# openjamoses/TOSEM-2021-Replication

Hardware: AMD Instinct MI355X
Metric: train_tokens_per_s (higher is better)
Workload: dtype bf16; 1 GPU; model=mltc-base, global_batch=128, seq_len=512, parallelism=dp1

## Files before the change

csrc/flash_attn.hip:

```cpp

#include "common.h"

typedef __attribute__((ext_vector_type(16))) float f32x16;
typedef __attribute__((ext_vector_type(2))) unsigned uint2_t;
typedef __attribute__((ext_vector_type(4))) unsigned uint4_t;

#define FA_DH 64
#define FA_KVB 32
#define FA_QB 32
#define FA_WAVES 4
#define FA_BLOCK (FA_WAVES * WAVE)
#define FA_QWG (FA_WAVES * FA_QB)
#define FA_Q2WG (2 * FA_QWG)

#define TILE_LDS_BYTES (FA_KVB * 128)
#define FWD_LDS_BYTES (2 * TILE_LDS_BYTES + FA_WAVES * 64 * sizeof(float))
#define BWD_LDS_BYTES (2 * TILE_LDS_BYTES + 64 * sizeof(float))
#define BWD_SEG_LDS_BYTES (BWD_LDS_BYTES + 32 * sizeof(int))
#define DQ_LDS_BYTES TILE_LDS_BYTES
#define DQR_LDS_BYTES (2 * TILE_LDS_BYTES + 16)

struct FaGeom {
  long qkv_bs, qkv_hs; int qkv_rs;
  long o_bs, o_hs; int o_rs;
  static FaGeom bhld(int H, int L) {
    return {(long)H * L * FA_DH, (long)L * FA_DH, FA_DH,
            (long)H * L * FA_DH, (long)L * FA_DH, FA_DH};
  }
  static FaGeom packed(int H, int L) {
    const int D = H * FA_DH;
    return {(long)L * 3 * D, 64L, 3 * D, (long)L * D, 64L, D};
  }
};


__device__ __forceinline__ int kswz(int row, int byte_off) {
  return byte_off ^ ((row & 7) << 4);
}

__device__ __forceinline__ int c_row(int r, int half) {
  return (r & 3) + 8 * (r >> 2) + 4 * half;
}

struct FaStager {
  int row, byte;
  __device__ __forceinline__ explicit FaStager(int tid)
      : row(tid >> 3), byte((tid & 7) * 16) {}
  __device__ __forceinline__ short8_t load(const short* base, int row0,
                                           int rs) const {
    return *(const short8_t*)(base + (long)(row0 + row) * rs + (byte >> 1));
  }
  __device__ __forceinline__ void store(short* lds, short8_t v) const {
    *(short8_t*)((char*)lds + row * 128 + kswz(row, byte)) = v;
  }
};

__device__ __forceinline__ short8_t tile_row_frag(const short* lds, int col,
                                                  int half, int c) {
  return *(const short8_t*)((const char*)lds + col * 128 +
                            kswz(col, (16 * c + 8 * half) * 2));
}

__device__ __forceinline__ void cvt_pk_swap(const float (&s)[16], int r0,
                                            int r1, uint4_t& u, int i) {
  unsigned lo, hi;
  asm("v_cvt_pk_bf16_f32 %0, %1, %2\n\ts_nop 1" : "=v"(lo)
      : "v"(s[r0]), "v"(s[r0 + 1]));
  asm("v_cvt_pk_bf16_f32 %0, %1, %2\n\ts_nop 1" : "=v"(hi)
      : "v"(s[r1]), "v"(s[r1 + 1]));
  auto sw = __builtin_amdgcn_permlane32_swap(lo, hi, false, false);
  u[i] = sw[0]; u[i + 2] = sw[1];
}

__device__ __forceinline__ void c_to_afrag2(const float (&sa)[16],
                                            short8_t (&fa)[2],
                                            const float (&sb)[16],
                                            short8_t (&fb)[2]) {
#pragma unroll
  for (int c = 0; c < 2; ++c) {
    uint4_t ua, ub;
#pragma unroll
    for (int i = 0; i < 2; ++i) {
      int r0 = c * 8 + 2 * i;
      int r1 = c * 8 + 4 + 2 * i;
      cvt_pk_swap(sa, r0, r1, ua, i);
      cvt_pk_swap(sb, r0, r1, ub, i);
    }
    fa[c] = __builtin_bit_cast(short8_t, ua);
    fb[c] = __builtin_bit_cast(short8_t, ub);
  }
}

struct FaTrFrags {
  uint2_t r[8];
  __device__ __forceinline__ short8_t frag(int c, int t) const {
    uint4_t w;
    w[0] = r[c * 4 + 0 * 2 + t][0];
    w[1] = r[c * 4 + 0 * 2 + t][1];
    w[2] = r[c * 4 + 1 * 2 + t][0];
    w[3] = r[c * 4 + 1 * 2 + t][1];
    return __builtin_bit_cast(short8_t, w);
  }
};

struct FaTrOffsets { unsigned a[8]; };

__device__ __forceinline__ FaTrOffsets tr_offsets(int lane, int half) {
  const int row_mate = (lane >> 2) & 3;
  const int d_lane = 16 * ((lane >> 4) & 1) + 4 * (lane & 3);
  FaTrOffsets o;
#pragma unroll
  for (int c = 0; c < 2; ++c)
#pragma unroll
    for (int rr = 0; rr < 2; ++rr)
#pragma unroll
      for (int t = 0; t < 2; ++t) {
        int row = 16 * c + 8 * half + 4 * rr + row_mate;
        int dcol = (32 * t + d_lane) * 2;
        o.a[c * 4 + rr * 2 + t] = row * 128 + kswz(row, dcol);
      }
  return o;
}

__device__ __forceinline__ void tr_issue(const short* lds,
                                         const FaTrOffsets& o, FaTrFrags& f) {
  const unsigned base = (unsigned)(unsigned long)(char*)lds;
  unsigned a[8];
#pragma unroll
  for (int i = 0; i < 8; ++i) a[i] = base + o.a[i];
  asm volatile(
      "ds_read_b64_tr_b16 %0, %8\n\t"
      "ds_read_b64_tr_b16 %1, %9\n\t"
      "ds_read_b64_tr_b16 %2, %10\n\t"
      "ds_read_b64_tr_b16 %3, %11\n\t"
      "ds_read_b64_tr_b16 %4, %12\n\t"
      "ds_read_b64_tr_b16 %5, %13\n\t"
      "ds_read_b64_tr_b16 %6, %14\n\t"
      "ds_read_b64_tr_b16 %7, %15\n\t"
      "s_waitcnt lgkmcnt(0)"
      : "=&v"(f.r[0]), "=&v"(f.r[1]), "=&v"(f.r[2]), "=&v"(f.r[3]),
        "=&v"(f.r[4]), "=&v"(f.r[5]), "=&v"(f.r[6]), "=&v"(f.r[7])
      : "v"(a[0]), "v"(a[1]), "v"(a[2]), "v"(a[3]), "v"(a[4]), "v"(a[5]),
        "v"(a[6]), "v"(a[7])
      : "memory");
}

__device__ __forceinline__ void tr_gather(const short* lds,
                                          const FaTrOffsets& o, FaTrFrags& f) {
  tr_issue(lds, o, f);
  __builtin_amdgcn_sched_barrier(0);
}

struct FaQBlocks { int bh, qA, qB; };

__device__ __forceinline__ FaQBlocks fa_qblocks(int L, int wid) {
  const int n_qblocks = (L + FA_Q2WG - 1) / FA_Q2WG;
  const int bid = xcd_group_remap(blockIdx.x, gridDim.x, n_qblocks);
  const int qA = (bid % n_qblocks) * FA_Q2WG + wid * FA_QB;
  return {bid / n_qblocks, qA, qA + FA_QWG};
}

__device__ __forceinline__ int fa_last_active_kv(const float* mrow, int L,
                                                 int tid, int* scratch) {
  if (tid == 0) *scratch = -1;
  __syncthreads();
  int loc = -1;
  for (int kv = tid; kv < L; kv += FA_BLOCK)
    if (mrow[kv] > -1.0e8f) loc = kv;
  if (loc >= 0) atomicMax(scratch, loc);
  __syncthreads();
  return *scratch;
}

#define FA_SEG_BIAS -1.0e9f

struct FaRange { int lo, hi; };

__device__ __forceinline__ FaRange fa_seg_range(const int* srow, int L,
                                                int r_lo, int r_hi, int tid,
                                                int* scratch) {
  const int s_first = srow[r_lo], s_last = srow[r_hi];
  if (tid == 0) { scratch[0] = r_lo; scratch[1] = r_hi; }
  __syncthreads();
  int lo = r_lo, hi = r_hi;
  for (int j = tid; j < L; j += FA_BLOCK) {
    const int s = srow[j];
    if (s == s_first) lo = min(lo, j);
    if (s == s_last) hi = max(hi, j);
  }
  atomicMin(&scratch[0], lo);
  atomicMax(&scratch[1], hi);
  __syncthreads();
  return {scratch[0], scratch[1]};
}

__device__ __forceinline__ bool fa_seg_tile_live(const int (&r)[16], int a,
                                                 int b) {
  bool hit = false;
#pragma unroll
  for (int i = 0; i < 16; ++i) hit |= (r[i] == a) | (r[i] == b);
  return __builtin_amdgcn_ballot_w64(hit) != 0;
}

template <bool SEG>
__global__ void __launch_bounds__(FA_BLOCK, 2)
flash_fwd_kernel(const short* __restrict__ q, const short* __restrict__ k,
                 const short* __restrict__ v, const float* __restrict__ mask,
                 const int* __restrict__ seg,
                 short* __restrict__ o, float* __restrict__ lse,
                 int B, int H, int L, float scale, FaGeom g) {
  extern __shared__ __attribute__((aligned(16))) char smem[];
  short* k_lds = (short*)smem;
  short* v_lds = (short*)(smem + TILE_LDS_BYTES);
  float* alpha_lds = (float*)(smem + 2 * TILE_LDS_BYTES);

  const int tid = threadIdx.x;
  const int lane = tid & (WAVE - 1);
  const int wid = tid / WAVE;
  const int col = lane & 31;
  const int half = lane >> 5;
  const FaTrOffsets tro = tr_offsets(lane, half);

  const FaQBlocks qb = fa_qblocks(L, wid);
  const int b = qb.bh / H;
  const int h = qb.bh % H;
  const long qkv_off = (long)b * g.qkv_bs + (long)h * g.qkv_hs;
  const long o_off = (long)b * g.o_bs + (long)h * g.o_hs;
  const int my_qA = qb.qA + col;
  const int my_qB = qb.qB + col;
  const bool validA = my_qA < L;
  const bool validB = my_qB < L;
  const float* mrow = (!SEG && mask) ? mask + (long)b * L : nullptr;
  const int* srow = SEG ? seg + (long)b * L : nullptr;
  int sqA = 0, sqB = 0;
  if constexpr (SEG) {
    sqA = srow[validA ? my_qA : L - 1];
    sqB = srow[validB ? my_qB : L - 1];
  }

  short8_t qfA[4], qfB[4];
  {
    const short* qrA = q + qkv_off + (long)(validA ? my_qA : L - 1) * g.qkv_rs;
    const short* qrB = q + qkv_off + (long)(validB ? my_qB : L - 1) * g.qkv_rs;
#pragma unroll
    for (int c = 0; c < 4; ++c) {
      qfA[c] = *(const short8_t*)(qrA + c * 16 + half * 8);
      qfB[c] = *(const short8_t*)(qrB + c * 16 + half * 8);
    }
  }

  f32x16 oA[2], oB[2];
#pragma unroll
  for (int t = 0; t < 2; ++t) { oA[t] = (f32x16)(0.f); oB[t] = (f32x16)(0.f); }
  float mA = -3.0e38f, lA = 0.f, mB = -3.0e38f, lB = 0.f;

  const int n_kv = L / FA_KVB;
  int kt_begin = 0;
  int n_kv_eff = n_kv;
  if (mrow) {
    int last = fa_last_active_kv(mrow, L, tid, (int*)alpha_lds);
    if (last >= 0) n_kv_eff = min(n_kv, last / FA_KVB + 1);
  }
  if constexpr (SEG) {
    const int q_lo = qb.qA - wid * FA_QB;
    const FaRange kr = fa_seg_range(srow, L, q_lo, min(q_lo + FA_Q2WG, L) - 1,
                                    tid, (int*)alpha_lds);
    kt_begin = kr.lo / FA_KVB;
    n_kv_eff = kr.hi / FA_KVB + 1;
  }
  const FaStager st(tid);
  short8_t kv8 = st.load(k + qkv_off, kt_begin * FA_KVB, g.qkv_rs);
  short8_t vv8 = st.load(v + qkv_off, kt_begin * FA_KVB, g.qkv_rs);
  for (int kt = kt_begin; kt < n_kv_eff; ++kt) {
    const int kv0 = kt * FA_KVB;
    __syncthreads();
    st.store(k_lds, kv8);
    st.store(v_lds, vv8);
    __syncthreads();
    if (kt + 1 < n_kv_eff) {
      kv8 = st.load(k + qkv_off, kv0 + FA_KVB, g.qkv_rs);
      vv8 = st.load(v + qkv_off, kv0 + FA_KVB, g.qkv_rs);
    }

    float mb_r[16];
    int sk_r[16];
#pragma unroll
    for (int r = 0; r < 16; ++r) {
      if constexpr (SEG) sk_r[r] = srow[kv0 + c_row(r, half)];
      else mb_r[r] = mrow ? mrow[kv0 + c_row(r, half)] : 0.f;
    }
    if constexpr (SEG) {
      if (!fa_seg_tile_live(sk_r, sqA, sqB)) continue;
    }

    f32x16 sA = (f32x16)(0.f), sB = (f32x16)(0.f);
    __builtin_amdgcn_s_setprio(1);
#pragma unroll
    for (int c = 0; c < 4; ++c) {
      short8_t kf = tile_row_frag(k_lds, col, half, c);
      sA = __builtin_amdgcn_mfma_f32_32x32x16_bf16(kf, qfA[c], sA, 0, 0, 0);
      sB = __builtin_amdgcn_mfma_f32_32x32x16_bf16(kf, qfB[c], sB, 0, 0, 0);
    }
    __builtin_amdgcn_s_setprio(0);

    float svA[16], svB[16];
    float tmaxA = -3.0e38f, tmaxB = -3.0e38f;
#pragma unroll
    for (int r = 0; r < 16; ++r) {
      float mbA, mbB;
      if constexpr (SEG) {
        mbA = sk_r[r] == sqA ? 0.f : FA_SEG_BIAS;
        mbB = sk_r[r] == sqB ? 0.f : FA_SEG_BIAS;
      } else {
        mbA = mbB = mb_r[r];
      }
      float xA = sA[r] * scale + mbA;
      float xB = sB[r] * scale + mbB;
      svA[r] = xA; svB[r] = xB;
      tmaxA = fmaxf(tmaxA, xA);
      tmaxB = fmaxf(tmaxB, xB);
    }
    tmaxA = fmaxf(tmaxA, __shfl_xor(tmaxA, 32, WAVE));
    tmaxB = fmaxf(tmaxB, __shfl_xor(tmaxB, 32, WAVE));
    float mnA = fmaxf(mA, tmaxA), mnB = fmaxf(mB, tmaxB);
    float aA = __expf(mA - mnA), aB = __expf(mB - mnB);
    float rsA = 0.f, rsB = 0.f;
#pragma unroll
    for (int r = 0; r < 16; ++r) {
      svA[r] = __expf(svA[r] - mnA);
      svB[r] = __expf(svB[r] - mnB);
      rsA += svA[r];
      rsB += svB[r];
    }
    rsA += __shfl_xor(rsA, 32, WAVE);
    rsB += __shfl_xor(rsB, 32, WAVE);
    lA = lA * aA + rsA; mA = mnA;
    lB = lB * aB + rsB; mB = mnB;

    if (__builtin_amdgcn_ballot_w64(aA != 1.f || aB != 1.f)) {
      alpha_lds[wid * 64 + col] = aA;
      alpha_lds[wid * 64 + 32 + col] = aB;
#pragma unroll
      for (int t = 0; t < 2; ++t) {
#pragma unroll
        for (int r = 0; r < 16; ++r) {
          int qrow = c_row(r, half);
          oA[t][r] *= alpha_lds[wid * 64 + qrow];
          oB[t][r] *= alpha_lds[wid * 64 + 32 + qrow];
        }
      }
    }

    short8_t pfA[2], pfB[2];
    c_to_afrag2(svA, pfA, svB, pfB);

    FaTrFrags vT;
    tr_gather(v_lds, tro, vT);
    __builtin_amdgcn_s_setprio(1);
#pragma unroll
    for (int t = 0; t < 2; ++t) {
#pragma unroll
      for (int c = 0; c < 2; ++c) {
        short8_t vf = vT.frag(c, t);
        oA[t] = __builtin_amdgcn_mfma_f32_32x32x16_bf16(pfA[c], vf, oA[t],
                                                        0, 0, 0);
        oB[t] = __builtin_amdgcn_mfma_f32_32x32x16_bf16(pfB[c], vf, oB[t],
                                                        0, 0, 0);
      }
    }
    __builtin_amdgcn_s_setprio(0);
  }

  if (lse != nullptr && half == 0) {
    if (validA) lse[(long)qb.bh * L + my_qA] = mA + __logf(lA);
    if (validB) lse[(long)qb.bh * L + my_qB] = mB + __logf(lB);
  }
  const float invA = 1.0f / lA, invB = 1.0f / lB;
#pragma unroll
  for (int r = 0; r < 16; ++r) {
    int rloc = c_row(r, half);
    float iA = __shfl(invA, rloc, WAVE);
    float iB = __shfl(invB, rloc, WAVE);
    int qA = qb.qA + rloc, qB = qb.qB + rloc;
#pragma unroll
    for (int t = 0; t < 2; ++t) {
      if (qA < L)
        o[o_off + (long)qA * g.o_rs + 32 * t + col] =
            f32_to_bf16(oA[t][r] * iA);
      if (qB < L)
        o[o_off + (long)qB * g.o_rs + 32 * t + col] =
            f32_to_bf16(oB[t][r] * iB);
    }
  }
}

static dim3 fa_grid(int B, int H, int L, int rows_per_wg) {
  return dim3(B * H * ((L + rows_per_wg - 1) / rows_per_wg));
}

static void fa_fwd_dispatch(const short* q, const short* k, const short* v,
                            const void* mask, const void* seg, void* o,
                            void* lse, int B, int H, int L, float scale,
                            FaGeom g, hipStream_t stream) {
  const dim3 grid = fa_grid(B, H, L, FA_Q2WG);
  if (seg)
    flash_fwd_kernel<true><<<grid, FA_BLOCK, FWD_LDS_BYTES, stream>>>(
        q, k, v, nullptr, (const int*)seg, (short*)o, (float*)lse, B, H, L,
        scale, g);
  else
    flash_fwd_kernel<false><<<grid, FA_BLOCK, FWD_LDS_BYTES, stream>>>(
        q, k, v, (const float*)mask, nullptr, (short*)o, (float*)lse, B, H, L,
        scale, g);
}

extern "C" hipError_t flash_fwd_launch(const void* q, const void* k,
                                       const void* v, const void* mask,
                                       const void* seg, void* o, void* lse,
                                       int B, int H, int L, float scale,
                                       hipStream_t stream) {
  fa_fwd_dispatch((const short*)q, (const short*)k, (const short*)v, mask,
                  seg, o, lse, B, H, L, scale, FaGeom::bhld(H, L), stream);
  return hipGetLastError();
}

extern "C" hipError_t flash_fwd_packed_launch(const void* qkv,
                                              const void* mask,
                                              const void* seg, void* o,
                                              void* lse, int B, int H, int L,
                                              float scale,
                                              hipStream_t stream) {
  const int D = H * FA_DH;
  fa_fwd_dispatch((const short*)qkv, (const short*)qkv + D,
                  (const short*)qkv + 2 * D, mask, seg, o, lse, B, H, L,
                  scale, FaGeom::packed(H, L), stream);
  return hipGetLastError();
}



template <bool SEG>
__global__ void __launch_bounds__(FA_BLOCK, 2)
flash_bwd_fused_kernel(const short* __restrict__ q, const short* __restrict__ k,
                       const short* __restrict__ v,
                       const short* __restrict__ dout,
                       const float* __restrict__ mask,
                       const int* __restrict__ seg,
                       const float* __restrict__ lse,
                       const float* __restrict__ ddot,
                       short* __restrict__ ds, short* __restrict__ dk,
                       short* __restrict__ dv,
                       int B, int H, int L, float scale, FaGeom g) {
  extern __shared__ __attribute__((aligned(16))) char smem[];
  short* q_lds = (short*)smem;
  short* do_lds = (short*)(smem + TILE_LDS_BYTES);
  float* lse_lds = (float*)(smem + 2 * TILE_LDS_BYTES);
  float* dd_lds = lse_lds + 32;
  int* seg_lds = (int*)(dd_lds + 32);

  const int tid = threadIdx.x;
  const int lane = tid & (WAVE - 1);
  const int wid = tid / WAVE;
  const int col = lane & 31;
  const int half = lane >> 5;
  const FaTrOffsets tro = tr_offsets(lane, half);

  const int n_kvblocks = (L + FA_QWG - 1) / FA_QWG;
  int bid = xcd_group_remap(blockIdx.x, gridDim.x, n_kvblocks);
  int bh = bid / n_kvblocks;
  int kb = bid % n_kvblocks;
  const int b = bh / H;
  const int h = bh % H;
  const long qkv_off = (long)b * g.qkv_bs + (long)h * g.qkv_hs;
  const long o_off = (long)b * g.o_bs + (long)h * g.o_hs;
  const long bh_sq = (long)bh * L * L;
  const int kv_base = kb * FA_QWG + wid * FA_KVB;
  const int my_kv = kv_base + col;
  const bool kv_valid = my_kv < L;
  const float* mrow = (!SEG && mask) ? mask + (long)b * L : nullptr;
  const float mb = mrow ? mrow[min(my_kv, L - 1)] : 0.f;
  const int* srow = SEG ? seg + (long)b * L : nullptr;
  int sk = 0;
  if constexpr (SEG) sk = srow[min(my_kv, L - 1)];

  bool skip_tile = false;
  bool wave_skip = false;
  if (mrow && ds == nullptr) {
    int* any_lds = (int*)lse_lds;
    if (tid == 0) *any_lds = 0;
    __syncthreads();
    if (kv_valid && mb > -1.0e8f) *any_lds = 1;
    __syncthreads();
    skip_tile = (*any_lds == 0) && (mrow[0] > -1.0e8f);
    __syncthreads();
    wave_skip = !skip_tile && (mrow[0] > -1.0e8f) &&
        __builtin_amdgcn_ballot_w64(kv_valid && mb > -1.0e8f) == 0;
  }

  short8_t kf[4], vf[4];
  if (!skip_tile) {
    const short* kr = k + qkv_off + (long)(kv_valid ? my_kv : L - 1) * g.qkv_rs;
    const short* vr = v + qkv_off + (long)(kv_valid ? my_kv : L - 1) * g.qkv_rs;
#pragma unroll
    for (int c = 0; c < 4; ++c) {
      kf[c] = *(const short8_t*)(kr + c * 16 + half * 8);
      vf[c] = *(const short8_t*)(vr + c * 16 + half * 8);
    }
  }
  f32x16 dv_acc[2], dk_acc[2];
#pragma unroll
  for (int t = 0; t < 2; ++t) {
    dv_acc[t] = (f32x16)(0.f);
    dk_acc[t] = (f32x16)(0.f);
  }
  if (!skip_tile) {
  int qt_begin = 0;
  int n_q = L / 32;
  if constexpr (SEG) {
    const int kv_lo = kb * FA_QWG;
    const FaRange qr = fa_seg_range(srow, L, kv_lo, min(kv_lo + FA_QWG, L) - 1,
                                    tid, (int*)lse_lds);
    qt_begin = qr.lo / 32;
    n_q = qr.hi / 32 + 1;
  }
  const FaStager st(tid);
  short8_t qv8 = st.load(q + qkv_off, qt_begin * 32, g.qkv_rs);
  short8_t dv8 = st.load(dout + o_off, qt_begin * 32, g.o_rs);
  for (int qt = qt_begin; qt < n_q; ++qt) {
    const int q0 = qt * 32;
    __syncthreads();
    st.store(q_lds, qv8);
    st.store(do_lds, dv8);
    if (tid < 32) {
      lse_lds[tid] = lse[(long)bh * L + q0 + tid];
      dd_lds[tid] = ddot[(long)bh * L + q0 + tid];
      if constexpr (SEG) seg_lds[tid] = srow[q0 + tid];
    }
    __syncthreads();
    if (qt + 1 < n_q) {
      qv8 = st.load(q + qkv_off, q0 + 32, g.qkv_rs);
      dv8 = st.load(dout + o_off, q0 + 32, g.o_rs);
    }

    if (wave_skip) continue;
    int sq_r[16];
    if constexpr (SEG) {
#pragma unroll
      for (int r = 0; r < 16; ++r) sq_r[r] = seg_lds[c_row(r, half)];
      if (!fa_seg_tile_live(sq_r, sk, sk)) continue;
    }
    f32x16 s_acc = (f32x16)(0.f);
    f32x16 dp_acc = (f32x16)(0.f);
    __builtin_amdgcn_s_setprio(1);
#pragma unroll
    for (int c = 0; c < 4; ++c) {
      short8_t qfrag = tile_row_frag(q_lds, col, half, c);
      short8_t dofrag = tile_row_frag(do_lds, col, half, c);
      s_acc = __builtin_amdgcn_mfma_f32_32x32x16_bf16(qfrag, kf[c], s_acc,
                                                      0, 0, 0);
      dp_acc = __builtin_amdgcn_mfma_f32_32x32x16_bf16(dofrag, vf[c], dp_acc,
                                                       0, 0, 0);
    }
    __builtin_amdgcn_s_setprio(0);

    float pv[16], gv[16];
#pragma unroll
    for (int r = 0; r < 16; ++r) {
      int ql = c_row(r, half);
      float bias = mb;
      if constexpr (SEG) bias = sq_r[r] == sk ? 0.f : FA_SEG_BIAS;
      pv[r] = __expf(s_acc[r] * scale + bias - lse_lds[ql]);
      gv[r] = scale * pv[r] * (dp_acc[r] - dd_lds[ql]);
    }
    if (!SEG && ds != nullptr && kv_valid) {
#pragma unroll
      for (int r = 0; r < 16; ++r)
        ds[bh_sq + (long)(q0 + c_row(r, half)) * L + my_kv] =
            f32_to_bf16(gv[r]);
    }

    short8_t pf[2], gf[2];
    c_to_afrag2(pv, pf, gv, gf);

    FaTrFrags doT, qT;
    tr_issue(do_lds, tro, doT);
    tr_gather(q_lds, tro, qT);
    __builtin_amdgcn_s_setprio(1);
#pragma unroll
    for (int t = 0; t < 2; ++t) {
#pragma unroll
      for (int c = 0; c < 2; ++c) {
        dv_acc[t] = __builtin_amdgcn_mfma_f32_32x32x16_bf16(
            pf[c], doT.frag(c, t), dv_acc[t], 0, 0, 0);
        dk_acc[t] = __builtin_amdgcn_mfma_f32_32x32x16_bf16(
            gf[c], qT.frag(c, t), dk_acc[t], 0, 0, 0);
      }
    }
    __builtin_amdgcn_s_setprio(0);
  }
  }

#pragma unroll
  for (int t = 0; t < 2; ++t) {
#pragma unroll
    for (int r = 0; r < 16; ++r) {
      int kvl = c_row(r, half);
      if (kv_base + kvl >= L) continue;
      long off = qkv_off + (long)(kv_base + kvl) * g.qkv_rs + 32 * t + col;
      dv[off] = f32_to_bf16(dv_acc[t][r]);
      dk[off] = f32_to_bf16(dk_acc[t][r]);
    }
  }
}

static void fa_bwd_fused_dispatch(const short* q, const short* k,
                                  const short* v, const void* dout,
                                  const void* mask, const void* seg,
                                  const void* lse, const void* ddot, void* ds,
                                  short* dk, short* dv, int B, int H, int L,
                                  float scale, FaGeom g, hipStream_t stream) {
  const dim3 grid = fa_grid(B, H, L, FA_QWG);
  if (seg)
    flash_bwd_fused_kernel<true><<<grid, FA_BLOCK, BWD_SEG_LDS_BYTES,
                                   stream>>>(
        q, k, v, (const short*)dout, nullptr, (const int*)seg,
        (const float*)lse, (const float*)ddot, nullptr, dk, dv, B, H, L,
        scale, g);
  else
    flash_bwd_fused_kernel<false><<<grid, FA_BLOCK, BWD_LDS_BYTES, stream>>>(
        q, k, v, (const short*)dout, (const float*)mask, nullptr,
        (const float*)lse, (const float*)ddot, (short*)ds, dk, dv, B, H, L,
        scale, g);
}

extern "C" hipError_t flash_bwd_fused_launch(
    const void* q, const void* k, const void* v, const void* dout,
    const void* mask, const void* seg, const void* lse, const void* ddot,
    void* ds, void* dk, void* dv, int B, int H, int L, float scale,
    hipStream_t stream) {
  if (seg && ds) return hipErrorInvalidValue;
  fa_bwd_fused_dispatch((const short*)q, (const short*)k, (const short*)v,
                        dout, mask, seg, lse, ddot, ds, (short*)dk,
                        (short*)dv, B, H, L, scale, FaGeom::bhld(H, L),
                        stream);
  return hipGetLastError();
}

extern "C" hipError_t flash_bwd_fused_packed_launch(
    const void* qkv, const void* dout, const void* mask, const void* seg,
    const void* lse, const void* ddot, void* dqkv, int B, int H, int L,
    float scale, hipStream_t stream) {
  const int D = H * FA_DH;
  fa_bwd_fused_dispatch((const short*)qkv, (const short*)qkv + D,
                        (const short*)qkv + 2 * D, dout, mask, seg, lse, ddot,
                        nullptr, (short*)dqkv + D, (short*)dqkv + 2 * D, B, H,
                        L, scale, FaGeom::packed(H, L), stream);
  return hipGetLastError();
}

extern "C" __global__ void __launch_bounds__(FA_BLOCK, 2)
flash_dq_kernel(const short* __restrict__ ds, const short* __restrict__ k,
                short* __restrict__ dq, int B, int H, int L) {
  extern __shared__ __attribute__((aligned(16))) char smem[];
  short* k_lds = (short*)smem;

  const int tid = threadIdx.x;
  const int lane = tid & (WAVE - 1);
  const int wid = tid / WAVE;
  const int col = lane & 31;
  const int half = lane >> 5;
  const FaTrOffsets tro = tr_offsets(lane, half);

  const FaQBlocks qb = fa_qblocks(L, wid);
  const long bh_off = (long)qb.bh * L * FA_DH;
  const long bh_sq = (long)qb.bh * L * L;
  const int my_qA = min(qb.qA + col, L - 1);
  const int my_qB = min(qb.qB + col, L - 1);
  const short* dsA_row = ds + bh_sq + (long)my_qA * L;
  const short* dsB_row = ds + bh_sq + (long)my_qB * L;

  f32x16 oA[2], oB[2];
#pragma unroll
  for (int t = 0; t < 2; ++t) { oA[t] = (f32x16)(0.f); oB[t] = (f32x16)(0.f); }

  const int n_kv = L / FA_KVB;
  const FaStager st(tid);
  short8_t kv8 = st.load(k + bh_off, 0, FA_DH);
  for (int kt = 0; kt < n_kv; ++kt) {
    const int kv0 = kt * FA_KVB;
    __syncthreads();
    st.store(k_lds, kv8);
    __syncthreads();
    if (kt + 1 < n_kv) kv8 = st.load(k + bh_off, kv0 + FA_KVB, FA_DH);
    short8_t aA[2], aB[2];
#pragma unroll
    for (int c = 0; c < 2; ++c) {
      aA[c] = *(const short8_t*)(dsA_row + kv0 + 16 * c + 8 * half);
      aB[c] = *(const short8_t*)(dsB_row + kv0 + 16 * c + 8 * half);
    }
    FaTrFrags kT;
    tr_gather(k_lds, tro, kT);
    __builtin_amdgcn_s_setprio(1);
#pragma unroll
    for (int t = 0; t < 2; ++t) {
#pragma unroll
      for (int c = 0; c < 2; ++c) {
        short8_t kf = kT.frag(c, t);
        oA[t] = __builtin_amdgcn_mfma_f32_32x32x16_bf16(aA[c], kf, oA[t],
                                                        0, 0, 0);
        oB[t] = __builtin_amdgcn_mfma_f32_32x32x16_bf16(aB[c], kf, oB[t],
                                                        0, 0, 0);
      }
    }
    __builtin_amdgcn_s_setprio(0);
  }

#pragma unroll
  for (int t = 0; t < 2; ++t) {
#pragma unroll
    for (int r = 0; r < 16; ++r) {
      int rloc = c_row(r, half);
      int qA = qb.qA + rloc, qB = qb.qB + rloc;
      if (qA < L)
        dq[bh_off + (long)qA * FA_DH + 32 * t + col] = f32_to_bf16(oA[t][r]);
      if (qB < L)
        dq[bh_off + (long)qB * FA_DH + 32 * t + col] = f32_to_bf16(oB[t][r]);
    }
  }
}

extern "C" hipError_t flash_dq_launch(const void* ds, const void* k, void* dq,
                                      int B, int H, int L,
                                      hipStream_t stream) {
  flash_dq_kernel<<<fa_grid(B, H, L, FA_Q2WG), FA_BLOCK, DQ_LDS_BYTES,
                    stream>>>(
      (const short*)ds, (const short*)k, (short*)dq, B, H, L);
  return hipGetLastError();
}

template <bool SEG>
__global__ void __launch_bounds__(FA_BLOCK, 2)
flash_dq_recompute_kernel(const short* __restrict__ q,
                          const short* __restrict__ k,
                          const short* __restrict__ v,
                          const short* __restrict__ dout,
                          const float* __restrict__ mask,
                          const int* __restrict__ seg,
                          const float* __restrict__ lse,
                          const float* __restrict__ ddot,
                          short* __restrict__ dq,
                          int B, int H, int L, float scale, FaGeom g) {
  extern __shared__ __attribute__((aligned(16))) char smem[];
  short* k_lds = (short*)smem;
  short* v_lds = (short*)(smem + TILE_LDS_BYTES);
  int* skip_scratch = (int*)(smem + 2 * TILE_LDS_BYTES);

  const int tid = threadIdx.x;
  const int lane = tid & (WAVE - 1);
  const int wid = tid / WAVE;
  const int col = lane & 31;
  const int half = lane >> 5;
  const FaTrOffsets tro = tr_offsets(lane, half);

  const FaQBlocks qb = fa_qblocks(L, wid);
  const int b = qb.bh / H;
  const int h = qb.bh % H;
  const long qkv_off = (long)b * g.qkv_bs + (long)h * g.qkv_hs;
  const long o_off = (long)b * g.o_bs + (long)h * g.o_hs;
  const int my_qA = qb.qA + col;
  const int my_qB = qb.qB + col;
  const bool validA = my_qA < L;
  const bool validB = my_qB < L;
  const float* mrow = (!SEG && mask) ? mask + (long)b * L : nullptr;
  const int* srow = SEG ? seg + (long)b * L : nullptr;
  int sqA = 0, sqB = 0;
  if constexpr (SEG) {
    sqA = srow[validA ? my_qA : L - 1];
    sqB = srow[validB ? my_qB : L - 1];
  }

  short8_t qfA[4], qfB[4], dofA[4], dofB[4];
  {
    const short* qrA = q + qkv_off + (long)(validA ? my_qA : L - 1) * g.qkv_rs;
    const short* qrB = q + qkv_off + (long)(validB ? my_qB : L - 1) * g.qkv_rs;
    const short* drA = dout + o_off + (long)(validA ? my_qA : L - 1) * g.o_rs;
    const short* drB = dout + o_off + (long)(validB ? my_qB : L - 1) * g.o_rs;
#pragma unroll
    for (int c = 0; c < 4; ++c) {
      qfA[c] = *(const short8_t*)(qrA + c * 16 + half * 8);
      qfB[c] = *(const short8_t*)(qrB + c * 16 + half * 8);
      dofA[c] = *(const short8_t*)(drA + c * 16 + half * 8);
      dofB[c] = *(const short8_t*)(drB + c * 16 + half * 8);
    }
  }
  const float lseA = lse[(long)qb.bh * L + (validA ? my_qA : L - 1)];
  const float lseB = lse[(long)qb.bh * L + (validB ? my_qB : L - 1)];
  const float ddA = ddot[(long)qb.bh * L + (validA ? my_qA : L - 1)];
  const float ddB = ddot[(long)qb.bh * L + (validB ? my_qB : L - 1)];

  f32x16 dqA[2], dqB[2];
#pragma unroll
  for (int t = 0; t < 2; ++t) { dqA[t] = (f32x16)(0.f); dqB[t] = (f32x16)(0.f); }

  const int n_kv = L / FA_KVB;
  int kt_begin = 0;
  int n_kv_eff = n_kv;
  if (mrow) {
    int last = fa_last_active_kv(mrow, L, tid, skip_scratch);
    if (last >= 0) n_kv_eff = min(n_kv, last / FA_KVB + 1);
  }
  if constexpr (SEG) {
    const int q_lo = qb.qA - wid * FA_QB;
    const FaRange kr = fa_seg_range(srow, L, q_lo, min(q_lo + FA_Q2WG, L) - 1,
                                    tid, skip_scratch);
    kt_begin = kr.lo / FA_KVB;
    n_kv_eff = kr.hi / FA_KVB + 1;
  }
  const FaStager st(tid);
  short8_t kv8 = st.load(k + qkv_off, kt_begin * FA_KVB, g.qkv_rs);
  short8_t vv8 = st.load(v + qkv_off, kt_begin * FA_KVB, g.qkv_rs);
  for (int kt = kt_begin; kt < n_kv_eff; ++kt) {
    const int kv0 = kt * FA_KVB;
    __syncthreads();
    st.store(k_lds, kv8);
    st.store(v_lds, vv8);
    __syncthreads();
    if (kt + 1 < n_kv_eff) {
      kv8 = st.load(k + qkv_off, kv0 + FA_KVB, g.qkv_rs);
      vv8 = st.load(v + qkv_off, kv0 + FA_KVB, g.qkv_rs);
    }

    float mb_r[16];
    int sk_r[16];
#pragma unroll
    for (int r = 0; r < 16; ++r) {
      if constexpr (SEG) sk_r[r] = srow[kv0 + c_row(r, half)];
      else mb_r[r] = mrow ? mrow[kv0 + c_row(r, half)] : 0.f;
    }
    if constexpr (SEG) {
      if (!fa_seg_tile_live(sk_r, sqA, sqB)) continue;
    }

    f32x16 sA = (f32x16)(0.f), sB = (f32x16)(0.f);
    f32x16 pA = (f32x16)(0.f), pB = (f32x16)(0.f);
    __builtin_amdgcn_s_setprio(1);
#pragma unroll
    for (int c = 0; c < 4; ++c) {
      short8_t kf = tile_row_frag(k_lds, col, half, c);
      short8_t vf = tile_row_frag(v_lds, col, half, c);
      sA = __builtin_amdgcn_mfma_f32_32x32x16_bf16(kf, qfA[c], sA, 0, 0, 0);
      sB = __builtin_amdgcn_mfma_f32_32x32x16_bf16(kf, qfB[c], sB, 0, 0, 0);
      pA = __builtin_amdgcn_mfma_f32_32x32x16_bf16(vf, dofA[c], pA, 0, 0, 0);
      pB = __builtin_amdgcn_mfma_f32_32x32x16_bf16(vf, dofB[c], pB, 0, 0, 0);
    }
    __builtin_amdgcn_s_setprio(0);

    float gA[16], gB[16];
#pragma unroll
    for (int r = 0; r < 16; ++r) {
      float mbA, mbB;
      if constexpr (SEG) {
        mbA = sk_r[r] == sqA ? 0.f : FA_SEG_BIAS;
        mbB = sk_r[r] == sqB ? 0.f : FA_SEG_BIAS;
      } else {
        mbA = mbB = mb_r[r];
      }
      float expA = __expf(sA[r] * scale + mbA - lseA);
      float expB = __expf(sB[r] * scale + mbB - lseB);
      gA[r] = scale * expA * (pA[r] - ddA);
      gB[r] = scale * expB * (pB[r] - ddB);
    }

    short8_t gfA[2], gfB[2];
    c_to_afrag2(gA, gfA, gB, gfB);

    FaTrFrags kT;
    tr_gather(k_lds, tro, kT);
    __builtin_amdgcn_s_setprio(1);
#pragma unroll
    for (int t = 0; t < 2; ++t) {
#pragma unroll
      for (int c = 0; c < 2; ++c) {
        short8_t kf = kT.frag(c, t);
        dqA[t] = __builtin_amdgcn_mfma_f32_32x32x16_bf16(gfA[c], kf, dqA[t],
                                                         0, 0, 0);
        dqB[t] = __builtin_amdgcn_mfma_f32_32x32x16_bf16(gfB[c], kf, dqB[t],
                                                         0, 0, 0);
      }
    }
    __builtin_amdgcn_s_setprio(0);
  }

#pragma unroll
  for (int t = 0; t < 2; ++t) {
#pragma unroll
    for (int r = 0; r < 16; ++r) {
      int rloc = c_row(r, half);
      int qA = qb.qA + rloc, qB = qb.qB + rloc;
      if (qA < L)
        dq[qkv_off + (long)qA * g.qkv_rs + 32 * t + col] =
            f32_to_bf16(dqA[t][r]);
      if (qB < L)
        dq[qkv_off + (long)qB * g.qkv_rs + 32 * t + col] =
            f32_to_bf16(dqB[t][r]);
    }
  }
}

static void fa_dq_recompute_dispatch(const short* q, const short* k,
                                     const short* v, const void* dout,
                                     const void* mask, const void* seg,
                                     const void* lse, const void* ddot,
                                     void* dq, int B, int H, int L,
                                     float scale, FaGeom g,
                                     hipStream_t stream) {
  const dim3 grid = fa_grid(B, H, L, FA_Q2WG);
  if (seg)
    flash_dq_recompute_kernel<true><<<grid, FA_BLOCK, DQR_LDS_BYTES,
                                      stream>>>(
        q, k, v, (const short*)dout, nullptr, (const int*)seg,
        (const float*)lse, (const float*)ddot, (short*)dq, B, H, L, scale, g);
  else
    flash_dq_recompute_kernel<false><<<grid, FA_BLOCK, DQR_LDS_BYTES,
                                       stream>>>(
        q, k, v, (const short*)dout, (const float*)mask, nullptr,
        (const float*)lse, (const float*)ddot, (short*)dq, B, H, L, scale, g);
}

extern "C" hipError_t flash_dq_recompute_launch(
    const void* q, const void* k, const void* v, const void* dout,
    const void* mask, const void* seg, const void* lse, const void* ddot,
    void* dq, int B, int H, int L, float scale, hipStream_t stream) {
  fa_dq_recompute_dispatch((const short*)q, (const short*)k, (const short*)v,
                           dout, mask, seg, lse, ddot, dq, B, H, L, scale,
                           FaGeom::bhld(H, L), stream);
  return hipGetLastError();
}

extern "C" hipError_t flash_dq_recompute_packed_launch(
    const void* qkv, const void* dout, const void* mask, const void* seg,
    const void* lse, const void* ddot, void* dqkv, int B, int H, int L,
    float scale, hipStream_t stream) {
  const int D = H * FA_DH;
  fa_dq_recompute_dispatch((const short*)qkv, (const short*)qkv + D,
                           (const short*)qkv + 2 * D, dout, mask, seg, lse,
                           ddot, dqkv, B, H, L, scale, FaGeom::packed(H, L),
                           stream);
  return hipGetLastError();
}

__device__ __forceinline__ float fa_row_dot(const short* dr, const short* orow,
                                            int sub) {
  short4_t a = *(const short4_t*)(dr + sub * 4);
  short4_t c = *(const short4_t*)(orow + sub * 4);
  float s = 0.f;
#pragma unroll
  for (int j = 0; j < 4; ++j) s += bf16_to_f32(a[j]) * bf16_to_f32(c[j]);
#pragma unroll
  for (int off = 8; off > 0; off >>= 1) s += __shfl_xor(s, off, 16);
  return s;
}

extern "C" __global__ void __launch_bounds__(256)
fa_dot_kernel(const short* __restrict__ dout, const short* __restrict__ o,
              float* __restrict__ ddot, long n_rows) {
  long row = ((long)blockIdx.x * 256 + threadIdx.x) >> 4;
  if (row >= n_rows) return;
  int sub = threadIdx.x & 15;
  float s = fa_row_dot(dout + row * FA_DH, o + row * FA_DH, sub);
  if (sub == 0) ddot[row] = s;
}

extern "C" __global__ void __launch_bounds__(256)
fa_dot_packed_kernel(const short* __restrict__ dout,
                     const short* __restrict__ o, float* __restrict__ ddot,
                     int B, int H, int L) {
  const int D = H * FA_DH;
  long n_rows = (long)B * L * H;
  long chunk = ((long)blockIdx.x * 256 + threadIdx.x) >> 4;
  if (chunk >= n_rows) return;
  int sub = threadIdx.x & 15;
  int h = (int)(chunk % H);
  long bl = chunk / H;
  int l = (int)(bl % L);
  int b = (int)(bl / L);
  float s = fa_row_dot(dout + bl * D + h * FA_DH, o + bl * D + h * FA_DH, sub);
  if (sub == 0) ddot[((long)b * H + h) * L + l] = s;
}

extern "C" hipError_t fa_dot_packed_launch(const void* dout, const void* o,
                                           void* ddot, int B, int H, int L,
                                           hipStream_t stream) {
  long total_threads = (long)B * H * L * 16;
  int grid = (int)((total_threads + 255) / 256);
  fa_dot_packed_kernel<<<grid, 256, 0, stream>>>(
      (const short*)dout, (const short*)o, (float*)ddot, B, H, L);
  return hipGetLastError();
}

extern "C" hipError_t fa_dot_launch(const void* dout, const void* o,
                                    void* ddot, long n_rows,
                                    hipStream_t stream) {
  long total_threads = n_rows * 16;
  int grid = (int)((total_threads + 255) / 256);
  fa_dot_kernel<<<grid, 256, 0, stream>>>((const short*)dout, (const short*)o,
                                          (float*)ddot, n_rows);
  return hipGetLastError();
}

extern "C" __global__ void __launch_bounds__(64)
tr_probe_kernel(const short* __restrict__ src, short* __restrict__ out,
                int scheme) {
  __shared__ __attribute__((aligned(16))) short lds[256];
  int lane = threadIdx.x;
  for (int i = lane; i < 256; i += 64) lds[i] = src[i];
  __syncthreads();
  int addr;
  switch (scheme) {
    case 0: addr = 0; break;
    case 1: addr = (lane & 15) * 2; break;
    case 2: addr = ((lane & 15) + (lane >> 4) * 64) * 2; break;
    case 3: addr = (lane >> 4) * 128; break;
    case 4: addr = (lane & 3) * 16; break;
    case 5: addr = ((lane & 3) * 32 + 4 * ((lane >> 2) & 7)) * 2; break;
    case 6: addr = ((lane & 3) * 8 + 4) * 2; break;
    case 7: addr = ((lane & 3) == 0) ? 16 : 0; break;
    case 8: addr = ((lane & 3) == 1) ? 16 : 0; break;
    case 9: addr = ((lane & 3) == 2) ? 16 : 0; break;
    case 10: addr = ((lane & 3) == 3) ? 16 : 0; break;
    case 11: addr = ((lane & 3) * 64 + 4 * ((lane >> 2) & 7)) * 2; break;
    default: addr = ((lane & 3) * 8 + ((lane >> 2) & 7) * 32) * 2; break;
  }
  typedef __attribute__((ext_vector_type(2))) unsigned uint2_t;
  uint2_t r;
  unsigned base = (unsigned)(unsigned long)((char*)lds + addr);
  asm volatile("ds_read_b64_tr_b16 %0, %1\n\ts_waitcnt lgkmcnt(0)"
               : "=v"(r) : "v"(base) : "memory");
  __builtin_amdgcn_sched_barrier(0);
  out[lane * 4 + 0] = (short)(r[0] & 0xffff);
  out[lane * 4 + 1] = (short)(r[0] >> 16);
  out[lane * 4 + 2] = (short)(r[1] & 0xffff);
  out[lane * 4 + 3] = (short)(r[1] >> 16);
}

extern "C" hipError_t tr_probe_launch(const void* src, void* out, int scheme,
                                      hipStream_t stream) {
  tr_probe_kernel<<<1, 64, 0, stream>>>((const short*)src, (short*)out,
                                        scheme);
  return hipGetLastError();
}
```

csrc/layernorm.hip:

```cpp

#include "common.h"
#include <cstdlib>
#include <cstring>

#define WAVES_PER_BLOCK 4
#define BLOCK (WAVES_PER_BLOCK * WAVE)
#define MAX_PKT 8

extern "C" {

__global__ void __launch_bounds__(BLOCK)
ln_fwd_kernel(const short* __restrict__ x, const short* __restrict__ res,
              const short* __restrict__ gamma,
              const short* __restrict__ beta, short* __restrict__ y,
              short* __restrict__ s_out,
              float* __restrict__ mean_out, float* __restrict__ rstd_out,
              int N, int D, float eps) {
  const int lane = threadIdx.x & (WAVE - 1);
  const int wid = threadIdx.x / WAVE;
  const int pkts = D / (WAVE * 8);
  for (int row = blockIdx.x * WAVES_PER_BLOCK + wid; row < N;
       row += gridDim.x * WAVES_PER_BLOCK) {
    const short* xr = x + (long)row * D;
    const short* rr = res ? res + (long)row * D : nullptr;
    short* yr = y + (long)row * D;
    short* sr = s_out ? s_out + (long)row * D : nullptr;
    float vals[MAX_PKT * 8];
    float s = 0.f;
    if (pkts <= MAX_PKT && D == pkts * WAVE * 8) {
#pragma unroll
      for (int p = 0; p < MAX_PKT; ++p) {
        if (p >= pkts) break;
        int base = (p * WAVE + lane) * 8;
        short8_t v = *(const short8_t*)(xr + base);
        short8_t so;
#pragma unroll
        for (int j = 0; j < 8; ++j) {
          float f = bf16_to_f32(v[j]);
          vals[p * 8 + j] = f;
        }
        if (rr) {
          short8_t rv = *(const short8_t*)(rr + base);
#pragma unroll
          for (int j = 0; j < 8; ++j) {
            short sum_b = f32_to_bf16(vals[p * 8 + j] + bf16_to_f32(rv[j]));
            vals[p * 8 + j] = bf16_to_f32(sum_b);
            so[j] = sum_b;
          }
          *(short8_t*)(sr + base) = so;
        }
#pragma unroll
        for (int j = 0; j < 8; ++j) s += vals[p * 8 + j];
      }
      float mean = wave_sum(s) / (float)D;
      float var = 0.f;
#pragma unroll
      for (int p = 0; p < MAX_PKT; ++p) {
        if (p >= pkts) break;
#pragma unroll
        for (int j = 0; j < 8; ++j) {
          float d = vals[p * 8 + j] - mean;
          var += d * d;
        }
      }
      var = wave_sum(var) / (float)D;
      float rstd = rsqrtf(var + eps);
      if (lane == 0) { mean_out[row] = mean; rstd_out[row] = rstd; }
#pragma unroll
      for (int p = 0; p < MAX_PKT; ++p) {
        if (p >= pkts) break;
        int base = (p * WAVE + lane) * 8;
        short8_t g8 = *(const short8_t*)(gamma + base);
        short8_t b8 = *(const short8_t*)(beta + base);
        short8_t o;
#pragma unroll
        for (int j = 0; j < 8; ++j) {
          float xhat = (vals[p * 8 + j] - mean) * rstd;
          o[j] = f32_to_bf16(xhat * bf16_to_f32(g8[j]) + bf16_to_f32(b8[j]));
        }
        *(short8_t*)(yr + base) = o;
      }
    } else {
      for (int i = lane * 8; i < D; i += WAVE * 8) {
        short8_t v = *(const short8_t*)(xr + i);
        if (rr) {
          short8_t rv = *(const short8_t*)(rr + i);
          short8_t so;
#pragma unroll
          for (int j = 0; j < 8; ++j) {
            so[j] = f32_to_bf16(bf16_to_f32(v[j]) + bf16_to_f32(rv[j]));
          }
          *(short8_t*)(sr + i) = so;
          v = so;
        }
#pragma unroll
        for (int j = 0; j < 8; ++j) s += bf16_to_f32(v[j]);
      }
      float mean = wave_sum(s) / (float)D;
      float var = 0.f;
      for (int i = lane * 8; i < D; i += WAVE * 8) {
        short8_t v = *(const short8_t*)((rr ? sr : xr) + i);
#pragma unroll
        for (int j = 0; j < 8; ++j) {
          float d = bf16_to_f32(v[j]) - mean;
          var += d * d;
        }
      }
      var = wave_sum(var) / (float)D;
      float rstd = rsqrtf(var + eps);
      if (lane == 0) { mean_out[row] = mean; rstd_out[row] = rstd; }
      for (int i = lane * 8; i < D; i += WAVE * 8) {
        short8_t v = *(const short8_t*)((rr ? sr : xr) + i);
        short8_t g8 = *(const short8_t*)(gamma + i);
        short8_t b8 = *(const short8_t*)(beta + i);
        short8_t o;
#pragma unroll
        for (int j = 0; j < 8; ++j) {
          float xhat = (bf16_to_f32(v[j]) - mean) * rstd;
          o[j] = f32_to_bf16(xhat * bf16_to_f32(g8[j]) + bf16_to_f32(b8[j]));
        }
        *(short8_t*)(yr + i) = o;
      }
    }
  }
}

}

template <int PKTS, bool HASRES>
__global__ void __launch_bounds__(BLOCK)
ln_fwd_t(const short* __restrict__ x, const short* __restrict__ res,
         const short* __restrict__ gamma, const short* __restrict__ beta,
         short* __restrict__ y, short* __restrict__ s_out,
         float* __restrict__ mean_out, float* __restrict__ rstd_out,
         int N, int D, float eps) {
  const int lane = threadIdx.x & (WAVE - 1);
  const int wid = threadIdx.x / WAVE;
  const int rstride = gridDim.x * WAVES_PER_BLOCK;
  int row = blockIdx.x * WAVES_PER_BLOCK + wid;
  if (row >= N) return;
  float gv[PKTS * 8], bv[PKTS * 8];
#pragma unroll
  for (int p = 0; p < PKTS; ++p) {
    int base = (p * WAVE + lane) * 8;
    short8_t g8 = *(const short8_t*)(gamma + base);
    short8_t b8 = *(const short8_t*)(beta + base);
#pragma unroll
    for (int j = 0; j < 8; ++j) {
      gv[p * 8 + j] = bf16_to_f32(g8[j]);
      bv[p * 8 + j] = bf16_to_f32(b8[j]);
    }
  }
  short8_t vx[PKTS], vr[PKTS];
#pragma unroll
  for (int p = 0; p < PKTS; ++p) {
    int base = (p * WAVE + lane) * 8;
    vx[p] = *(const short8_t*)(x + (long)row * D + base);
    if (HASRES) vr[p] = *(const short8_t*)(res + (long)row * D + base);
  }
  while (true) {
    const int next = row + rstride;
    float vals[PKTS * 8];
    float s = 0.f;
#pragma unroll
    for (int p = 0; p < PKTS; ++p) {
      short8_t so;
#pragma unroll
      for (int j = 0; j < 8; ++j) {
        float f = bf16_to_f32(vx[p][j]);
        if (HASRES) {
          short sum_b = f32_to_bf16(f + bf16_to_f32(vr[p][j]));
          f = bf16_to_f32(sum_b);
          so[j] = sum_b;
        }
        vals[p * 8 + j] = f;
        s += f;
      }
      if (HASRES)
        *(short8_t*)(s_out + (long)row * D + (p * WAVE + lane) * 8) = so;
    }
    if (next < N) {
#pragma unroll
      for (int p = 0; p < PKTS; ++p) {
        int base = (p * WAVE + lane) * 8;
        vx[p] = *(const short8_t*)(x + (long)next * D + base);
        if (HASRES) vr[p] = *(const short8_t*)(res + (long)next * D + base);
      }
    }
    float mean = wave_sum(s) / (float)D;
    float var = 0.f;
#pragma unroll
    for (int k = 0; k < PKTS * 8; ++k) {
      float d = vals[k] - mean;
      var += d * d;
    }
    var = wave_sum(var) / (float)D;
    float rstd = rsqrtf(var + eps);
    if (lane == 0) { mean_out[row] = mean; rstd_out[row] = rstd; }
#pragma unroll
    for (int p = 0; p < PKTS; ++p) {
      short8_t o;
#pragma unroll
      for (int j = 0; j < 8; ++j) {
        int k = p * 8 + j;
        o[j] = f32_to_bf16((vals[k] - mean) * rstd * gv[k] + bv[k]);
      }
      *(short8_t*)(y + (long)row * D + (p * WAVE + lane) * 8) = o;
    }
    if (next >= N) break;
    row = next;
  }
}

template <int PKTS, bool HASDE>
__global__ void __launch_bounds__(BLOCK)
ln_bwd_t(const short* __restrict__ dy, const short* __restrict__ x,
         const short* __restrict__ gamma, const float* __restrict__ mean_in,
         const float* __restrict__ rstd_in,
         const short* __restrict__ ds_extra, short* __restrict__ dx,
         float* __restrict__ ws_dgamma, float* __restrict__ ws_dbeta,
         int N, int D) {
  const int lane = threadIdx.x & (WAVE - 1);
  const int wid = threadIdx.x / WAVE;
  float gv[PKTS * 8];
#pragma unroll
  for (int p = 0; p < PKTS; ++p) {
    short8_t g8 = *(const short8_t*)(gamma + (p * WAVE + lane) * 8);
#pragma unroll
    for (int j = 0; j < 8; ++j) gv[p * 8 + j] = bf16_to_f32(g8[j]);
  }
  float dg_acc[PKTS * 8] = {0.f}, db_acc[PKTS * 8] = {0.f};
  const int rstride = gridDim.x * WAVES_PER_BLOCK;
  int row = blockIdx.x * WAVES_PER_BLOCK + wid;
  const bool active = row < N;
  short8_t vd[PKTS], vxp[PKTS], ve[PKTS];
  if (active) {
#pragma unroll
    for (int p = 0; p < PKTS; ++p) {
      int base = (p * WAVE + lane) * 8;
      vd[p] = *(const short8_t*)(dy + (long)row * D + base);
      vxp[p] = *(const short8_t*)(x + (long)row * D + base);
      if (HASDE) ve[p] = *(const short8_t*)(ds_extra + (long)row * D + base);
    }
  }
  while (active) {
    const int next = row + rstride;
    const float mean = mean_in[row], rstd = rstd_in[row];
    float xh[PKTS * 8], dyg[PKTS * 8], ev[PKTS * 8];
    float s1 = 0.f, s2 = 0.f;
#pragma unroll
    for (int p = 0; p < PKTS; ++p) {
#pragma unroll
      for (int j = 0; j < 8; ++j) {
        int k = p * 8 + j;
        float d = bf16_to_f32(vd[p][j]);
        float h = (bf16_to_f32(vxp[p][j]) - mean) * rstd;
        float g = d * gv[k];
        if (HASDE) ev[k] = bf16_to_f32(ve[p][j]);
        xh[k] = h; dyg[k] = g;
        dg_acc[k] += d * h;
        db_acc[k] += d;
        s1 += g; s2 += g * h;
      }
    }
    if (next < N) {
#pragma unroll
      for (int p = 0; p < PKTS; ++p) {
        int base = (p * WAVE + lane) * 8;
        vd[p] = *(const short8_t*)(dy + (long)next * D + base);
        vxp[p] = *(const short8_t*)(x + (long)next * D + base);
        if (HASDE) ve[p] = *(const short8_t*)(ds_extra + (long)next * D + base);
      }
    }
    s1 = wave_sum(s1) / (float)D;
    s2 = wave_sum(s2) / (float)D;
#pragma unroll
    for (int p = 0; p < PKTS; ++p) {
      short8_t o;
#pragma unroll
      for (int j = 0; j < 8; ++j) {
        int k = p * 8 + j;
        float d_ = rstd * (dyg[k] - s1 - xh[k] * s2);
        if (HASDE) d_ += ev[k];
        o[j] = f32_to_bf16(d_);
      }
      *(short8_t*)(dx + (long)row * D + (p * WAVE + lane) * 8) = o;
    }
    if (next >= N) break;
    row = next;
  }
  float* og = ws_dgamma +
              (long)(blockIdx.x * WAVES_PER_BLOCK + wid) * D;
  float* ob = ws_dbeta + (long)(blockIdx.x * WAVES_PER_BLOCK + wid) * D;
#pragma unroll
  for (int p = 0; p < PKTS; ++p) {
    int base = (p * WAVE + lane) * 8;
#pragma unroll
    for (int j = 0; j < 8; ++j) {
      og[base + j] = dg_acc[p * 8 + j];
      ob[base + j] = db_acc[p * 8 + j];
    }
  }
}

template <int PKTS, bool HASDE>
__global__ void __launch_bounds__(BLOCK)
ln_bwd_t2(const short* __restrict__ dy, const short* __restrict__ x,
          const short* __restrict__ gamma, const float* __restrict__ mean_in,
          const float* __restrict__ rstd_in,
          const short* __restrict__ ds_extra, short* __restrict__ dx,
          float* __restrict__ ws_dgamma, float* __restrict__ ws_dbeta,
          int N, int D) {
  const int lane = threadIdx.x & (WAVE - 1);
  const int wid = threadIdx.x / WAVE;
  float gv[PKTS * 8];
#pragma unroll
  for (int p = 0; p < PKTS; ++p) {
    short8_t g8 = *(const short8_t*)(gamma + (p * WAVE + lane) * 8);
#pragma unroll
    for (int j = 0; j < 8; ++j) gv[p * 8 + j] = bf16_to_f32(g8[j]);
  }
  float dg_acc[PKTS * 8] = {0.f}, db_acc[PKTS * 8] = {0.f};
  const int rstride = gridDim.x * WAVES_PER_BLOCK * 2;
  int rowA = (blockIdx.x * WAVES_PER_BLOCK + wid) * 2;
  short8_t vdA[PKTS], vxA[PKTS], veA[PKTS];
  short8_t vdB[PKTS], vxB[PKTS], veB[PKTS];
  bool actA = rowA < N, actB = rowA + 1 < N;
  if (actA) {
#pragma unroll
    for (int p = 0; p < PKTS; ++p) {
      int base = (p * WAVE + lane) * 8;
      vdA[p] = *(const short8_t*)(dy + (long)rowA * D + base);
      vxA[p] = *(const short8_t*)(x + (long)rowA * D + base);
      if (HASDE) veA[p] = *(const short8_t*)(ds_extra + (long)rowA * D + base);
      if (actB) {
        vdB[p] = *(const short8_t*)(dy + (long)(rowA + 1) * D + base);
        vxB[p] = *(const short8_t*)(x + (long)(rowA + 1) * D + base);
        if (HASDE)
          veB[p] = *(const short8_t*)(ds_extra + (long)(rowA + 1) * D + base);
      }
    }
  }
  while (actA) {
    const int next = rowA + rstride;
    const float meanA = mean_in[rowA], rstdA = rstd_in[rowA];
    const float meanB = actB ? mean_in[rowA + 1] : 0.f;
    const float rstdB = actB ? rstd_in[rowA + 1] : 0.f;
    float xhA[PKTS * 8], dygA[PKTS * 8];
    float xhB[PKTS * 8], dygB[PKTS * 8];
    float s1A = 0.f, s2A = 0.f, s1B = 0.f, s2B = 0.f;
#pragma unroll
    for (int p = 0; p < PKTS; ++p) {
#pragma unroll
      for (int j = 0; j < 8; ++j) {
        int k = p * 8 + j;
        float dA = bf16_to_f32(vdA[p][j]);
        float hA = (bf16_to_f32(vxA[p][j]) - meanA) * rstdA;
        float gA = dA * gv[k];
        xhA[k] = hA; dygA[k] = gA;
        dg_acc[k] += dA * hA;
        db_acc[k] += dA;
        s1A += gA; s2A += gA * hA;
        if (actB) {
          float dB = bf16_to_f32(vdB[p][j]);
          float hB = (bf16_to_f32(vxB[p][j]) - meanB) * rstdB;
          float gB = dB * gv[k];
          xhB[k] = hB; dygB[k] = gB;
          dg_acc[k] += dB * hB;
          db_acc[k] += dB;
          s1B += gB; s2B += gB * hB;
        }
      }
    }
    if (next < N) {
#pragma unroll
      for (int p = 0; p < PKTS; ++p) {
        int base = (p * WAVE + lane) * 8;
        vdA[p] = *(const short8_t*)(dy + (long)next * D + base);
        vxA[p] = *(const short8_t*)(x + (long)next * D + base);
        if (next + 1 < N) {
          vdB[p] = *(const short8_t*)(dy + (long)(next + 1) * D + base);
          vxB[p] = *(const short8_t*)(x + (long)(next + 1) * D + base);
        }
      }
    }
    s1A = wave_sum(s1A) / (float)D;
    s2A = wave_sum(s2A) / (float)D;
    if (actB) {
      s1B = wave_sum(s1B) / (float)D;
      s2B = wave_sum(s2B) / (float)D;
    }
#pragma unroll
    for (int p = 0; p < PKTS; ++p) {
      short8_t oA, oB;
#pragma unroll
      for (int j = 0; j < 8; ++j) {
        int k = p * 8 + j;
        float dA_ = rstdA * (dygA[k] - s1A - xhA[k] * s2A);
        if (HASDE) dA_ += bf16_to_f32(veA[p][j]);
        oA[j] = f32_to_bf16(dA_);
        if (actB) {
          float dB_ = rstdB * (dygB[k] - s1B - xhB[k] * s2B);
          if (HASDE) dB_ += bf16_to_f32(veB[p][j]);
          oB[j] = f32_to_bf16(dB_);
        }
      }
      int base = (p * WAVE + lane) * 8;
      *(short8_t*)(dx + (long)rowA * D + base) = oA;
      if (actB) *(short8_t*)(dx + (long)(rowA + 1) * D + base) = oB;
    }
    if (next >= N) break;
    rowA = next;
    actB = rowA + 1 < N;
    if (HASDE) {
#pragma unroll
      for (int p = 0; p < PKTS; ++p) {
        int base = (p * WAVE + lane) * 8;
        veA[p] = *(const short8_t*)(ds_extra + (long)rowA * D + base);
        if (actB)
          veB[p] = *(const short8_t*)(ds_extra + (long)(rowA + 1) * D + base);
      }
    }
  }
  float* og = ws_dgamma + (long)(blockIdx.x * WAVES_PER_BLOCK + wid) * D;
  float* ob = ws_dbeta + (long)(blockIdx.x * WAVES_PER_BLOCK + wid) * D;
#pragma unroll
  for (int p = 0; p < PKTS; ++p) {
    int base = (p * WAVE + lane) * 8;
#pragma unroll
    for (int j = 0; j < 8; ++j) {
      og[base + j] = dg_acc[p * 8 + j];
      ob[base + j] = db_acc[p * 8 + j];
    }
  }
}

template <int MAXP>
__global__ void __launch_bounds__(BLOCK)
ln_bwd_g(const short* __restrict__ dy, const short* __restrict__ x,
         const short* __restrict__ gamma, const float* __restrict__ mean_in,
         const float* __restrict__ rstd_in,
         const short* __restrict__ ds_extra,
         short* __restrict__ dx,
         float* __restrict__ ws_dgamma, float* __restrict__ ws_dbeta,
         int N, int D) {
  const int lane = threadIdx.x & (WAVE - 1);
  const int wid = threadIdx.x / WAVE;
  extern __shared__ __attribute__((aligned(16))) char smem[];
  float* sg = (float*)smem;
  float* sb = sg + D;
  float dg_acc[MAXP * 8] = {0.f}, db_acc[MAXP * 8] = {0.f};
  for (int row = blockIdx.x * WAVES_PER_BLOCK + wid; row < N;
       row += gridDim.x * WAVES_PER_BLOCK) {
    const short* dyr = dy + (long)row * D;
    const short* xr = x + (long)row * D;
    const short* der = ds_extra ? ds_extra + (long)row * D : nullptr;
    short* dxr = dx + (long)row * D;
    const float mean = mean_in[row], rstd = rstd_in[row];
    short8_t vd[MAXP], vx[MAXP], vg[MAXP];
    float s1 = 0.f, s2 = 0.f;
#pragma unroll
    for (int p = 0; p < MAXP; ++p) {
      int base = (p * WAVE + lane) * 8;
      if (base >= D) continue;
      vd[p] = *(const short8_t*)(dyr + base);
      vx[p] = *(const short8_t*)(xr + base);
      vg[p] = *(const short8_t*)(gamma + base);
#pragma unroll
      for (int j = 0; j < 8; ++j) {
        float d = bf16_to_f32(vd[p][j]);
        float h = (bf16_to_f32(vx[p][j]) - mean) * rstd;
        float g = d * bf16_to_f32(vg[p][j]);
        dg_acc[p * 8 + j] += d * h;
        db_acc[p * 8 + j] += d;
        s1 += g; s2 += g * h;
      }
    }
    s1 = wave_sum(s1) / (float)D;
    s2 = wave_sum(s2) / (float)D;
#pragma unroll
    for (int p = 0; p < MAXP; ++p) {
      int base = (p * WAVE + lane) * 8;
      if (base >= D) continue;
      short8_t ev;
      if (der) ev = *(const short8_t*)(der + base);
      short8_t o;
#pragma unroll
      for (int j = 0; j < 8; ++j) {
        float h = (bf16_to_f32(vx[p][j]) - mean) * rstd;
        float g = bf16_to_f32(vd[p][j]) * bf16_to_f32(vg[p][j]);
        float d_ = rstd * (g - s1 - h * s2);
        if (der) d_ += bf16_to_f32(ev[j]);
        o[j] = f32_to_bf16(d_);
      }
      *(short8_t*)(dxr + base) = o;
    }
  }
  for (int w = 0; w < WAVES_PER_BLOCK; ++w) {
    if (wid == w) {
#pragma unroll
      for (int p = 0; p < MAXP; ++p) {
        int base = (p * WAVE + lane) * 8;
        if (base >= D) continue;
#pragma unroll
        for (int j = 0; j < 8; ++j) {
          float pg = w ? sg[base + j] : 0.f, pb = w ? sb[base + j] : 0.f;
          sg[base + j] = pg + dg_acc[p * 8 + j];
          sb[base + j] = pb + db_acc[p * 8 + j];
        }
      }
    }
    __syncthreads();
  }
  float* og = ws_dgamma + (long)blockIdx.x * D;
  float* ob = ws_dbeta + (long)blockIdx.x * D;
  for (int i = threadIdx.x; i < D; i += BLOCK) { og[i] = sg[i]; ob[i] = sb[i]; }
}

#define LN_BWD_G_MAX_D 4096
__global__ void __launch_bounds__(BLOCK)
ln_bwd_wide_kernel(const short* __restrict__ dy, const short* __restrict__ x,
                   const short* __restrict__ gamma,
                   const float* __restrict__ mean_in,
                   const float* __restrict__ rstd_in,
                   const short* __restrict__ ds_extra,
                   short* __restrict__ dx, float* __restrict__ ws_dgamma,
                   float* __restrict__ ws_dbeta, int N, int D) {
  const int lane = threadIdx.x & (WAVE - 1);
  const int wid = threadIdx.x / WAVE;
  float* og = ws_dgamma + (long)(blockIdx.x * WAVES_PER_BLOCK + wid) * D;
  float* ob = ws_dbeta + (long)(blockIdx.x * WAVES_PER_BLOCK + wid) * D;
  for (int i = lane * 8; i < D; i += WAVE * 8) {
#pragma unroll
    for (int j = 0; j < 8; ++j) { og[i + j] = 0.f; ob[i + j] = 0.f; }
  }
  for (int row = blockIdx.x * WAVES_PER_BLOCK + wid; row < N;
       row += gridDim.x * WAVES_PER_BLOCK) {
    const short* dyr = dy + (long)row * D;
    const short* xr = x + (long)row * D;
    const short* der = ds_extra ? ds_extra + (long)row * D : nullptr;
    short* dxr = dx + (long)row * D;
    const float mean = mean_in[row], rstd = rstd_in[row];
    float s1 = 0.f, s2 = 0.f;
    for (int i = lane * 8; i < D; i += WAVE * 8) {
      short8_t vd = *(const short8_t*)(dyr + i);
      short8_t vx = *(const short8_t*)(xr + i);
      short8_t g8 = *(const short8_t*)(gamma + i);
#pragma unroll
      for (int j = 0; j < 8; ++j) {
        float g = bf16_to_f32(vd[j]) * bf16_to_f32(g8[j]);
        float h = (bf16_to_f32(vx[j]) - mean) * rstd;
        s1 += g; s2 += g * h;
      }
    }
    s1 = wave_sum(s1) / (float)D;
    s2 = wave_sum(s2) / (float)D;
    for (int i = lane * 8; i < D; i += WAVE * 8) {
      short8_t vd = *(const short8_t*)(dyr + i);
      short8_t vx = *(const short8_t*)(xr + i);
      short8_t g8 = *(const short8_t*)(gamma + i);
      short8_t ev;
      if (der) ev = *(const short8_t*)(der + i);
      short8_t o;
#pragma unroll
      for (int j = 0; j < 8; ++j) {
        float d = bf16_to_f32(vd[j]);
        float h = (bf16_to_f32(vx[j]) - mean) * rstd;
        float g = d * bf16_to_f32(g8[j]);
        float d_ = rstd * (g - s1 - h * s2);
        if (der) d_ += bf16_to_f32(ev[j]);
        o[j] = f32_to_bf16(d_);
        og[i + j] += d * h;
        ob[i + j] += d;
      }
      *(short8_t*)(dxr + i) = o;
    }
  }
}

extern "C" {

__global__ void __launch_bounds__(256)
colsum_stage_kernel(const float* __restrict__ ws, float* __restrict__ out,
                    int R, int D, int rows_per_split) {
  int col = (blockIdx.x * 256 + threadIdx.x) * 4;
  if (col >= D) return;
  int r0 = blockIdx.y * rows_per_split;
  int r1 = min(R, r0 + rows_per_split);
  float4_t s = {0.f, 0.f, 0.f, 0.f};
  for (int r = r0; r < r1; ++r) {
    float4_t v = *(const float4_t*)(ws + (long)r * D + col);
#pragma unroll
    for (int j = 0; j < 4; ++j) s[j] += v[j];
  }
  *(float4_t*)(out + (long)blockIdx.y * D + col) = s;
}

__global__ void __launch_bounds__(256)
colsum_bf16_stage1_kernel(const short* __restrict__ x,
                          float* __restrict__ scratch, long N, int D,
                          long rows_per_split) {
  int col = (blockIdx.x * 256 + threadIdx.x) * 8;
  if (col >= D) return;
  long r0 = (long)blockIdx.y * rows_per_split;
  long r1 = min(N, r0 + rows_per_split);
  float s[8] = {0.f};
  for (long r = r0; r < r1; ++r) {
    short8_t v = *(const short8_t*)(x + r * D + col);
#pragma unroll
    for (int j = 0; j < 8; ++j) s[j] += bf16_to_f32(v[j]);
  }
  float* out = scratch + (long)blockIdx.y * D + col;
#pragma unroll
  for (int j = 0; j < 8; ++j) out[j] = s[j];
}

__global__ void __launch_bounds__(256)
colsum_bf16_stage2_kernel(const float* __restrict__ scratch,
                          short* __restrict__ out, int splits, int D) {
  int col = blockIdx.x * 256 + threadIdx.x;
  if (col >= D) return;
  float s = 0.f;
  for (int r = 0; r < splits; ++r) s += scratch[(long)r * D + col];
  out[col] = f32_to_bf16(s);
}

hipError_t colsum_bf16_launch(const void* x, void* scratch, void* out,
                              long N, int D, hipStream_t stream) {
  int gx = (D / 8 + 255) / 256;
  int splits = 1024 / gx;
  if (splits > 1024) splits = 1024;
  if ((long)splits > N) splits = (int)N;
  long rows_per_split = (N + splits - 1) / splits;
  dim3 g1(gx, splits);
  colsum_bf16_stage1_kernel<<<g1, 256, 0, stream>>>(
      (const short*)x, (float*)scratch, N, D, rows_per_split);
  hipError_t e = hipGetLastError();
  if (e != hipSuccess) return e;
  if (splits > 16 && D % 4 == 0) {
    float* mid = (float*)scratch + (long)1024 * D;
    int rps2 = (splits + 15) / 16;
    colsum_stage_kernel<<<dim3((D / 4 + 255) / 256, 16), 256, 0, stream>>>(
        (const float*)scratch, mid, splits, D, rps2);
    e = hipGetLastError();
    if (e != hipSuccess) return e;
    colsum_bf16_stage2_kernel<<<dim3((D + 255) / 256), 256, 0, stream>>>(
        mid, (short*)out, 16, D);
    return hipGetLastError();
  }
  colsum_bf16_stage2_kernel<<<dim3((D + 255) / 256), 256, 0, stream>>>(
      (const float*)scratch, (short*)out, splits, D);
  return hipGetLastError();
}

hipError_t ln_fwd_launch(const void* x, const void* res, const void* gamma,
                         const void* beta, void* y, void* s_out, void* mean,
                         void* rstd, int N, int D, float eps, int grid,
                         hipStream_t stream) {
#define LNF_T(P)                                                              \
  do {                                                                        \
    if (res)                                                                  \
      ln_fwd_t<P, true><<<grid, BLOCK, 0, stream>>>(                          \
          (const short*)x, (const short*)res, (const short*)gamma,            \
          (const short*)beta, (short*)y, (short*)s_out, (float*)mean,         \
          (float*)rstd, N, D, eps);                                           \
    else                                                                      \
      ln_fwd_t<P, false><<<grid, BLOCK, 0, stream>>>(                         \
          (const short*)x, nullptr, (const short*)gamma, (const short*)beta,  \
          (short*)y, (short*)s_out, (float*)mean, (float*)rstd, N, D, eps);   \
  } while (0)
  if (D == 512) LNF_T(1);
  else if (D == 1024) LNF_T(2);
  else if (D == 2048) LNF_T(4);
  else
    ln_fwd_kernel<<<grid, BLOCK, 0, stream>>>(
        (const short*)x, (const short*)res, (const short*)gamma,
        (const short*)beta, (short*)y, (short*)s_out, (float*)mean,
        (float*)rstd, N, D, eps);
#undef LNF_T
  return hipGetLastError();
}

static int ln_bwd_use_1row() {
  static int v = -1;
  if (v < 0) {
    const char* e = getenv("TOSEM_LN_BWD");
    v = (e && strcmp(e, "1row") == 0) ? 1 : 0;
  }
  return v;
}

hipError_t ln_bwd_launch(const void* dy, const void* x, const void* gamma,
                         const void* mean, const void* rstd,
                         const void* ds_extra, void* dx,
                         void* ws_dgamma, void* ws_dbeta, int N, int D,
                         int grid, hipStream_t stream) {
  size_t shm = (size_t)D * 2 * sizeof(float);
#define LNB_T(P)                                                              \
  do {                                                                        \
    if (ln_bwd_use_1row()) {                                                  \
      if (ds_extra)                                                           \
        ln_bwd_t<P, true><<<grid, BLOCK, 0, stream>>>(                        \
            (const short*)dy, (const short*)x, (const short*)gamma,           \
            (const float*)mean, (const float*)rstd, (const short*)ds_extra,   \
            (short*)dx, (float*)ws_dgamma, (float*)ws_dbeta, N, D);           \
      else                                                                    \
        ln_bwd_t<P, false><<<grid, BLOCK, 0, stream>>>(                       \
            (const short*)dy, (const short*)x, (const short*)gamma,           \
            (const float*)mean, (const float*)rstd, nullptr, (short*)dx,      \
            (float*)ws_dgamma, (float*)ws_dbeta, N, D);                       \
      break;                                                                  \
    }                                                                         \
    if (ds_extra)                                                             \
      ln_bwd_t2<P, true><<<grid, BLOCK, 0, stream>>>(                         \
          (const short*)dy, (const short*)x, (const short*)gamma,             \
          (const float*)mean, (const float*)rstd, (const short*)ds_extra,     \
          (short*)dx, (float*)ws_dgamma, (float*)ws_dbeta, N, D);             \
    else                                                                      \
      ln_bwd_t2<P, false><<<grid, BLOCK, 0, stream>>>(                        \
          (const short*)dy, (const short*)x, (const short*)gamma,             \
          (const float*)mean, (const float*)rstd, nullptr, (short*)dx,        \
          (float*)ws_dgamma, (float*)ws_dbeta, N, D);                         \
  } while (0)
#define LNB_G(P)                                                              \
  ln_bwd_g<P><<<grid, BLOCK, shm, stream>>>(                                  \
      (const short*)dy, (const short*)x, (const short*)gamma,                 \
      (const float*)mean, (const float*)rstd, (const short*)ds_extra,         \
      (short*)dx, (float*)ws_dgamma, (float*)ws_dbeta, N, D)
  if (D == 512) LNB_T(1);
  else if (D == 1024) LNB_T(2);
  else if (D <= 512) LNB_G(1);
  else if (D <= 1024) LNB_G(2);
  else if (D <= 2048) LNB_G(4);
  else if (D <= LN_BWD_G_MAX_D) LNB_G(8);
  else
    ln_bwd_wide_kernel<<<grid, BLOCK, 0, stream>>>(
        (const short*)dy, (const short*)x, (const short*)gamma,
        (const float*)mean, (const float*)rstd, (const short*)ds_extra,
        (short*)dx, (float*)ws_dgamma, (float*)ws_dbeta, N, D);
#undef LNB_G
#undef LNB_T
  return hipGetLastError();
}

int ln_bwd_ws_rows(int D, int grid) {
  const bool per_wave = D == 512 || D == 1024 || D > LN_BWD_G_MAX_D;
  return per_wave ? grid * WAVES_PER_BLOCK : grid;
}

#define COLSUM_MAX_SPLITS 256
#define COLSUM_MID 16
hipError_t colsum_launch(const void* ws, void* scratch, void* out, int R,
                         int D, hipStream_t stream) {
  int gx = (D / 4 + 255) / 256;
  dim3 grid1(gx, 1);
  if (R <= COLSUM_MID) {
    colsum_stage_kernel<<<grid1, 256, 0, stream>>>(
        (const float*)ws, (float*)out, R, D, R);
    return hipGetLastError();
  }
  int splits = 1024 / gx;
  if (splits > COLSUM_MAX_SPLITS) splits = COLSUM_MAX_SPLITS;
  if (splits > R) splits = R;
  int rows_per_split = (R + splits - 1) / splits;
  colsum_stage_kernel<<<dim3(gx, splits), 256, 0, stream>>>(
      (const float*)ws, (float*)scratch, R, D, rows_per_split);
  hipError_t e = hipGetLastError();
  if (e != hipSuccess) return e;
  if (splits <= COLSUM_MID) {
    colsum_stage_kernel<<<grid1, 256, 0, stream>>>(
        (const float*)scratch, (float*)out, splits, D, splits);
    return hipGetLastError();
  }
  float* mid = (float*)scratch + (long)COLSUM_MAX_SPLITS * D;
  int rps2 = (splits + COLSUM_MID - 1) / COLSUM_MID;
  colsum_stage_kernel<<<dim3(gx, COLSUM_MID), 256, 0, stream>>>(
      (const float*)scratch, mid, splits, D, rps2);
  e = hipGetLastError();
  if (e != hipSuccess) return e;
  colsum_stage_kernel<<<grid1, 256, 0, stream>>>(
      mid, (float*)out, COLSUM_MID, D, COLSUM_MID);
  return hipGetLastError();
}

}
```

csrc/ops.cpp:

```cpp

#include <torch/extension.h>
#include <c10/hip/HIPStream.h>
#include <hip/hip_runtime.h>
#include <algorithm>
#include <numeric>

extern "C" {
hipError_t ln_fwd_launch(const void*, const void*, const void*, const void*,
                         void*, void*, void*, void*, int, int, float, int,
                         hipStream_t);
hipError_t ln_bwd_launch(const void*, const void*, const void*, const void*,
                         const void*, const void*, void*, void*, void*, int,
                         int, int, hipStream_t);
int ln_bwd_ws_rows(int, int);
hipError_t colsum_launch(const void*, void*, void*, int, int, hipStream_t);
hipError_t bias_gelu_fwd_launch(const void*, const void*, void*, long, int,
                                int, hipStream_t);
hipError_t bias_gelu_bwd_launch(const void*, const void*, const void*, void*,
                                void*, long, int, int, hipStream_t);
hipError_t softmax_fwd_launch(const void*, const void*, void*, long, int, int,
                              float, int, hipStream_t);
hipError_t softmax_bwd_launch(const void*, const void*, void*, long, int,
                              float, int, hipStream_t);
hipError_t adamw_launch(void*, const void*, int, void*, void*, void*, long,
                        float, float, float, float, float, int, float, int,
                        hipStream_t);
hipError_t adamw_clipped_launch(void*, const void*, int, void*, void*, void*,
                                long, float, float, float, float, float, int,
                                const void*, int, hipStream_t);
int grad_norm_grid(long);
hipError_t grad_clip_state_launch(const void*, int, long, float, float, void*,
                                  void*, hipStream_t);
hipError_t qkv_repack_launch(const void*, void*, int, int, int, int, int,
                             hipStream_t);
hipError_t out_repack_launch(const void*, void*, int, int, int, int, int,
                             hipStream_t);
hipError_t qkv_repack_bwd3_launch(const void*, const void*, const void*,
                                  void*, int, int, int, int, hipStream_t);
hipError_t flash_fwd_launch(const void*, const void*, const void*, const void*,
                            const void*, void*, void*, int, int, int, float,
                            hipStream_t);
hipError_t p_from_lse_launch(const void*, const void*, const void*, void*,
                             long, int, int, float, int, hipStream_t);
hipError_t flash_bwd_fused_launch(const void*, const void*, const void*,
                                  const void*, const void*, const void*,
                                  const void*, const void*, void*, void*,
                                  void*, int, int, int, float, hipStream_t);
hipError_t fa_dot_launch(const void*, const void*, void*, long, hipStream_t);
hipError_t fa_dot_packed_launch(const void*, const void*, void*, int, int,
                                int, hipStream_t);
hipError_t flash_fwd_packed_launch(const void*, const void*, const void*,
                                   void*, void*, int, int, int, float,
                                   hipStream_t);
hipError_t flash_bwd_fused_packed_launch(const void*, const void*,
                                         const void*, const void*,
                                         const void*, const void*, void*,
                                         int, int, int, float, hipStream_t);
hipError_t flash_dq_recompute_packed_launch(const void*, const void*,
                                            const void*, const void*,
                                            const void*, const void*, void*,
                                            int, int, int, float,
                                            hipStream_t);
hipError_t flash_dq_recompute_launch(const void*, const void*, const void*,
                                     const void*, const void*, const void*,
                                     const void*, const void*, void*, int,
                                     int, int, float, hipStream_t);
hipError_t flash_dq_launch(const void*, const void*, void*, int, int, int,
                           hipStream_t);
hipError_t masked_pool_fwd_launch(const void*, const void*, void*, void*,
                                  void*, int, int, int, hipStream_t);
hipError_t masked_pool_bwd_launch(const void*, const void*, const void*,
                                  void*, int, int, int, hipStream_t);
hipError_t segment_pool_fwd_launch(const void*, const void*, const void*,
                                   void*, int, long, int, hipStream_t);
hipError_t segment_pool_bwd_launch(const void*, const void*, const void*,
                                   void*, int, long, int, hipStream_t);
hipError_t tr_probe_launch(const void*, void*, int, hipStream_t);
hipError_t colsum_bf16_launch(const void*, void*, void*, long, int,
                              hipStream_t);
hipError_t wgrad_gemm_launch(const void*, const void*, void*, void*, int,
                             int, long, int, hipStream_t);
}

torch::Tensor lt_linear_gelu_bias(torch::Tensor, torch::Tensor,
                                  torch::Tensor);
bool lt_probe_epilogue(long, long, long, long);
std::vector<double> lt_bench_algos(long, long, long, bool, bool, long);

namespace {

#define CHECK_HIP(call)                                                   \
  do {                                                                    \
    hipError_t e_ = (call);                                               \
    TORCH_CHECK(e_ == hipSuccess, "HIP error: ", hipGetErrorString(e_));  \
  } while (0)

hipStream_t cur_stream() {
  return c10::hip::getCurrentHIPStream().stream();
}

void check_bf16(const torch::Tensor& t, const char* name) {
  TORCH_CHECK(t.is_contiguous(), name, " must be contiguous");
  TORCH_CHECK(t.scalar_type() == torch::kBFloat16, name, " must be bf16");
  TORCH_CHECK(t.device().is_cuda(), name, " must be on GPU");
}

void check_f32(const torch::Tensor& t, const char* name) {
  TORCH_CHECK(t.is_contiguous(), name, " must be contiguous");
  TORCH_CHECK(t.scalar_type() == torch::kFloat32, name, " must be f32");
  TORCH_CHECK(t.device().is_cuda(), name, " must be on GPU");
}


struct FlashDims { long B, H, L; };
using NamedTensor = std::pair<const char*, torch::Tensor>;

const void* flash_mask_ptr(const c10::optional<torch::Tensor>& mask,
                           const FlashDims& d) {
  if (!mask.has_value()) return nullptr;
  check_f32(*mask, "mask");
  TORCH_CHECK(mask->dim() == 2 && mask->size(0) == d.B &&
              mask->size(1) == d.L, "mask must be [B, L]");
  return mask->data_ptr();
}

const void* flash_seg_ptr(const c10::optional<torch::Tensor>& seg,
                          const c10::optional<torch::Tensor>& mask,
                          const torch::Tensor& x, const FlashDims& d) {
  if (!seg.has_value()) return nullptr;
  TORCH_CHECK(!mask.has_value(), "mask and seg are mutually exclusive");
  TORCH_CHECK(seg->scalar_type() == torch::kInt32, "seg must be int32");
  TORCH_CHECK(seg->device() == x.device(), "seg must be on the same device "
              "as the attention inputs");
  TORCH_CHECK(seg->is_contiguous(), "seg must be contiguous");
  TORCH_CHECK(seg->dim() == 2 && seg->size(0) == d.B && seg->size(1) == d.L,
              "seg must be [B, L]");
  return seg->data_ptr();
}

void check_i32(const torch::Tensor& t, const torch::Tensor& like,
               const char* name) {
  TORCH_CHECK(t.is_contiguous(), name, " must be contiguous");
  TORCH_CHECK(t.scalar_type() == torch::kInt32, name, " must be int32");
  TORCH_CHECK(t.device() == like.device(), name, " must be on the same "
              "device as the data");
}

void check_flash_rows(std::initializer_list<NamedTensor> rows,
                      const FlashDims& d) {
  for (const auto& [name, t] : rows) {
    check_f32(t, name);
    TORCH_CHECK(t.dim() == 3 && t.size(0) == d.B && t.size(1) == d.H &&
                t.size(2) == d.L, name, " must be [B, H, L]");
  }
}

FlashDims check_flash_bhld(const char* xname, const torch::Tensor& x,
                           std::initializer_list<NamedTensor> same,
                           std::initializer_list<NamedTensor> rows) {
  check_bf16(x, xname);
  TORCH_CHECK(x.dim() == 4, xname, " must be [B, H, L, 64]");
  const FlashDims d{x.size(0), x.size(1), x.size(2)};
  TORCH_CHECK(x.size(3) == 64, "flash kernels are specialized for head_dim 64");
  TORCH_CHECK(d.L % 32 == 0, "flash kernels need L % 32 == 0");
  for (const auto& [name, t] : same) {
    check_bf16(t, name);
    TORCH_CHECK(t.sizes() == x.sizes(), name, " must match ", xname,
                "'s shape");
  }
  check_flash_rows(rows, d);
  return d;
}

FlashDims check_flash_packed(const torch::Tensor& qkv, long H,
                             std::initializer_list<NamedTensor> outs,
                             std::initializer_list<NamedTensor> rows) {
  check_bf16(qkv, "qkv");
  TORCH_CHECK(qkv.dim() == 3, "qkv must be [B, L, 3D]");
  const FlashDims d{qkv.size(0), H, qkv.size(1)};
  TORCH_CHECK(qkv.size(2) == 3 * H * 64, "qkv last dim must be 3*H*64");
  TORCH_CHECK(d.L % 32 == 0, "flash kernels need L % 32 == 0");
  for (const auto& [name, t] : outs) {
    check_bf16(t, name);
    TORCH_CHECK(t.dim() == 3 && t.size(0) == d.B && t.size(1) == d.L &&
                t.size(2) == H * 64, name, " must be [B, L, H*64]");
  }
  check_flash_rows(rows, d);
  return d;
}

}

std::vector<torch::Tensor> layernorm_fwd(torch::Tensor x,
                                         c10::optional<torch::Tensor> residual,
                                         torch::Tensor gamma,
                                         torch::Tensor beta, double eps) {
  check_bf16(x, "x"); check_bf16(gamma, "gamma"); check_bf16(beta, "beta");
  const int D = (int)x.size(-1);
  const long N = x.numel() / D;
  TORCH_CHECK(D % 8 == 0, "D must be a multiple of 8, got ", D);
  auto y = torch::empty_like(x);
  auto opts = x.options().dtype(torch::kFloat32);
  auto mean = torch::empty({N}, opts);
  auto rstd = torch::empty({N}, opts);
  int grid = (int)std::min<long>((N + 3) / 4, 4096);
  const void* res_ptr = nullptr;
  torch::Tensor s_out;
  void* s_ptr = nullptr;
  if (residual.has_value()) {
    check_bf16(*residual, "residual");
    TORCH_CHECK(residual->sizes() == x.sizes(), "residual shape mismatch");
    res_ptr = residual->data_ptr();
    s_out = torch::empty_like(x);
    s_ptr = s_out.data_ptr();
  } else {
    s_out = x;
  }
  CHECK_HIP(ln_fwd_launch(x.data_ptr(), res_ptr, gamma.data_ptr(),
                          beta.data_ptr(), y.data_ptr(), s_ptr,
                          mean.data_ptr(), rstd.data_ptr(), (int)N, D,
                          (float)eps, grid, cur_stream()));
  return {y, s_out, mean, rstd};
}

std::vector<torch::Tensor> layernorm_bwd(torch::Tensor dy, torch::Tensor x,
                                         torch::Tensor gamma, torch::Tensor mean,
                                         torch::Tensor rstd,
                                         c10::optional<torch::Tensor> ds_extra) {
  check_bf16(dy, "dy"); check_bf16(x, "x"); check_bf16(gamma, "gamma");
  const int D = (int)x.size(-1);
  const long N = x.numel() / D;
  TORCH_CHECK(D % 8 == 0, "D must be a multiple of 8, got ", D);
  auto dx = torch::empty_like(x);
  int grid = (int)std::min<long>((N + 3) / 4, D > 4096 ? 256 : 1024);
  long ws_rows = ln_bwd_ws_rows(D, grid);
  auto opts = x.options().dtype(torch::kFloat32);
  auto ws_dg = torch::empty({ws_rows, D}, opts);
  auto ws_db = torch::empty({ws_rows, D}, opts);
  const void* de = nullptr;
  if (ds_extra.has_value()) {
    check_bf16(*ds_extra, "ds_extra");
    TORCH_CHECK(ds_extra->numel() == x.numel(), "ds_extra shape mismatch");
    de = ds_extra->data_ptr();
  }
  CHECK_HIP(ln_bwd_launch(dy.data_ptr(), x.data_ptr(), gamma.data_ptr(),
                          mean.data_ptr(), rstd.data_ptr(), de, dx.data_ptr(),
                          ws_dg.data_ptr(), ws_db.data_ptr(), (int)N, D, grid,
                          cur_stream()));
  auto dgamma = torch::empty({D}, opts);
  auto dbeta = torch::empty({D}, opts);
  auto scratch = torch::empty({256 + 16, D}, opts);
  CHECK_HIP(colsum_launch(ws_dg.data_ptr(), scratch.data_ptr(),
                          dgamma.data_ptr(), (int)ws_rows, D, cur_stream()));
  CHECK_HIP(colsum_launch(ws_db.data_ptr(), scratch.data_ptr(),
                          dbeta.data_ptr(), (int)ws_rows, D, cur_stream()));
  return {dx, dgamma, dbeta};
}

torch::Tensor bias_gelu_fwd(torch::Tensor x, torch::Tensor b) {
  check_bf16(x, "x"); check_bf16(b, "b");
  const int D = (int)x.size(-1);
  const long n = x.numel();
  TORCH_CHECK(D % 8 == 0, "D must be a multiple of 8");
  auto y = torch::empty_like(x);
  int grid = (int)std::min<long>((n / 32 + 255) / 256, 4096);
  long g0f = D / std::__gcd((long)D, 8192L);
  if (g0f <= 2048) grid = (int)((grid + g0f - 1) / g0f * g0f);
  CHECK_HIP(bias_gelu_fwd_launch(x.data_ptr(), b.data_ptr(), y.data_ptr(), n,
                                 D, grid, cur_stream()));
  return y;
}

std::vector<torch::Tensor> bias_gelu_bwd(torch::Tensor dy, torch::Tensor x,
                                         torch::Tensor b) {
  check_bf16(dy, "dy"); check_bf16(x, "x"); check_bf16(b, "b");
  const int D = (int)x.size(-1);
  const long n = x.numel();
  TORCH_CHECK(D % 8 == 0, "D must be a multiple of 8");
  auto dx = torch::empty_like(x);
  int grid = (int)std::min<long>((n / 32 + 255) / 256, 1024);
  long g = std::__gcd((long)D, 8192L);
  long g0 = D / g;
  if (g0 <= 2048) grid = (int)((grid + g0 - 1) / g0 * g0);
  auto ws = torch::empty({grid, D}, x.options().dtype(torch::kFloat32));
  CHECK_HIP(bias_gelu_bwd_launch(dy.data_ptr(), x.data_ptr(), b.data_ptr(),
                                 dx.data_ptr(), ws.data_ptr(), n, D, grid,
                                 cur_stream()));
  auto dbias = torch::empty({D}, x.options().dtype(torch::kFloat32));
  auto scratch = torch::empty({256 + 16, D},
                             x.options().dtype(torch::kFloat32));
  CHECK_HIP(colsum_launch(ws.data_ptr(), scratch.data_ptr(), dbias.data_ptr(),
                          grid, D, cur_stream()));
  return {dx, dbias};
}

torch::Tensor softmax_fwd(torch::Tensor scores, c10::optional<torch::Tensor> mask,
                          double scale) {
  check_bf16(scores, "scores");
  const int Lk = (int)scores.size(-1);
  const long n_rows = scores.numel() / Lk;
  TORCH_CHECK(Lk % 8 == 0, "Lk must be a multiple of 8");
  int H_Lq = 1;
  const void* mptr = nullptr;
  if (mask.has_value()) {
    check_f32(*mask, "mask");
    TORCH_CHECK(scores.dim() == 4, "masked softmax expects [B,H,Lq,Lk]");
    TORCH_CHECK(mask->size(0) == scores.size(0) && mask->size(-1) == Lk,
                "mask must be [B,Lk]");
    H_Lq = (int)(scores.size(1) * scores.size(2));
    mptr = mask->data_ptr();
  }
  auto p = torch::empty_like(scores);
  int grid = (int)std::min<long>((n_rows + 3) / 4, 2048);
  CHECK_HIP(softmax_fwd_launch(scores.data_ptr(), mptr, p.data_ptr(), n_rows,
                               Lk, H_Lq, (float)scale, grid, cur_stream()));
  return p;
}

torch::Tensor softmax_bwd(torch::Tensor dp, torch::Tensor p, double scale) {
  check_bf16(dp, "dp"); check_bf16(p, "p");
  const int Lk = (int)p.size(-1);
  const long n_rows = p.numel() / Lk;
  auto ds = torch::empty_like(p);
  int grid = (int)std::min<long>((n_rows + 3) / 4, 2048);
  CHECK_HIP(softmax_bwd_launch(dp.data_ptr(), p.data_ptr(), ds.data_ptr(),
                               n_rows, Lk, (float)scale, grid, cur_stream()));
  return ds;
}

void adamw_step(torch::Tensor p, torch::Tensor grad, torch::Tensor m,
                torch::Tensor v, torch::Tensor master, double lr, double beta1,
                double beta2, double eps, double wd, long step,
                double grad_scale) {
  check_bf16(p, "p"); check_f32(m, "m"); check_f32(v, "v");
  check_f32(master, "master");
  TORCH_CHECK(grad.is_contiguous() && grad.device().is_cuda(), "bad grad");
  int gf32 = grad.scalar_type() == torch::kFloat32;
  TORCH_CHECK(gf32 || grad.scalar_type() == torch::kBFloat16,
              "grad must be f32 or bf16");
  const long n = p.numel();
  TORCH_CHECK(n % 4 == 0, "flat parameter buffer must be padded to 4 elems");
  TORCH_CHECK(grad.numel() == n && m.numel() == n && v.numel() == n &&
              master.numel() == n, "size mismatch");
  int grid = (int)std::min<long>((n / 4 + 255) / 256, 2048);
  CHECK_HIP(adamw_launch(p.data_ptr(), grad.data_ptr(), gf32, m.data_ptr(),
                         v.data_ptr(), master.data_ptr(), n, (float)lr,
                         (float)beta1, (float)beta2, (float)eps, (float)wd,
                         (int)step, (float)grad_scale, grid, cur_stream()));
}

int check_flat_grad(const torch::Tensor& grad) {
  TORCH_CHECK(grad.is_contiguous() && grad.device().is_cuda(), "bad grad");
  int gf32 = grad.scalar_type() == torch::kFloat32;
  TORCH_CHECK(gf32 || grad.scalar_type() == torch::kBFloat16,
              "grad must be f32 or bf16");
  TORCH_CHECK(grad.numel() > 0 && grad.numel() % 8 == 0,
              "flat gradient buffer must be padded to 8 elems");
  TORCH_CHECK(reinterpret_cast<uintptr_t>(grad.data_ptr()) % 16 == 0,
              "flat gradient buffer must be 16-byte aligned");
  return gf32;
}

torch::Tensor grad_clip_state(torch::Tensor grad, double grad_scale,
                              double max_norm) {
  int gf32 = check_flat_grad(grad);
  TORCH_CHECK(max_norm > 0, "max_norm must be greater than 0");
  const long n = grad.numel();
  auto opts = torch::TensorOptions().dtype(torch::kFloat32)
                  .device(grad.device());
  auto partials = torch::empty({grad_norm_grid(n)}, opts);
  auto state = torch::empty({4}, opts);
  CHECK_HIP(grad_clip_state_launch(grad.data_ptr(), gf32, n,
                                   (float)grad_scale, (float)max_norm,
                                   partials.data_ptr(), state.data_ptr(),
                                   cur_stream()));
  return state;
}

void adamw_step_clipped(torch::Tensor p, torch::Tensor grad, torch::Tensor m,
                        torch::Tensor v, torch::Tensor master, double lr,
                        double beta1, double beta2, double eps, double wd,
                        long step, torch::Tensor clip_state) {
  check_bf16(p, "p"); check_f32(m, "m"); check_f32(v, "v");
  check_f32(master, "master"); check_f32(clip_state, "clip_state");
  int gf32 = check_flat_grad(grad);
  TORCH_CHECK(clip_state.numel() == 4, "clip_state must hold 4 floats");
  const long n = p.numel();
  TORCH_CHECK(grad.numel() == n && m.numel() == n && v.numel() == n &&
              master.numel() == n, "size mismatch");
  int grid = (int)std::min<long>((n / 4 + 255) / 256, 2048);
  CHECK_HIP(adamw_clipped_launch(p.data_ptr(), grad.data_ptr(), gf32,
                                 m.data_ptr(), v.data_ptr(),
                                 master.data_ptr(), n, (float)lr,
                                 (float)beta1, (float)beta2, (float)eps,
                                 (float)wd, (int)step, clip_state.data_ptr(),
                                 grid, cur_stream()));
}

torch::Tensor qkv_repack(torch::Tensor qkv, long H, bool backward) {
  check_bf16(qkv, "qkv");
  long B, L, dh;
  torch::Tensor out;
  if (!backward) {
    B = qkv.size(0); L = qkv.size(1);
    dh = qkv.numel() / (B * L * 3 * H);
    out = torch::empty({3, B, H, L, dh}, qkv.options());
  } else {
    B = qkv.size(1); L = qkv.size(3);
    dh = qkv.size(4);
    out = torch::empty({B, L, 3 * H * dh}, qkv.options());
  }
  TORCH_CHECK(dh % 8 == 0, "head_dim must be a multiple of 8");
  CHECK_HIP(qkv_repack_launch(qkv.data_ptr(), out.data_ptr(), (int)B, (int)L,
                              (int)H, (int)dh, backward ? 1 : 0,
                              cur_stream()));
  return out;
}

torch::Tensor qkv_repack_bwd3(torch::Tensor dq, torch::Tensor dk,
                              torch::Tensor dv) {
  check_bf16(dq, "dq"); check_bf16(dk, "dk"); check_bf16(dv, "dv");
  long B = dq.size(0), H = dq.size(1), L = dq.size(2), dh = dq.size(3);
  auto out = torch::empty({B, L, 3 * H * dh}, dq.options());
  CHECK_HIP(qkv_repack_bwd3_launch(dq.data_ptr(), dk.data_ptr(), dv.data_ptr(),
                                   out.data_ptr(), (int)B, (int)L, (int)H,
                                   (int)dh, cur_stream()));
  return out;
}

torch::Tensor out_repack(torch::Tensor x, bool backward) {
  check_bf16(x, "x");
  long B, L, H, dh;
  torch::Tensor out;
  if (!backward) {
    B = x.size(0); H = x.size(1); L = x.size(2); dh = x.size(3);
    out = torch::empty({B, L, H * dh}, x.options());
  } else {
    TORCH_CHECK(false, "pass the 4-D grad with explicit dims via out_repack_bwd");
  }
  TORCH_CHECK(dh % 8 == 0, "head_dim must be a multiple of 8");
  CHECK_HIP(out_repack_launch(x.data_ptr(), out.data_ptr(), (int)B, (int)L,
                              (int)H, (int)dh, 0, cur_stream()));
  return out;
}

torch::Tensor out_repack_bwd(torch::Tensor dgrad, long H) {
  check_bf16(dgrad, "dgrad");
  long B = dgrad.size(0), L = dgrad.size(1);
  long dh = dgrad.numel() / (B * L * H);
  auto out = torch::empty({B, H, L, dh}, dgrad.options());
  CHECK_HIP(out_repack_launch(dgrad.data_ptr(), out.data_ptr(), (int)B,
                              (int)L, (int)H, (int)dh, 1, cur_stream()));
  return out;
}

std::vector<torch::Tensor> flash_fwd(torch::Tensor q, torch::Tensor k,
                                     torch::Tensor v,
                                     c10::optional<torch::Tensor> mask,
                                     double scale,
                                     c10::optional<torch::Tensor> seg) {
  const auto [B, H, L] = check_flash_bhld("q", q, {{"k", k}, {"v", v}}, {});
  const void* mptr = flash_mask_ptr(mask, {B, H, L});
  const void* sptr = flash_seg_ptr(seg, mask, q, {B, H, L});
  auto o = torch::empty_like(q);
  auto lse = torch::empty({B, H, L}, q.options().dtype(torch::kFloat32));
  CHECK_HIP(flash_fwd_launch(q.data_ptr(), k.data_ptr(), v.data_ptr(), mptr,
                             sptr, o.data_ptr(), lse.data_ptr(), (int)B,
                             (int)H, (int)L, (float)scale, cur_stream()));
  return {o, lse};
}

torch::Tensor p_from_lse(torch::Tensor scores, c10::optional<torch::Tensor> mask,
                         torch::Tensor lse, double scale) {
  check_bf16(scores, "scores"); check_f32(lse, "lse");
  const int Lk = (int)scores.size(-1);
  const long n_rows = scores.numel() / Lk;
  TORCH_CHECK(lse.numel() == n_rows, "lse size mismatch");
  int H_Lq = 1;
  const void* mptr = nullptr;
  if (mask.has_value()) {
    check_f32(*mask, "mask");
    H_Lq = (int)(scores.size(1) * scores.size(2));
    mptr = mask->data_ptr();
  }
  auto p = torch::empty_like(scores);
  int grid = (int)std::min<long>((n_rows + 3) / 4, 2048);
  CHECK_HIP(p_from_lse_launch(scores.data_ptr(), mptr, lse.data_ptr(),
                              p.data_ptr(), n_rows, Lk, H_Lq, (float)scale,
                              grid, cur_stream()));
  return p;
}

torch::Tensor fa_dot(torch::Tensor dout, torch::Tensor o) {
  check_bf16(dout, "dout"); check_bf16(o, "o");
  TORCH_CHECK(dout.dim() == 4 && o.sizes() == dout.sizes(),
              "dout and o must both be [B, H, L, 64]");
  const long n_rows = dout.numel() / dout.size(-1);
  TORCH_CHECK(dout.size(-1) == 64, "fa_dot expects head_dim 64");
  auto d = torch::empty({n_rows}, dout.options().dtype(torch::kFloat32));
  CHECK_HIP(fa_dot_launch(dout.data_ptr(), o.data_ptr(), d.data_ptr(), n_rows,
                          cur_stream()));
  return d.view({dout.size(0), dout.size(1), dout.size(2)});
}

std::vector<torch::Tensor> flash_bwd_fused(torch::Tensor q, torch::Tensor k,
                                           torch::Tensor v, torch::Tensor dout,
                                           c10::optional<torch::Tensor> mask,
                                           torch::Tensor lse,
                                           torch::Tensor ddot, double scale,
                                           bool emit_ds,
                                           c10::optional<torch::Tensor> seg) {
  const auto [B, H, L] = check_flash_bhld(
      "q", q, {{"k", k}, {"v", v}, {"dout", dout}},
      {{"lse", lse}, {"ddot", ddot}});
  const void* mptr = flash_mask_ptr(mask, {B, H, L});
  const void* sptr = flash_seg_ptr(seg, mask, q, {B, H, L});
  TORCH_CHECK(!(sptr && emit_ds), "seg with emit_ds=True is not supported: "
              "the flash_dq A/B path is unsegmented");
  auto dk = torch::empty_like(k);
  auto dv = torch::empty_like(v);
  torch::Tensor ds;
  void* ds_ptr = nullptr;
  if (emit_ds) {
    ds = torch::empty({B, H, L, L}, q.options());
    ds_ptr = ds.data_ptr();
  }
  CHECK_HIP(flash_bwd_fused_launch(q.data_ptr(), k.data_ptr(), v.data_ptr(),
                                   dout.data_ptr(), mptr, sptr,
                                   lse.data_ptr(), ddot.data_ptr(), ds_ptr,
                                   dk.data_ptr(), dv.data_ptr(), (int)B,
                                   (int)H, (int)L, (float)scale,
                                   cur_stream()));
  if (emit_ds) return {ds, dk, dv};
  return {dk, dv};
}

torch::Tensor wgrad_gemm(torch::Tensor dy, torch::Tensor x,
                         long splits) {
  check_bf16(dy, "dy"); check_bf16(x, "x");
  TORCH_CHECK(dy.dim() == 2 && x.dim() == 2, "2-D operands required");
  const long K = dy.size(0), M = dy.size(1), N = x.size(1);
  TORCH_CHECK(x.size(0) == K, "K mismatch");
  TORCH_CHECK(M % 256 == 0 && N % 256 == 0, "M, N must be 256-multiples");
  TORCH_CHECK(K % 32 == 0, "K must be a 32-multiple");
  int S = (int)splits;
  if (S <= 0) {
    long tiles = (M / 256) * (N / 256);
    S = 1;
    while (S < 32 && tiles * S < 512 && (K / (2L * S)) % 32 == 0) S *= 2;
  }
  TORCH_CHECK((K / S) % 32 == 0, "K/S must be a 32-multiple");
  auto ws = torch::empty({S, M, N}, dy.options().dtype(torch::kFloat32));
  auto out = torch::empty({M, N}, dy.options());
  CHECK_HIP(wgrad_gemm_launch(dy.data_ptr(), x.data_ptr(), ws.data_ptr(),
                              out.data_ptr(), (int)M, (int)N, K, S,
                              cur_stream()));
  return out;
}

torch::Tensor bias_grad(torch::Tensor dy) {
  check_bf16(dy, "dy");
  const int D = (int)dy.size(-1);
  const long N = dy.numel() / D;
  TORCH_CHECK(D % 8 == 0, "D % 8 == 0 required");
  auto scratch = torch::empty({1024 + 16, D},
                              dy.options().dtype(torch::kFloat32));
  auto out = torch::empty({D}, dy.options());
  CHECK_HIP(colsum_bf16_launch(dy.data_ptr(), scratch.data_ptr(),
                               out.data_ptr(), N, D, cur_stream()));
  return out;
}

std::vector<torch::Tensor> flash_fwd_packed(torch::Tensor qkv, long H,
                                            c10::optional<torch::Tensor> mask,
                                            double scale,
                                            c10::optional<torch::Tensor> seg) {
  const auto dims = check_flash_packed(qkv, H, {}, {});
  const long B = dims.B, L = dims.L;
  const void* mptr = flash_mask_ptr(mask, dims);
  const void* sptr = flash_seg_ptr(seg, mask, qkv, dims);
  auto o = torch::empty({B, L, H * 64}, qkv.options());
  auto lse = torch::empty({B, H, L}, qkv.options().dtype(torch::kFloat32));
  CHECK_HIP(flash_fwd_packed_launch(qkv.data_ptr(), mptr, sptr, o.data_ptr(),
                                    lse.data_ptr(), (int)B, (int)H, (int)L,
                                    (float)scale, cur_stream()));
  return {o, lse};
}

torch::Tensor flash_bwd_packed(torch::Tensor qkv, torch::Tensor o,
                               torch::Tensor dout,
                               c10::optional<torch::Tensor> mask,
                               torch::Tensor lse, long H, double scale,
                               c10::optional<torch::Tensor> seg) {
  const auto dims = check_flash_packed(qkv, H, {{"o", o}, {"dout", dout}},
                                       {{"lse", lse}});
  const long B = dims.B, L = dims.L;
  const void* mptr = flash_mask_ptr(mask, dims);
  const void* sptr = flash_seg_ptr(seg, mask, qkv, dims);
  auto ddot = torch::empty({B, H, L}, qkv.options().dtype(torch::kFloat32));
  CHECK_HIP(fa_dot_packed_launch(dout.data_ptr(), o.data_ptr(),
                                 ddot.data_ptr(), (int)B, (int)H, (int)L,
                                 cur_stream()));
  auto dqkv = torch::empty_like(qkv);
  CHECK_HIP(flash_bwd_fused_packed_launch(
      qkv.data_ptr(), dout.data_ptr(), mptr, sptr, lse.data_ptr(),
      ddot.data_ptr(), dqkv.data_ptr(), (int)B, (int)H, (int)L, (float)scale,
      cur_stream()));
  CHECK_HIP(flash_dq_recompute_packed_launch(
      qkv.data_ptr(), dout.data_ptr(), mptr, sptr, lse.data_ptr(),
      ddot.data_ptr(), dqkv.data_ptr(), (int)B, (int)H, (int)L, (float)scale,
      cur_stream()));
  return dqkv;
}

torch::Tensor flash_dq_recompute(torch::Tensor q, torch::Tensor k,
                                 torch::Tensor v, torch::Tensor dout,
                                 c10::optional<torch::Tensor> mask,
                                 torch::Tensor lse, torch::Tensor ddot,
                                 double scale,
                                 c10::optional<torch::Tensor> seg) {
  const auto [B, H, L] = check_flash_bhld(
      "q", q, {{"k", k}, {"v", v}, {"dout", dout}},
      {{"lse", lse}, {"ddot", ddot}});
  const void* mptr = flash_mask_ptr(mask, {B, H, L});
  const void* sptr = flash_seg_ptr(seg, mask, q, {B, H, L});
  auto dq = torch::empty_like(q);
  CHECK_HIP(flash_dq_recompute_launch(q.data_ptr(), k.data_ptr(),
                                      v.data_ptr(), dout.data_ptr(), mptr,
                                      sptr, lse.data_ptr(), ddot.data_ptr(),
                                      dq.data_ptr(), (int)B, (int)H, (int)L,
                                      (float)scale, cur_stream()));
  return dq;
}

torch::Tensor flash_dq(torch::Tensor ds, torch::Tensor k) {
  const auto [B, H, L] = check_flash_bhld("k", k, {}, {});
  check_bf16(ds, "ds");
  TORCH_CHECK(ds.dim() == 4 && ds.size(0) == B && ds.size(1) == H &&
              ds.size(2) == L && ds.size(3) == L, "ds must be [B, H, L, L]");
  auto dq = torch::empty_like(k);
  CHECK_HIP(flash_dq_launch(ds.data_ptr(), k.data_ptr(), dq.data_ptr(),
                            (int)B, (int)H, (int)L, cur_stream()));
  return dq;
}

std::vector<torch::Tensor> masked_pool_fwd(torch::Tensor x,
                                           c10::optional<torch::Tensor> mask) {
  check_bf16(x, "x");
  TORCH_CHECK(x.dim() == 3, "x must be [B, L, D]");
  long B = x.size(0), L = x.size(1), D = x.size(2);
  TORCH_CHECK(D % 8 == 0, "D must be a multiple of 8");
  const void* mptr = nullptr;
  if (mask.has_value()) {
    TORCH_CHECK(mask->scalar_type() == torch::kBool && mask->is_contiguous(),
                "mask must be contiguous bool");
    mptr = mask->data_ptr();
  }
  auto pooled = torch::empty({B, D}, x.options());
  auto counts = torch::empty({B}, x.options().dtype(torch::kFloat32));
  auto ws = torch::empty({B, 16, D}, x.options().dtype(torch::kFloat32));
  CHECK_HIP(masked_pool_fwd_launch(x.data_ptr(), mptr, pooled.data_ptr(),
                                   counts.data_ptr(), ws.data_ptr(), (int)B,
                                   (int)L, (int)D, cur_stream()));
  return {pooled, counts};
}

torch::Tensor masked_pool_bwd(torch::Tensor dpooled,
                              c10::optional<torch::Tensor> mask,
                              torch::Tensor counts, long L) {
  check_bf16(dpooled, "dpooled");
  long B = dpooled.size(0), D = dpooled.size(1);
  const void* mptr = nullptr;
  if (mask.has_value()) mptr = mask->data_ptr();
  auto dx = torch::empty({B, L, D}, dpooled.options());
  CHECK_HIP(masked_pool_bwd_launch(dpooled.data_ptr(), mptr,
                                   counts.data_ptr(), dx.data_ptr(), (int)B,
                                   (int)L, (int)D, cur_stream()));
  return dx;
}

torch::Tensor segment_pool_fwd(torch::Tensor x, torch::Tensor seg_start,
                               torch::Tensor seg_len) {
  check_bf16(x, "x");
  TORCH_CHECK(x.dim() == 2, "x must be [T, D]");
  const long T = x.size(0), D = x.size(1);
  TORCH_CHECK(D % 8 == 0, "D must be a multiple of 8");
  check_i32(seg_start, x, "seg_start");
  check_i32(seg_len, x, "seg_len");
  TORCH_CHECK(seg_start.dim() == 1 && seg_len.dim() == 1 &&
              seg_start.size(0) == seg_len.size(0),
              "seg_start and seg_len must both be [N]");
  const long N = seg_start.size(0);
  auto pooled = torch::empty({N, D}, x.options());
  CHECK_HIP(segment_pool_fwd_launch(x.data_ptr(), seg_start.data_ptr(),
                                    seg_len.data_ptr(), pooled.data_ptr(),
                                    (int)N, T, (int)D, cur_stream()));
  return pooled;
}

torch::Tensor segment_pool_bwd(torch::Tensor dpooled, torch::Tensor pos2seg,
                               torch::Tensor seg_len, long T) {
  check_bf16(dpooled, "dpooled");
  TORCH_CHECK(dpooled.dim() == 2, "dpooled must be [N, D]");
  const long N = dpooled.size(0), D = dpooled.size(1);
  TORCH_CHECK(D % 8 == 0, "D must be a multiple of 8");
  check_i32(pos2seg, dpooled, "pos2seg");
  check_i32(seg_len, dpooled, "seg_len");
  TORCH_CHECK(pos2seg.dim() == 1 && pos2seg.size(0) == T,
              "pos2seg must be [T]");
  TORCH_CHECK(seg_len.dim() == 1 && seg_len.size(0) == N,
              "seg_len must be [N]");
  auto dx = torch::empty({T, D}, dpooled.options());
  CHECK_HIP(segment_pool_bwd_launch(dpooled.data_ptr(), pos2seg.data_ptr(),
                                    seg_len.data_ptr(), dx.data_ptr(), (int)N,
                                    T, (int)D, cur_stream()));
  return dx;
}

torch::Tensor tr_probe(torch::Tensor src, long scheme) {
  check_bf16(src, "src");
  TORCH_CHECK(src.numel() == 256);
  auto out = torch::zeros({64, 4}, src.options());
  CHECK_HIP(tr_probe_launch(src.data_ptr(), out.data_ptr(), (int)scheme,
                            cur_stream()));
  return out;
}

PYBIND11_MODULE(TORCH_EXTENSION_NAME, m) {
  m.def("tr_probe", &tr_probe, "ds_read_b64_tr_b16 semantics probe");
  m.def("masked_pool_fwd", &masked_pool_fwd, "masked mean-pool fwd");
  m.def("masked_pool_bwd", &masked_pool_bwd, "masked mean-pool bwd");
  m.def("segment_pool_fwd", &segment_pool_fwd,
        "per-segment mean-pool fwd (sequence packing)");
  m.def("segment_pool_bwd", &segment_pool_bwd,
        "per-segment mean-pool bwd (sequence packing)");
  m.def("flash_fwd", &flash_fwd,
        "flash attention fwd (gfx950 MFMA, dh=64); seg: optional int32 "
        "[B, L] non-decreasing segment ids, exclusive with mask",
        py::arg("q"), py::arg("k"), py::arg("v"), py::arg("mask"),
        py::arg("scale"), py::arg("seg") = py::none());
  m.def("flash_bwd_fused", &flash_bwd_fused,
        "fused flash bwd: register-accumulated dK/dV (+ optional dS)",
        py::arg("q"), py::arg("k"), py::arg("v"), py::arg("dout"),
        py::arg("mask"), py::arg("lse"), py::arg("ddot"), py::arg("scale"),
        py::arg("emit_ds") = false, py::arg("seg") = py::none());
  m.def("flash_dq_recompute", &flash_dq_recompute,
        "dQ by recompute: S/dP/dS in-register, no dS materialization",
        py::arg("q"), py::arg("k"), py::arg("v"), py::arg("dout"),
        py::arg("mask"), py::arg("lse"), py::arg("ddot"), py::arg("scale"),
        py::arg("seg") = py::none());
  m.def("wgrad_gemm", &wgrad_gemm,
        "split-K wgrad GEMM: dW = dy^T @ x (custom MFMA)",
        py::arg("dy"), py::arg("x"), py::arg("splits") = 0);
  m.def("flash_fwd_packed", &flash_fwd_packed,
        "flash fwd on the packed [B,L,3D] QKV projection output",
        py::arg("qkv"), py::arg("H"), py::arg("mask"), py::arg("scale"),
        py::arg("seg") = py::none());
  m.def("flash_bwd_packed", &flash_bwd_packed,
        "full packed flash bwd: ddot + dK/dV + dQ into one [B,L,3D] grad",
        py::arg("qkv"), py::arg("o"), py::arg("dout"), py::arg("mask"),
        py::arg("lse"), py::arg("H"), py::arg("scale"),
        py::arg("seg") = py::none());
  m.def("fa_dot", &fa_dot, "rowsum(dO*O) per attention row");
  m.def("flash_dq", &flash_dq, "dQ = dS @ K (MFMA, tr_b16 K^T fragments)");
  m.def("bias_grad", &bias_grad, "bf16 column-sum for linear bias grads");
  m.def("p_from_lse", &p_from_lse, "probabilities from saved logsumexp");
  m.def("qkv_repack", &qkv_repack, "qkv layout repack (fwd/bwd)");
  m.def("qkv_repack_bwd3", &qkv_repack_bwd3, "qkv repack bwd from dq,dk,dv");
  m.def("out_repack", &out_repack, "attention output merge");
  m.def("out_repack_bwd", &out_repack_bwd, "attention output merge bwd");
  m.def("layernorm_fwd", &layernorm_fwd, "fused LayerNorm fwd (bf16, gfx950)");
  m.def("layernorm_bwd", &layernorm_bwd, "fused LayerNorm bwd");
  m.def("bias_gelu_fwd", &bias_gelu_fwd, "fused bias+GeLU fwd");
  m.def("lt_linear_gelu_bias", &lt_linear_gelu_bias,
        "hipBLASLt GEMM with fused GELU_BIAS epilogue (inference)");
  m.def("lt_bench_algos", &lt_bench_algos,
        "time the heuristic's top algos for a bf16 GEMM config");
  m.def("lt_probe_epilogue", &lt_probe_epilogue,
        "does this hipBLASLt have kernels for (m, n, k, epilogue)?");
  m.def("bias_gelu_bwd", &bias_gelu_bwd, "fused bias+GeLU bwd");
  m.def("softmax_fwd", &softmax_fwd, "fused scaled masked softmax fwd");
  m.def("softmax_bwd", &softmax_bwd, "fused softmax bwd");
  m.def("adamw_step", &adamw_step, "fused AdamW over flat params");
  m.def("grad_clip_state", &grad_clip_state,
        "deterministic global grad norm -> device {norm, scale, finite, "
        "sumsq}");
  m.def("adamw_step_clipped", &adamw_step_clipped,
        "fused AdamW reading its grad scale / skip flag from clip_state");
}
```

tosem2021_amd/models/classifier.py:

```python
from __future__ import annotations

import math
import os
from dataclasses import dataclass, field
from typing import Dict, Optional

import torch
import torch.nn as nn
import torch.nn.functional as F

from tosem2021_amd import ops

N_STRATEGIES = 19
N_PROPERTIES = 21
N_STAGES = 9
N_METHODS = 4

HEAD_SIZES = {
    "strategy": N_STRATEGIES,
    "property": N_PROPERTIES,
    "stage": N_STAGES,
    "method": N_METHODS,
}
MULTILABEL_HEADS = ("strategy", "property")


@dataclass
class MLTCConfig:
    vocab_size: int = 32768
    d_model: int = 1024
    n_heads: int = 16
    n_layers: int = 12
    d_ff: int = 4096
    max_seq: int = 512
    dropout: float = 0.0
    layer_norm_eps: float = 1e-5
    heads: Dict[str, int] = field(default_factory=lambda: dict(HEAD_SIZES))

    @property
    def head_dim(self) -> int:
        assert self.d_model % self.n_heads == 0
        return self.d_model // self.n_heads


CONFIGS: Dict[str, MLTCConfig] = {
    "mltc-base": MLTCConfig(),
    "mltc-tiny": MLTCConfig(vocab_size=512, d_model=128, n_heads=4, n_layers=2,
                            d_ff=256, max_seq=64),
    "mltc-large": MLTCConfig(d_model=2048, n_heads=32, n_layers=24,
                             d_ff=8192),
}


class FusedLayerNorm(nn.Module):
    def __init__(self, d: int, eps: float):
        super().__init__()
        self.weight = nn.Parameter(torch.ones(d))
        self.bias = nn.Parameter(torch.zeros(d))
        self.eps = eps

    def forward(self, x):
        return ops.fused_layernorm(x, self.weight, self.bias, self.eps)


_USE_FUSED_LINEAR = os.environ.get("TOSEM_FUSED_LINEAR", "0") == "1"
_USE_WGRAD = os.environ.get("TOSEM_WGRAD", "0") == "1"


def _linear(mod: nn.Linear, x: torch.Tensor) -> torch.Tensor:
    if x.is_cuda and torch.is_grad_enabled():
        if _USE_WGRAD and ops.wgrad_linear_supported(
                mod.out_features, mod.in_features,
                x.numel() // x.shape[-1]):
            return ops.wgrad_linear(x, mod.weight, mod.bias)
        if _USE_FUSED_LINEAR and mod.bias is not None:
            return ops.fused_linear(x, mod.weight, mod.bias)
    return mod(x)


class Attention(nn.Module):

    def __init__(self, cfg: MLTCConfig):
        super().__init__()
        self.n_heads = cfg.n_heads
        self.head_dim = cfg.head_dim
        self.scale = 1.0 / math.sqrt(cfg.head_dim)
        self.qkv = nn.Linear(cfg.d_model, 3 * cfg.d_model, bias=True)
        self.proj = nn.Linear(cfg.d_model, cfg.d_model, bias=True)

    def forward(self, x, mask_bias: Optional[torch.Tensor],
                seg: Optional[torch.Tensor] = None):
        B, L, D = x.shape
        if ops.flash_supported(self.head_dim, L):
            out = ops.flash_attention_packed(_linear(self.qkv, x), self.n_heads,
                                             mask_bias, self.scale, seg)
            return _linear(self.proj, out)
        if seg is not None:
            if x.is_cuda:
                raise RuntimeError(
                    "sequence packing on the GPU needs the segment-aware "
                    f"flash kernels: head_dim 64 and L % 32 == 0, got "
                    f"head_dim {self.head_dim}, L {L}")
            q, k, v = ops.qkv_repack(self.qkv(x), self.n_heads)
            s = torch.matmul(q, k.transpose(-1, -2)).float() * self.scale
            p = torch.softmax(s + ops.reference.segment_bias(seg), dim=-1)
            out = torch.matmul(p.to(v.dtype), v)
            return self.proj(ops.out_repack(out))
        q, k, v = ops.qkv_repack(self.qkv(x), self.n_heads)
        scores = torch.matmul(q, k.transpose(-1, -2))
        p = ops.fused_softmax(scores, mask_bias, self.scale)
        out = torch.matmul(p, v)
        return self.proj(ops.out_repack(out))


class FFN(nn.Module):

    def __init__(self, cfg: MLTCConfig):
        super().__init__()
        self.up = nn.Linear(cfg.d_model, cfg.d_ff, bias=False)
        self.up_bias = nn.Parameter(torch.zeros(cfg.d_ff))
        self.down = nn.Linear(cfg.d_ff, cfg.d_model, bias=True)

    def forward(self, x):
        if x.is_cuda and not torch.is_grad_enabled():
            B, L, D = x.shape
            a = ops.lt_linear_gelu_bias(x.reshape(-1, D).contiguous(),
                                        self.up.weight, self.up_bias)
            return self.down(a.view(B, L, -1))
        h = _linear(self.up, x)
        h = ops.fused_bias_gelu(h, self.up_bias)
        return _linear(self.down, h)


class EncoderBlock(nn.Module):

    def __init__(self, cfg: MLTCConfig):
        super().__init__()
        self.ln1 = FusedLayerNorm(cfg.d_model, cfg.layer_norm_eps)
        self.attn = Attention(cfg)
        self.ln2 = FusedLayerNorm(cfg.d_model, cfg.layer_norm_eps)
        self.ffn = FFN(cfg)
        self.dropout = cfg.dropout

    def _drop(self, h):
        return F.dropout(h, self.dropout, self.training) if self.dropout else h

    def forward(self, x, delta, mask_bias, seg=None):
        if delta is None:
            y1 = ops.fused_layernorm(x, self.ln1.weight, self.ln1.bias,
                                     self.ln1.eps)
            s1 = x
        else:
            y1, s1 = ops.fused_add_layernorm(x, delta, self.ln1.weight,
                                             self.ln1.bias, self.ln1.eps)
        h = self._drop(self.attn(y1, mask_bias, seg))
        y2, s2 = ops.fused_add_layernorm(s1, h, self.ln2.weight,
                                         self.ln2.bias, self.ln2.eps)
        h2 = self._drop(self.ffn(y2))
        return s2, h2


class MLTC(nn.Module):
    def __init__(self, cfg: MLTCConfig):
        super().__init__()
        self.cfg = cfg
        self.tok_emb = nn.Embedding(cfg.vocab_size, cfg.d_model)
        self.pos_emb = nn.Embedding(cfg.max_seq, cfg.d_model)
        self.blocks = nn.ModuleList(EncoderBlock(cfg) for _ in range(cfg.n_layers))
        self.ln_f = FusedLayerNorm(cfg.d_model, cfg.layer_norm_eps)
        self.heads = nn.ModuleDict(
            {name: nn.Linear(cfg.d_model, n) for name, n in cfg.heads.items()}
        )
        self.apply(self._init)

    @staticmethod
    def _init(m):
        if isinstance(m, (nn.Linear, nn.Embedding)):
            nn.init.normal_(m.weight, std=0.02)
            if isinstance(m, nn.Linear) and m.bias is not None:
                nn.init.zeros_(m.bias)

    def forward(self, tokens: Optional[torch.Tensor],
                attn_mask: Optional[torch.Tensor] = None,
                packing=None) -> Dict[str, torch.Tensor]:
        if packing is not None:
            return self._forward_packed(tokens, attn_mask, packing)
        B, L = tokens.shape
        pos = torch.arange(L, device=tokens.device)
        x = self.tok_emb(tokens) + self.pos_emb(pos)[None, :, :]
        mask_bias = None
        if attn_mask is not None:
            mask_bias = torch.where(
                attn_mask, 0.0, -1e9
            ).to(torch.float32).contiguous()
        delta = None
        for blk in self.blocks:
            x, delta = blk(x, delta, mask_bias)
        if delta is None:
            x = self.ln_f(x)
        else:
            x, _ = ops.fused_add_layernorm(x, delta, self.ln_f.weight,
                                           self.ln_f.bias, self.ln_f.eps)
        pooled = ops.masked_mean_pool(x, attn_mask)
        return {name: head(pooled) for name, head in self.heads.items()}

    def _forward_packed(self, tokens, attn_mask, packing):
        if attn_mask is not None:
            raise ValueError("attn_mask and packing are mutually exclusive: "
                             "a packed batch carries its own padding segment")
        if tokens is None:
            tokens = packing.tokens
        R, L = tokens.shape
        x = self.tok_emb(tokens) + self.pos_emb(packing.pos)
        delta = None
        for blk in self.blocks:
            x, delta = blk(x, delta, None, packing.seg)
        if delta is None:
            x = self.ln_f(x)
        else:
            x, _ = ops.fused_add_layernorm(x, delta, self.ln_f.weight,
                                           self.ln_f.bias, self.ln_f.eps)
        pooled = ops.segment_mean_pool(x.reshape(R * L, -1), packing.seg_start,
                                       packing.seg_len, packing.pos2seg)
        return {name: head(pooled) for name, head in self.heads.items()}

    def set_pos_weights(self, weights: Dict[str, torch.Tensor]) -> None:
        for name, w in weights.items():
            self.register_buffer(f"_pw_{name}", w.float(), persistent=False)

    def set_loss_options(self, focal_gamma: Dict[str, float] = None,
                         label_smoothing: float = 0.0) -> None:
        self._focal_gamma = dict(focal_gamma or {})
        self._label_smoothing = float(label_smoothing)

    def loss(self, logits: Dict[str, torch.Tensor],
             labels: Dict[str, torch.Tensor]) -> torch.Tensor:
        total = None
        gammas = getattr(self, "_focal_gamma", {})
        smooth = getattr(self, "_label_smoothing", 0.0)
        for name, lg in logits.items():
            if name not in labels:
                continue
            lg = lg.float()
            if name in MULTILABEL_HEADS:
                pw = getattr(self, f"_pw_{name}", None)
                y = labels[name].float()
                if smooth > 0:
                    y = y * (1.0 - smooth) + 0.5 * smooth
                gamma = gammas.get(name, 0.0)
                if gamma > 0:
                    bce = F.binary_cross_entropy_with_logits(
                        lg, y, pos_weight=pw, reduction="none")
                    p = torch.sigmoid(lg)
                    p_t = p * y + (1 - p) * (1 - y)
                    li = ((1 - p_t).clamp(min=1e-4) ** gamma * bce).mean()
                else:
                    li = F.binary_cross_entropy_with_logits(
                        lg, y, pos_weight=pw)
            else:
                li = F.cross_entropy(lg, labels[name],
                                     label_smoothing=smooth)
            total = li if total is None else total + li
        assert total is not None, "no labels matched any head"
        return total


def build_model(name_or_cfg, dtype=torch.bfloat16) -> MLTC:
    cfg = CONFIGS[name_or_cfg] if isinstance(name_or_cfg, str) else name_or_cfg
    model = MLTC(cfg)
    return model.to(dtype)
```

tosem2021_amd/ops/__init__.py:

```python
from __future__ import annotations

from typing import Optional

import torch

from . import reference

_EXT = None
_EXT_ERR: Optional[str] = None


def hip_ops():
    global _EXT, _EXT_ERR
    if _EXT is None:
        try:
            from tosem2021_amd import _hip_ops

            _EXT = _hip_ops
        except ImportError as e:
            _EXT_ERR = str(e)
            raise RuntimeError(
                "tosem2021_amd._hip_ops is not built. On a GPU box this is a "
                "hard error (no eager fallback). Build it in-tree with: "
                "PYTORCH_ROCM_ARCH=gfx950 python setup.py build_ext --inplace "
                f"(import error: {e})"
            ) from e
    return _EXT


def hip_available() -> bool:
    try:
        hip_ops()
        return True
    except RuntimeError:
        return False


class _LayerNormFn(torch.autograd.Function):
    @staticmethod
    def forward(ctx, x, gamma, beta, eps):
        if x.is_cuda:
            y, _, mean, rstd = hip_ops().layernorm_fwd(x, None, gamma, beta, eps)
        else:
            y, mean, rstd = reference.layernorm_fwd(x, gamma, beta, eps)
        ctx.save_for_backward(x, gamma, mean, rstd)
        return y

    @staticmethod
    def backward(ctx, dy):
        x, gamma, mean, rstd = ctx.saved_tensors
        dy = dy.contiguous()
        if x.is_cuda:
            dx, dgamma, dbeta = hip_ops().layernorm_bwd(dy, x, gamma, mean,
                                                        rstd, None)
        else:
            dx, dgamma, dbeta = reference.layernorm_bwd(dy, x, gamma, mean, rstd)
        return dx, dgamma.to(gamma.dtype), dbeta.to(gamma.dtype), None


def fused_layernorm(x, gamma, beta, eps: float = 1e-5):
    return _LayerNormFn.apply(x.contiguous(), gamma, beta, eps)


class _AddLayerNormFn(torch.autograd.Function):

    @staticmethod
    def forward(ctx, x, residual, gamma, beta, eps):
        if x.is_cuda:
            y, s, mean, rstd = hip_ops().layernorm_fwd(x, residual, gamma,
                                                       beta, eps)
        else:
            y, s, mean, rstd = reference.add_layernorm_fwd(x, residual, gamma,
                                                           beta, eps)
        ctx.save_for_backward(s, gamma, mean, rstd)
        return y, s

    @staticmethod
    def backward(ctx, dy, ds):
        s, gamma, mean, rstd = ctx.saved_tensors
        dy = dy.contiguous()
        if s.is_cuda:
            de = ds.contiguous() if ds is not None else None
            dx, dgamma, dbeta = hip_ops().layernorm_bwd(dy, s, gamma, mean,
                                                        rstd, de)
        else:
            dx, dgamma, dbeta = reference.layernorm_bwd(dy, s, gamma, mean, rstd)
            if ds is not None:
                dx = dx + ds
        return dx, dx, dgamma.to(gamma.dtype), dbeta.to(gamma.dtype), None


def fused_add_layernorm(x, residual, gamma, beta, eps: float = 1e-5):
    return _AddLayerNormFn.apply(x.contiguous(), residual.contiguous(),
                                 gamma, beta, eps)


class _BiasGeluFn(torch.autograd.Function):
    @staticmethod
    def forward(ctx, x, b):
        ctx.save_for_backward(x, b)
        if x.is_cuda:
            return hip_ops().bias_gelu_fwd(x, b)
        return reference.bias_gelu_fwd(x, b)

    @staticmethod
    def backward(ctx, dy):
        x, b = ctx.saved_tensors
        dy = dy.contiguous()
        if x.is_cuda:
            dx, dbias = hip_ops().bias_gelu_bwd(dy, x, b)
        else:
            dx, dbias = reference.bias_gelu_bwd(dy, x, b)
        return dx, dbias.to(b.dtype)


def fused_bias_gelu(x, b):
    return _BiasGeluFn.apply(x.contiguous(), b)


class _SoftmaxFn(torch.autograd.Function):
    @staticmethod
    def forward(ctx, scores, mask, scale):
        if scores.is_cuda:
            p = hip_ops().softmax_fwd(scores, mask, scale)
        else:
            p = reference.softmax_fwd(scores, mask, scale)
        ctx.save_for_backward(p)
        ctx.scale = scale
        return p

    @staticmethod
    def backward(ctx, dp):
        (p,) = ctx.saved_tensors
        dp = dp.contiguous()
        if p.is_cuda:
            ds = hip_ops().softmax_bwd(dp, p, ctx.scale)
        else:
            ds = reference.softmax_bwd(dp, p, ctx.scale)
        return ds, None, None


def fused_softmax(scores, mask=None, scale: float = 1.0):
    return _SoftmaxFn.apply(scores.contiguous(), mask, scale)


class _QkvRepackFn(torch.autograd.Function):

    @staticmethod
    def forward(ctx, qkv, n_heads):
        ctx.n_heads = n_heads
        if qkv.is_cuda:
            stacked = hip_ops().qkv_repack(qkv, n_heads, False)
        else:
            B, L, _ = qkv.shape
            dh = qkv.shape[-1] // (3 * n_heads)
            stacked = (qkv.view(B, L, 3, n_heads, dh).permute(2, 0, 3, 1, 4)
                       .contiguous())
        q, k, v = stacked.unbind(0)
        return q, k, v

    @staticmethod
    def backward(ctx, dq, dk, dv):
        dq = dq.contiguous(); dk = dk.contiguous(); dv = dv.contiguous()
        if dq.is_cuda:
            return hip_ops().qkv_repack_bwd3(dq, dk, dv), None
        B, H, L, dh = dq.shape
        g = torch.stack([dq, dk, dv], dim=0)
        return g.permute(1, 3, 0, 2, 4).reshape(B, L, 3 * H * dh), None


def qkv_repack(qkv, n_heads: int):
    return _QkvRepackFn.apply(qkv.contiguous(), n_heads)


class _OutRepackFn(torch.autograd.Function):

    @staticmethod
    def forward(ctx, x):
        ctx.n_heads = x.shape[1]
        if x.is_cuda:
            return hip_ops().out_repack(x, False)
        B, H, L, dh = x.shape
        return x.permute(0, 2, 1, 3).reshape(B, L, H * dh)

    @staticmethod
    def backward(ctx, g):
        g = g.contiguous()
        if g.is_cuda:
            return hip_ops().out_repack_bwd(g, ctx.n_heads)
        B, L, D = g.shape
        H = ctx.n_heads
        return g.view(B, L, H, D // H).permute(0, 2, 1, 3).contiguous()


def out_repack(x):
    return _OutRepackFn.apply(x.contiguous())


class _LinearFn(torch.autograd.Function):

    @staticmethod
    def forward(ctx, x, w, b):
        ctx.save_for_backward(x, w)
        return torch.addmm(b, x, w.t())

    @staticmethod
    def backward(ctx, dy):
        x, w = ctx.saved_tensors
        dy = dy.contiguous()
        dx = torch.matmul(dy, w)
        dw = torch.matmul(dy.transpose(0, 1), x)
        db = hip_ops().bias_grad(dy) if dy.is_cuda else dy.sum(0)
        return dx, dw, db


def fused_linear(x, w, b):
    lead = x.shape[:-1]
    y = _LinearFn.apply(x.reshape(-1, x.shape[-1]).contiguous(), w, b)
    return y.view(*lead, -1)


class _LinearWgradFn(torch.autograd.Function):

    @staticmethod
    def forward(ctx, x, w, b):
        ctx.save_for_backward(x, w)
        ctx.has_bias = b is not None
        if b is None:
            return torch.matmul(x, w.t())
        return torch.addmm(b, x, w.t())

    @staticmethod
    def backward(ctx, dy):
        x, w = ctx.saved_tensors
        dy = dy.contiguous()
        dx = torch.matmul(dy, w)
        dw = hip_ops().wgrad_gemm(dy, x, 0)
        db = hip_ops().bias_grad(dy) if ctx.has_bias else None
        return dx, dw, db


def wgrad_linear_supported(out_features: int, in_features: int,
                           tokens: int) -> bool:
    return out_features % 256 == 0 and in_features % 256 == 0 and \
        tokens % 32 == 0


def wgrad_linear(x, w, b=None):
    lead = x.shape[:-1]
    y = _LinearWgradFn.apply(x.reshape(-1, x.shape[-1]).contiguous(), w, b)
    return y.view(*lead, -1)


def lt_linear_gelu_bias(x, w1, b1):
    return hip_ops().lt_linear_gelu_bias(x, w1, b1)


class _FlashAttentionFn(torch.autograd.Function):

    @staticmethod
    def forward(ctx, q, k, v, mask, scale, seg=None):
        if q.is_cuda:
            o, lse = hip_ops().flash_fwd(q, k, v, mask, scale, seg)
        else:
            bias = reference.segment_bias(seg) if seg is not None else None
            o, lse = reference.flash_attention_fwd(q, k, v, mask, scale, bias)
        ctx.save_for_backward(q, k, v, o, lse)
        ctx.mask = mask
        ctx.seg = seg
        ctx.scale = scale
        return o

    @staticmethod
    def backward(ctx, do):
        q, k, v, o, lse = ctx.saved_tensors
        mask, seg, scale = ctx.mask, ctx.seg, ctx.scale
        do = do.contiguous()
        if q.is_cuda:
            ddot = hip_ops().fa_dot(do, o)
            dk, dv = hip_ops().flash_bwd_fused(q, k, v, do, mask, lse,
                                               ddot, scale, False, seg)
            dq = hip_ops().flash_dq_recompute(q, k, v, do, mask, lse,
                                              ddot, scale, seg)
            return dq, dk, dv, None, None, None
        bias = reference.segment_bias(seg) if seg is not None else None
        s = torch.matmul(q, k.transpose(-1, -2))
        p = reference.p_from_lse(s, mask, lse, scale, bias)
        dp = torch.matmul(do, v.transpose(-1, -2))
        dsc = reference.softmax_bwd(dp, p, scale)
        dq = torch.matmul(dsc, k)
        dk = torch.matmul(dsc.transpose(-1, -2), q)
        dv = torch.matmul(p.transpose(-1, -2), do)
        return dq, dk, dv, None, None, None


def _check_mask_seg(mask, seg):
    if mask is not None and seg is not None:
        raise ValueError("mask and seg are mutually exclusive: a packed "
                         "batch marks its padding as a trailing segment")


def check_segments(seg: torch.Tensor) -> None:
    if seg.dim() != 2 or seg.dtype not in (torch.int32, torch.int64):
        raise ValueError("seg must be an integer [B, L] tensor")
    if seg.shape[1] > 1:
        bad = (seg[:, 1:] < seg[:, :-1]).any(dim=1)
        if bool(bad.any()):
            rows = torch.nonzero(bad).flatten().tolist()
            raise ValueError(f"seg rows {rows} are not non-decreasing")


def flash_attention(q, k, v, mask=None, scale: float = 1.0, seg=None):
    _check_mask_seg(mask, seg)
    return _FlashAttentionFn.apply(q.contiguous(), k.contiguous(),
                                   v.contiguous(), mask, scale, seg)


class _FlashAttentionPackedFn(torch.autograd.Function):

    @staticmethod
    def forward(ctx, qkv, n_heads, mask, scale, seg=None):
        if qkv.is_cuda:
            o, lse = hip_ops().flash_fwd_packed(qkv, n_heads, mask, scale,
                                                seg)
        else:
            B, L, D3 = qkv.shape
            d = D3 // 3
            q, k, v = (t.view(B, L, n_heads, 64).transpose(1, 2).contiguous()
                       for t in qkv.split(d, dim=-1))
            bias = reference.segment_bias(seg) if seg is not None else None
            o4, lse = reference.flash_attention_fwd(q, k, v, mask, scale,
                                                    bias)
            o = o4.transpose(1, 2).reshape(B, L, d)
        ctx.save_for_backward(qkv, o, lse)
        ctx.n_heads = n_heads
        ctx.mask = mask
        ctx.seg = seg
        ctx.scale = scale
        return o

    @staticmethod
    def backward(ctx, do):
        qkv, o, lse = ctx.saved_tensors
        n_heads, mask, scale = ctx.n_heads, ctx.mask, ctx.scale
        seg = ctx.seg
        do = do.contiguous()
        if qkv.is_cuda:
            dqkv = hip_ops().flash_bwd_packed(qkv, o, do, mask, lse,
                                              n_heads, scale, seg)
            return dqkv, None, None, None, None
        bias = reference.segment_bias(seg) if seg is not None else None
        B, L, D3 = qkv.shape
        d = D3 // 3
        q, k, v = (t.view(B, L, n_heads, 64).transpose(1, 2).contiguous()
                   for t in qkv.split(d, dim=-1))
        do4 = do.view(B, L, n_heads, 64).transpose(1, 2).contiguous()
        s = torch.matmul(q, k.transpose(-1, -2))
        p = reference.p_from_lse(s, mask, lse, scale, bias)
        dp = torch.matmul(do4, v.transpose(-1, -2))
        dsc = reference.softmax_bwd(dp, p, scale)
        dq = torch.matmul(dsc, k)
        dk = torch.matmul(dsc.transpose(-1, -2), q)
        dv = torch.matmul(p.transpose(-1, -2), do4)
        dqkv = torch.cat(
            [t.transpose(1, 2).reshape(B, L, d) for t in (dq, dk, dv)],
            dim=-1)
        return dqkv, None, None, None, None


def flash_attention_packed(qkv, n_heads: int, mask=None, scale: float = 1.0,
                           seg=None):
    _check_mask_seg(mask, seg)
    return _FlashAttentionPackedFn.apply(qkv.contiguous(), n_heads, mask,
                                         scale, seg)


def flash_supported(head_dim: int, L: int) -> bool:
    return head_dim == 64 and L % 32 == 0


class _MaskedPoolFn(torch.autograd.Function):
    @staticmethod
    def forward(ctx, x, mask):
        if x.is_cuda:
            pooled, counts = hip_ops().masked_pool_fwd(x, mask)
        else:
            if mask is not None:
                w = mask.to(x.dtype).unsqueeze(-1)
                counts = mask.sum(-1).clamp(min=1).float()
                pooled = ((x.float() * w.float()).sum(1) /
                          counts.unsqueeze(-1)).to(x.dtype)
            else:
                counts = torch.full((x.shape[0],), x.shape[1],
                                    dtype=torch.float32)
                pooled = x.float().mean(1).to(x.dtype)
        ctx.save_for_backward(counts)
        ctx.mask = mask
        ctx.L = x.shape[1]
        return pooled

    @staticmethod
    def backward(ctx, dpooled):
        (counts,) = ctx.saved_tensors
        mask = ctx.mask
        dpooled = dpooled.contiguous()
        if dpooled.is_cuda:
            dx = hip_ops().masked_pool_bwd(dpooled, mask, counts, ctx.L)
        else:
            g = (dpooled.float() / counts.unsqueeze(-1)).unsqueeze(1)
            dx = g.expand(-1, ctx.L, -1)
            if mask is not None:
                dx = dx * mask.unsqueeze(-1).float()
            dx = dx.to(dpooled.dtype)
        return dx, None


def masked_mean_pool(x, mask=None):
    return _MaskedPoolFn.apply(x.contiguous(),
                               mask.contiguous() if mask is not None else None)


class _SegmentPoolFn(torch.autograd.Function):
    @staticmethod
    def forward(ctx, x, seg_start, seg_len, pos2seg):
        if x.is_cuda:
            pooled = hip_ops().segment_pool_fwd(x, seg_start, seg_len)
        else:
            pooled = reference.segment_pool_fwd(x, seg_start, seg_len,
                                                pos2seg)
        ctx.save_for_backward(seg_len, pos2seg)
        return pooled

    @staticmethod
    def backward(ctx, dpooled):
        seg_len, pos2seg = ctx.saved_tensors
        dpooled = dpooled.contiguous()
        if dpooled.is_cuda:
            dx = hip_ops().segment_pool_bwd(dpooled, pos2seg, seg_len,
                                            pos2seg.shape[0])
        else:
            dx = reference.segment_pool_bwd(dpooled, seg_len, pos2seg)
        return dx, None, None, None


def segment_mean_pool(x, seg_start, seg_len, pos2seg):
    return _SegmentPoolFn.apply(x.contiguous(), seg_start, seg_len, pos2seg)


def adamw_step(p, grad, m, v, master, *, lr, beta1=0.9, beta2=0.999, eps=1e-8,
               wd=0.01, step, grad_scale=1.0):
    if p.is_cuda:
        hip_ops().adamw_step(p, grad, m, v, master, lr, beta1, beta2, eps, wd,
                             step, grad_scale)
    else:
        reference.adamw_step(p, grad, m, v, master, lr, beta1, beta2, eps, wd,
                             step, grad_scale)


def grad_clip_state(grad, *, grad_scale=1.0, max_norm):
    if not max_norm > 0:
        raise ValueError(f"max_norm must be greater than 0, got {max_norm}")
    if grad.is_cuda:
        return hip_ops().grad_clip_state(grad, grad_scale, max_norm)
    return reference.grad_clip_state(grad, grad_scale, max_norm)


def adamw_step_clipped(p, grad, m, v, master, *, lr, beta1=0.9, beta2=0.999,
                       eps=1e-8, wd=0.01, step, clip_state):
    if p.is_cuda:
        hip_ops().adamw_step_clipped(p, grad, m, v, master, lr, beta1, beta2,
                                     eps, wd, step, clip_state)
    else:
        reference.adamw_step_clipped(p, grad, m, v, master, lr, beta1, beta2,
                                     eps, wd, step, clip_state)
```

tosem2021_amd/ops/reference.py:

```python
from __future__ import annotations

import math
from typing import Optional, Tuple

import torch


def layernorm_fwd(
    x: torch.Tensor, gamma: torch.Tensor, beta: torch.Tensor, eps: float
) -> Tuple[torch.Tensor, torch.Tensor, torch.Tensor]:
    xf = x.float()
    mean = xf.mean(dim=-1)
    var = xf.var(dim=-1, unbiased=False)
    rstd = torch.rsqrt(var + eps)
    xhat = (xf - mean.unsqueeze(-1)) * rstd.unsqueeze(-1)
    y = xhat * gamma.float() + beta.float()
    return y.to(x.dtype), mean.reshape(-1), rstd.reshape(-1)


def add_layernorm_fwd(x, residual, gamma, beta, eps):
    s = (x.float() + residual.float()).to(x.dtype)
    y, mean, rstd = layernorm_fwd(s, gamma, beta, eps)
    return y, s, mean, rstd


def layernorm_bwd(
    dy: torch.Tensor,
    x: torch.Tensor,
    gamma: torch.Tensor,
    mean: torch.Tensor,
    rstd: torch.Tensor,
) -> Tuple[torch.Tensor, torch.Tensor, torch.Tensor]:
    D = x.shape[-1]
    xf = x.float().reshape(-1, D)
    dyf = dy.float().reshape(-1, D)
    mean = mean.reshape(-1, 1)
    rstd = rstd.reshape(-1, 1)
    xhat = (xf - mean) * rstd
    dyg = dyf * gamma.float()
    c1 = dyg.mean(dim=-1, keepdim=True)
    c2 = (dyg * xhat).mean(dim=-1, keepdim=True)
    dx = rstd * (dyg - c1 - xhat * c2)
    dgamma = (dyf * xhat).sum(dim=0)
    dbeta = dyf.sum(dim=0)
    return dx.reshape(x.shape).to(x.dtype), dgamma, dbeta


def bias_gelu_fwd(x: torch.Tensor, b: torch.Tensor) -> torch.Tensor:
    pre = x.float() + b.float()
    return torch.nn.functional.gelu(pre, approximate="tanh").to(x.dtype)


def bias_gelu_bwd(
    dy: torch.Tensor, x: torch.Tensor, b: torch.Tensor
) -> Tuple[torch.Tensor, torch.Tensor]:
    pre = (x.float() + b.float()).requires_grad_(True)
    with torch.enable_grad():
        y = torch.nn.functional.gelu(pre, approximate="tanh")
    (dpre,) = torch.autograd.grad(y, pre, dy.float())
    dbias = dpre.reshape(-1, x.shape[-1]).sum(dim=0)
    return dpre.to(x.dtype), dbias


def softmax_fwd(
    scores: torch.Tensor, mask: Optional[torch.Tensor], scale: float
) -> torch.Tensor:
    s = scores.float() * scale
    if mask is not None:
        s = s + mask.float().view(mask.shape[0], 1, 1, mask.shape[-1])
    return torch.softmax(s, dim=-1).to(scores.dtype)


def softmax_bwd(dp: torch.Tensor, p: torch.Tensor, scale: float) -> torch.Tensor:
    dpf = dp.float()
    pf = p.float()
    dot = (dpf * pf).sum(dim=-1, keepdim=True)
    return (scale * pf * (dpf - dot)).to(p.dtype)


def segment_bias(seg: torch.Tensor) -> torch.Tensor:
    same = seg.unsqueeze(-1) == seg.unsqueeze(-2)
    zero = torch.zeros((), dtype=torch.float32, device=seg.device)
    return torch.where(same, zero, zero - 1e9).unsqueeze(1)


def flash_attention_fwd(q, k, v, mask, scale, bias=None):
    s = torch.matmul(q.float(), k.float().transpose(-1, -2)) * scale
    if mask is not None:
        s = s + mask.float().view(mask.shape[0], 1, 1, -1)
    if bias is not None:
        s = s + bias
    lse = torch.logsumexp(s, dim=-1)
    p = torch.softmax(s, dim=-1)
    o = torch.matmul(p, v.float())
    return o.to(q.dtype), lse


def p_from_lse(scores, mask, lse, scale, bias=None):
    s = scores.float() * scale
    if mask is not None:
        s = s + mask.float().view(mask.shape[0], 1, 1, -1)
    if bias is not None:
        s = s + bias
    return torch.exp(s - lse.unsqueeze(-1)).to(scores.dtype)


def segment_pool_fwd(x, seg_start, seg_len, pos2seg):
    n = seg_len.shape[0]
    valid = pos2seg >= 0
    acc = torch.zeros(n, x.shape[-1], dtype=torch.float32, device=x.device)
    acc.index_add_(0, pos2seg[valid].long(), x[valid].float())
    return (acc / seg_len.clamp(min=1).float().unsqueeze(-1)).to(x.dtype)


def segment_pool_bwd(dpooled, seg_len, pos2seg):
    valid = pos2seg >= 0
    idx = pos2seg.clamp(min=0).long()
    g = dpooled.float() / seg_len.clamp(min=1).float().unsqueeze(-1)
    dx = g[idx] * valid.unsqueeze(-1).float()
    return dx.to(dpooled.dtype)


def adamw_step(
    p: torch.Tensor,
    grad: torch.Tensor,
    m: torch.Tensor,
    v: torch.Tensor,
    master: torch.Tensor,
    lr: float,
    beta1: float,
    beta2: float,
    eps: float,
    wd: float,
    step: int,
    grad_scale: float = 1.0,
) -> None:
    g = grad.float() * grad_scale
    m.mul_(beta1).add_(g, alpha=1 - beta1)
    v.mul_(beta2).addcmul_(g, g, value=1 - beta2)
    bc1 = 1.0 / (1.0 - beta1**step)
    bc2 = 1.0 / (1.0 - beta2**step)
    mhat = m * bc1
    vhat = v * bc2
    master.add_(-(lr * (mhat / (vhat.sqrt() + eps) + wd * master)))
    p.copy_(master.to(p.dtype))


def grad_clip_state(grad: torch.Tensor, grad_scale: float,
                    max_norm: float) -> torch.Tensor:
    f32 = torch.float32
    sumsq64 = grad.detach().double().pow(2).sum().cpu()
    sumsq = sumsq64.to(f32)
    gs = torch.tensor(grad_scale, dtype=f32)
    norm = (gs.double() * sumsq64.sqrt()).to(f32)
    ratio = torch.tensor(max_norm, dtype=f32) / (norm + 1e-6)
    one = torch.ones((), dtype=f32)
    coef = torch.where(ratio < 1, ratio, one)
    finite = torch.isfinite(sumsq).to(f32)
    return torch.stack([norm, gs * coef, finite, sumsq]).to(grad.device)


def adamw_step_clipped(p, grad, m, v, master, lr, beta1, beta2, eps, wd,
                       step, clip_state) -> None:
    if float(clip_state[2]) == 0.0:
        return
    adamw_step(p, grad, m, v, master, lr, beta1, beta2, eps, wd, step,
               grad_scale=float(clip_state[1]))
```

Measured before the change: 795,800 tokens/s.

## Fold bias-gradient column sums into attention and layernorm backward kernels

Adds optional epilogues to the fused flash-attention backward kernels (dK/dV and dQ recompute) and the layernorm backward kernels. They accumulate per-column sums of the bf16 gradients they already write and store per-block partials to a workspace, so the QKV bias and down-projection bias gradients come out without separate reduction passes over the activations. Layernorm backward also merges per-wave dgamma/dbeta partials in shared memory before writing, which shrinks the workspace. The model gains a fold mode that routes these biases through the fused ops. The cost is extra shared-memory syncs, more template variants and an extra workspace reduction.

```diff
diff --git a/csrc/flash_attn.hip b/csrc/flash_attn.hip
--- a/csrc/flash_attn.hip
+++ b/csrc/flash_attn.hip
@@ -160,6 +160,24 @@
   return {bid / n_qblocks, qA, qA + FA_QWG};
 }
 
+__device__ __forceinline__ float fa_half_merge(float s) {
+  return s + __shfl_xor(s, 32, WAVE);
+}
+
+__device__ __forceinline__ void fa_colsum_merge_store(const float* cs, int tid,
+                                                      float* dst0,
+                                                      float* dst1) {
+  if (tid < 2 * FA_DH) {
+    const int slot = tid / FA_DH, c = tid % FA_DH;
+    const float* p = cs + slot * FA_WAVES * FA_DH + c;
+    float s = p[0];
+#pragma unroll
+    for (int w = 1; w < FA_WAVES; ++w) s += p[w * FA_DH];
+    float* dst = slot ? dst1 : dst0;
+    if (dst) dst[c] = s;
+  }
+}
+
 __device__ __forceinline__ int fa_last_active_kv(const float* mrow, int L,
                                                  int tid, int* scratch) {
   if (tid == 0) *scratch = -1;
@@ -438,7 +456,7 @@
 
 
 
-template <bool SEG>
+template <bool SEG, bool BIAS>
 __global__ void __launch_bounds__(FA_BLOCK, 2)
 flash_bwd_fused_kernel(const short* __restrict__ q, const short* __restrict__ k,
                        const short* __restrict__ v,
@@ -449,7 +467,8 @@
                        const float* __restrict__ ddot,
                        short* __restrict__ ds, short* __restrict__ dk,
                        short* __restrict__ dv,
-                       int B, int H, int L, float scale, FaGeom g) {
+                       int B, int H, int L, float scale, FaGeom g,
+                       float* __restrict__ bias_ws, int bias_ld) {
   extern __shared__ __attribute__((aligned(16))) char smem[];
   short* q_lds = (short*)smem;
   short* do_lds = (short*)(smem + TILE_LDS_BYTES);
@@ -599,6 +618,7 @@
   }
   }
 
+  float csk[2] = {0.f, 0.f}, csv[2] = {0.f, 0.f};
 #pragma unroll
   for (int t = 0; t < 2; ++t) {
 #pragma unroll
@@ -606,9 +626,32 @@
       int kvl = c_row(r, half);
       if (kv_base + kvl >= L) continue;
       long off = qkv_off + (long)(kv_base + kvl) * g.qkv_rs + 32 * t + col;
-      dv[off] = f32_to_bf16(dv_acc[t][r]);
-      dk[off] = f32_to_bf16(dk_acc[t][r]);
-    }
+      const short vb = f32_to_bf16(dv_acc[t][r]);
+      const short kb16 = f32_to_bf16(dk_acc[t][r]);
+      dv[off] = vb;
+      dk[off] = kb16;
+      if constexpr (BIAS) {
+        csv[t] += bf16_to_f32(vb);
+        csk[t] += bf16_to_f32(kb16);
+      }
+    }
+  }
+  if constexpr (BIAS) {
+    float* cs = (float*)smem;
+    __syncthreads();
+#pragma unroll
+    for (int t = 0; t < 2; ++t) {
+      float sk_ = fa_half_merge(csk[t]);
+      float sv_ = fa_half_merge(csv[t]);
+      if (half == 0) {
+        cs[(0 * FA_WAVES + wid) * FA_DH + 32 * t + col] = sk_;
+        cs[(1 * FA_WAVES + wid) * FA_DH + 32 * t + col] = sv_;
+      }
+    }
+    __syncthreads();
+    const int third = bias_ld / 3;
+    float* row = bias_ws + ((long)b * n_kvblocks + kb) * bias_ld + h * FA_DH;
+    fa_colsum_merge_store(cs, tid, row + third, row + 2 * third);
   }
 }
 
@@ -617,19 +660,32 @@
                                   const void* mask, const void* seg,
                                   const void* lse, const void* ddot, void* ds,
                                   short* dk, short* dv, int B, int H, int L,
-                                  float scale, FaGeom g, hipStream_t stream) {
+                                  float scale, FaGeom g, float* bias_ws,
+                                  hipStream_t stream) {
   const dim3 grid = fa_grid(B, H, L, FA_QWG);
-  if (seg)
-    flash_bwd_fused_kernel<true><<<grid, FA_BLOCK, BWD_SEG_LDS_BYTES,
-                                   stream>>>(
-        q, k, v, (const short*)dout, nullptr, (const int*)seg,
-        (const float*)lse, (const float*)ddot, nullptr, dk, dv, B, H, L,
-        scale, g);
-  else
-    flash_bwd_fused_kernel<false><<<grid, FA_BLOCK, BWD_LDS_BYTES, stream>>>(
-        q, k, v, (const short*)dout, (const float*)mask, nullptr,
-        (const float*)lse, (const float*)ddot, (short*)ds, dk, dv, B, H, L,
-        scale, g);
+  const int bias_ld = 3 * H * FA_DH;
+#define FA_BWD_SEG_ARGS                                                       \
+  q, k, v, (const short*)dout, nullptr, (const int*)seg, (const float*)lse,   \
+      (const float*)ddot, nullptr, dk, dv, B, H, L, scale, g, bias_ws, bias_ld
+#define FA_BWD_ARGS                                                           \
+  q, k, v, (const short*)dout, (const float*)mask, nullptr,                   \
+      (const float*)lse, (const float*)ddot, (short*)ds, dk, dv, B, H, L,     \
+      scale, g, bias_ws, bias_ld
+  if (seg && bias_ws) {
+    flash_bwd_fused_kernel<true, true><<<grid, FA_BLOCK, BWD_SEG_LDS_BYTES,
+                                         stream>>>(FA_BWD_SEG_ARGS);
+  } else if (seg) {
+    flash_bwd_fused_kernel<true, false><<<grid, FA_BLOCK, BWD_SEG_LDS_BYTES,
+                                          stream>>>(FA_BWD_SEG_ARGS);
+  } else if (bias_ws) {
+    flash_bwd_fused_kernel<false, true><<<grid, FA_BLOCK, BWD_LDS_BYTES,
+                                          stream>>>(FA_BWD_ARGS);
+  } else {
+    flash_bwd_fused_kernel<false, false><<<grid, FA_BLOCK, BWD_LDS_BYTES,
+                                           stream>>>(FA_BWD_ARGS);
+  }
+#undef FA_BWD_ARGS
+#undef FA_BWD_SEG_ARGS
 }
 
 extern "C" hipError_t flash_bwd_fused_launch(
@@ -641,19 +697,20 @@
   fa_bwd_fused_dispatch((const short*)q, (const short*)k, (const short*)v,
                         dout, mask, seg, lse, ddot, ds, (short*)dk,
                         (short*)dv, B, H, L, scale, FaGeom::bhld(H, L),
-                        stream);
+                        nullptr, stream);
   return hipGetLastError();
 }
 
 extern "C" hipError_t flash_bwd_fused_packed_launch(
     const void* qkv, const void* dout, const void* mask, const void* seg,
-    const void* lse, const void* ddot, void* dqkv, int B, int H, int L,
-    float scale, hipStream_t stream) {
+    const void* lse, const void* ddot, void* dqkv, void* bias_ws, int B,
+    int H, int L, float scale, hipStream_t stream) {
   const int D = H * FA_DH;
   fa_bwd_fused_dispatch((const short*)qkv, (const short*)qkv + D,
                         (const short*)qkv + 2 * D, dout, mask, seg, lse, ddot,
                         nullptr, (short*)dqkv + D, (short*)dqkv + 2 * D, B, H,
-                        L, scale, FaGeom::packed(H, L), stream);
+                        L, scale, FaGeom::packed(H, L), (float*)bias_ws,
+                        stream);
   return hipGetLastError();
 }
 
@@ -737,7 +794,7 @@
   return hipGetLastError();
 }
 
-template <bool SEG>
+template <bool SEG, bool BIAS>
 __global__ void __launch_bounds__(FA_BLOCK, 2)
 flash_dq_recompute_kernel(const short* __restrict__ q,
                           const short* __restrict__ k,
@@ -748,7 +805,8 @@
                           const float* __restrict__ lse,
                           const float* __restrict__ ddot,
                           short* __restrict__ dq,
-                          int B, int H, int L, float scale, FaGeom g) {
+                          int B, int H, int L, float scale, FaGeom g,
+                          float* __restrict__ bias_ws, int bias_ld) {
   extern __shared__ __attribute__((aligned(16))) char smem[];
   short* k_lds = (short*)smem;
   short* v_lds = (short*)(smem + TILE_LDS_BYTES);
@@ -890,19 +948,43 @@
     __builtin_amdgcn_s_setprio(0);
   }
 
+  float csA[2] = {0.f, 0.f}, csB[2] = {0.f, 0.f};
 #pragma unroll
   for (int t = 0; t < 2; ++t) {
 #pragma unroll
     for (int r = 0; r < 16; ++r) {
       int rloc = c_row(r, half);
       int qA = qb.qA + rloc, qB = qb.qB + rloc;
-      if (qA < L)
-        dq[qkv_off + (long)qA * g.qkv_rs + 32 * t + col] =
-            f32_to_bf16(dqA[t][r]);
-      if (qB < L)
-        dq[qkv_off + (long)qB * g.qkv_rs + 32 * t + col] =
-            f32_to_bf16(dqB[t][r]);
-    }
+      if (qA < L) {
+        const short a16 = f32_to_bf16(dqA[t][r]);
+        dq[qkv_off + (long)qA * g.qkv_rs + 32 * t + col] = a16;
+        if constexpr (BIAS) csA[t] += bf16_to_f32(a16);
+      }
+      if (qB < L) {
+        const short b16 = f32_to_bf16(dqB[t][r]);
+        dq[qkv_off + (long)qB * g.qkv_rs + 32 * t + col] = b16;
+        if constexpr (BIAS) csB[t] += bf16_to_f32(b16);
+      }
+    }
+  }
+  if constexpr (BIAS) {
+    float* cs = (float*)smem;
+    __syncthreads();
+#pragma unroll
+    for (int t = 0; t < 2; ++t) {
+      float sA_ = fa_half_merge(csA[t]);
+      float sB_ = fa_half_merge(csB[t]);
+      if (half == 0) {
+        cs[(0 * FA_WAVES + wid) * FA_DH + 32 * t + col] = sA_;
+        cs[(1 * FA_WAVES + wid) * FA_DH + 32 * t + col] = sB_;
+      }
+    }
+    __syncthreads();
+    const int n128 = (L + FA_QWG - 1) / FA_QWG;
+    const int blkA = (qb.qA - wid * FA_QB) / FA_QWG;
+    float* row = bias_ws + ((long)b * n128 + blkA) * bias_ld + h * FA_DH;
+    fa_colsum_merge_store(cs, tid, row,
+                          blkA + 1 < n128 ? row + bias_ld : nullptr);
   }
 }
 
@@ -911,19 +993,32 @@
                                      const void* mask, const void* seg,
                                      const void* lse, const void* ddot,
                                      void* dq, int B, int H, int L,
-                                     float scale, FaGeom g,
+                                     float scale, FaGeom g, float* bias_ws,
                                      hipStream_t stream) {
   const dim3 grid = fa_grid(B, H, L, FA_Q2WG);
-  if (seg)
-    flash_dq_recompute_kernel<true><<<grid, FA_BLOCK, DQR_LDS_BYTES,
-                                      stream>>>(
-        q, k, v, (const short*)dout, nullptr, (const int*)seg,
-        (const float*)lse, (const float*)ddot, (short*)dq, B, H, L, scale, g);
-  else
-    flash_dq_recompute_kernel<false><<<grid, FA_BLOCK, DQR_LDS_BYTES,
-                                       stream>>>(
-        q, k, v, (const short*)dout, (const float*)mask, nullptr,
-        (const float*)lse, (const float*)ddot, (short*)dq, B, H, L, scale, g);
+  const int bias_ld = 3 * H * FA_DH;
+#define FA_DQR_SEG_ARGS                                                       \
+  q, k, v, (const short*)dout, nullptr, (const int*)seg, (const float*)lse,   \
+      (const float*)ddot, (short*)dq, B, H, L, scale, g, bias_ws, bias_ld
+#define FA_DQR_ARGS                                                           \
+  q, k, v, (const short*)dout, (const float*)mask, nullptr,                   \
+      (const float*)lse, (const float*)ddot, (short*)dq, B, H, L, scale, g,   \
+      bias_ws, bias_ld
+  if (seg && bias_ws) {
+    flash_dq_recompute_kernel<true, true><<<grid, FA_BLOCK, DQR_LDS_BYTES,
+                                            stream>>>(FA_DQR_SEG_ARGS);
+  } else if (seg) {
+    flash_dq_recompute_kernel<true, false><<<grid, FA_BLOCK, DQR_LDS_BYTES,
+                                             stream>>>(FA_DQR_SEG_ARGS);
+  } else if (bias_ws) {
+    flash_dq_recompute_kernel<false, true><<<grid, FA_BLOCK, DQR_LDS_BYTES,
+                                             stream>>>(FA_DQR_ARGS);
+  } else {
+    flash_dq_recompute_kernel<false, false><<<grid, FA_BLOCK, DQR_LDS_BYTES,
+                                              stream>>>(FA_DQR_ARGS);
+  }
+#undef FA_DQR_ARGS
+#undef FA_DQR_SEG_ARGS
 }
 
 extern "C" hipError_t flash_dq_recompute_launch(
@@ -932,19 +1027,19 @@
     void* dq, int B, int H, int L, float scale, hipStream_t stream) {
   fa_dq_recompute_dispatch((const short*)q, (const short*)k, (const short*)v,
                            dout, mask, seg, lse, ddot, dq, B, H, L, scale,
-                           FaGeom::bhld(H, L), stream);
+                           FaGeom::bhld(H, L), nullptr, stream);
   return hipGetLastError();
 }
 
 extern "C" hipError_t flash_dq_recompute_packed_launch(
     const void* qkv, const void* dout, const void* mask, const void* seg,
-    const void* lse, const void* ddot, void* dqkv, int B, int H, int L,
-    float scale, hipStream_t stream) {
+    const void* lse, const void* ddot, void* dqkv, void* bias_ws, int B,
+    int H, int L, float scale, hipStream_t stream) {
   const int D = H * FA_DH;
   fa_dq_recompute_dispatch((const short*)qkv, (const short*)qkv + D,
                            (const short*)qkv + 2 * D, dout, mask, seg, lse,
                            ddot, dqkv, B, H, L, scale, FaGeom::packed(H, L),
-                           stream);
+                           (float*)bias_ws, stream);
   return hipGetLastError();
 }
 
diff --git a/csrc/layernorm.hip b/csrc/layernorm.hip
--- a/csrc/layernorm.hip
+++ b/csrc/layernorm.hip
@@ -212,14 +212,45 @@
   }
 }
 
-template <int PKTS, bool HASDE>
+template <int PKTS, int NOUT>
+__device__ __forceinline__ void ln_bwd_merge_store(
+    const float (&acc)[NOUT][PKTS * 8], float* __restrict__ sm,
+    float* __restrict__ ws, int lane, int wid) {
+  constexpr int DT = PKTS * WAVE * 8;
+  for (int w = 0; w < WAVES_PER_BLOCK; ++w) {
+    if (wid == w) {
+#pragma unroll
+      for (int o = 0; o < NOUT; ++o) {
+#pragma unroll
+        for (int p = 0; p < PKTS; ++p) {
+          float4_t* s4 = (float4_t*)(sm + o * DT + (p * WAVE + lane) * 8);
+          float4_t a = {0.f, 0.f, 0.f, 0.f}, b = {0.f, 0.f, 0.f, 0.f};
+          if (w) { a = s4[0]; b = s4[1]; }
+#pragma unroll
+          for (int j = 0; j < 4; ++j) {
+            a[j] += acc[o][p * 8 + j];
+            b[j] += acc[o][p * 8 + 4 + j];
+          }
+          s4[0] = a; s4[1] = b;
+        }
+      }
+    }
+    __syncthreads();
+  }
+  float* orow = ws + (long)blockIdx.x * (NOUT * DT);
+  for (int i = threadIdx.x * 4; i < NOUT * DT; i += BLOCK * 4)
+    *(float4_t*)(orow + i) = *(const float4_t*)(sm + i);
+}
+
+template <int PKTS, bool HASDE, bool DRES>
 __global__ void __launch_bounds__(BLOCK)
 ln_bwd_t(const short* __restrict__ dy, const short* __restrict__ x,
          const short* __restrict__ gamma, const float* __restrict__ mean_in,
          const float* __restrict__ rstd_in,
          const short* __restrict__ ds_extra, short* __restrict__ dx,
-         float* __restrict__ ws_dgamma, float* __restrict__ ws_dbeta,
-         int N, int D) {
+         float* __restrict__ ws, int N, int D) {
+  constexpr int NOUT = DRES ? 3 : 2;
+  __shared__ __attribute__((aligned(16))) float sm[NOUT * PKTS * WAVE * 8];
   const int lane = threadIdx.x & (WAVE - 1);
   const int wid = threadIdx.x / WAVE;
   float gv[PKTS * 8];
@@ -229,7 +260,7 @@
 #pragma unroll
     for (int j = 0; j < 8; ++j) gv[p * 8 + j] = bf16_to_f32(g8[j]);
   }
-  float dg_acc[PKTS * 8] = {0.f}, db_acc[PKTS * 8] = {0.f};
+  float acc[NOUT][PKTS * 8] = {{0.f}};
   const int rstride = gridDim.x * WAVES_PER_BLOCK;
   int row = blockIdx.x * WAVES_PER_BLOCK + wid;
   const bool active = row < N;
@@ -258,8 +289,8 @@
         float g = d * gv[k];
         if (HASDE) ev[k] = bf16_to_f32(ve[p][j]);
         xh[k] = h; dyg[k] = g;
-        dg_acc[k] += d * h;
-        db_acc[k] += d;
+        acc[0][k] += d * h;
+        acc[1][k] += d;
         s1 += g; s2 += g * h;
       }
     }
@@ -283,34 +314,25 @@
         float d_ = rstd * (dyg[k] - s1 - xh[k] * s2);
         if (HASDE) d_ += ev[k];
         o[j] = f32_to_bf16(d_);
+        if (DRES) acc[NOUT - 1][k] += bf16_to_f32(o[j]);
       }
       *(short8_t*)(dx + (long)row * D + (p * WAVE + lane) * 8) = o;
     }
     if (next >= N) break;
     row = next;
   }
-  float* og = ws_dgamma +
-              (long)(blockIdx.x * WAVES_PER_BLOCK + wid) * D;
-  float* ob = ws_dbeta + (long)(blockIdx.x * WAVES_PER_BLOCK + wid) * D;
-#pragma unroll
-  for (int p = 0; p < PKTS; ++p) {
-    int base = (p * WAVE + lane) * 8;
-#pragma unroll
-    for (int j = 0; j < 8; ++j) {
-      og[base + j] = dg_acc[p * 8 + j];
-      ob[base + j] = db_acc[p * 8 + j];
-    }
-  }
-}
-
-template <int PKTS, bool HASDE>
+  ln_bwd_merge_store<PKTS, NOUT>(acc, sm, ws, lane, wid);
+}
+
+template <int PKTS, bool HASDE, bool DRES>
 __global__ void __launch_bounds__(BLOCK)
 ln_bwd_t2(const short* __restrict__ dy, const short* __restrict__ x,
           const short* __restrict__ gamma, const float* __restrict__ mean_in,
           const float* __restrict__ rstd_in,
           const short* __restrict__ ds_extra, short* __restrict__ dx,
-          float* __restrict__ ws_dgamma, float* __restrict__ ws_dbeta,
-          int N, int D) {
+          float* __restrict__ ws, int N, int D) {
+  constexpr int NOUT = DRES ? 3 : 2;
+  __shared__ __attribute__((aligned(16))) float sm[NOUT * PKTS * WAVE * 8];
   const int lane = threadIdx.x & (WAVE - 1);
   const int wid = threadIdx.x / WAVE;
   float gv[PKTS * 8];
@@ -320,7 +342,7 @@
 #pragma unroll
     for (int j = 0; j < 8; ++j) gv[p * 8 + j] = bf16_to_f32(g8[j]);
   }
-  float dg_acc[PKTS * 8] = {0.f}, db_acc[PKTS * 8] = {0.f};
+  float acc[NOUT][PKTS * 8] = {{0.f}};
   const int rstride = gridDim.x * WAVES_PER_BLOCK * 2;
   int rowA = (blockIdx.x * WAVES_PER_BLOCK + wid) * 2;
   short8_t vdA[PKTS], vxA[PKTS], veA[PKTS];
@@ -358,16 +380,16 @@
         float hA = (bf16_to_f32(vxA[p][j]) - meanA) * rstdA;
         float gA = dA * gv[k];
         xhA[k] = hA; dygA[k] = gA;
-        dg_acc[k] += dA * hA;
-        db_acc[k] += dA;
+        acc[0][k] += dA * hA;
+        acc[1][k] += dA;
         s1A += gA; s2A += gA * hA;
         if (actB) {
           float dB = bf16_to_f32(vdB[p][j]);
           float hB = (bf16_to_f32(vxB[p][j]) - meanB) * rstdB;
           float gB = dB * gv[k];
           xhB[k] = hB; dygB[k] = gB;
-          dg_acc[k] += dB * hB;
-          db_acc[k] += dB;
+          acc[0][k] += dB * hB;
+          acc[1][k] += dB;
           s1B += gB; s2B += gB * hB;
         }
       }
@@ -399,10 +421,12 @@
         float dA_ = rstdA * (dygA[k] - s1A - xhA[k] * s2A);
         if (HASDE) dA_ += bf16_to_f32(veA[p][j]);
         oA[j] = f32_to_bf16(dA_);
+        if (DRES) acc[NOUT - 1][k] += bf16_to_f32(oA[j]);
         if (actB) {
           float dB_ = rstdB * (dygB[k] - s1B - xhB[k] * s2B);
           if (HASDE) dB_ += bf16_to_f32(veB[p][j]);
           oB[j] = f32_to_bf16(dB_);
+          if (DRES) acc[NOUT - 1][k] += bf16_to_f32(oB[j]);
         }
       }
       int base = (p * WAVE + lane) * 8;
@@ -422,34 +446,22 @@
       }
     }
   }
-  float* og = ws_dgamma + (long)(blockIdx.x * WAVES_PER_BLOCK + wid) * D;
-  float* ob = ws_dbeta + (long)(blockIdx.x * WAVES_PER_BLOCK + wid) * D;
-#pragma unroll
-  for (int p = 0; p < PKTS; ++p) {
-    int base = (p * WAVE + lane) * 8;
-#pragma unroll
-    for (int j = 0; j < 8; ++j) {
-      og[base + j] = dg_acc[p * 8 + j];
-      ob[base + j] = db_acc[p * 8 + j];
-    }
-  }
-}
-
-template <int MAXP>
+  ln_bwd_merge_store<PKTS, NOUT>(acc, sm, ws, lane, wid);
+}
+
+template <int MAXP, bool DRES>
 __global__ void __launch_bounds__(BLOCK)
 ln_bwd_g(const short* __restrict__ dy, const short* __restrict__ x,
          const short* __restrict__ gamma, const float* __restrict__ mean_in,
          const float* __restrict__ rstd_in,
          const short* __restrict__ ds_extra,
-         short* __restrict__ dx,
-         float* __restrict__ ws_dgamma, float* __restrict__ ws_dbeta,
-         int N, int D) {
+         short* __restrict__ dx, float* __restrict__ ws, int N, int D) {
+  constexpr int NOUT = DRES ? 3 : 2;
   const int lane = threadIdx.x & (WAVE - 1);
   const int wid = threadIdx.x / WAVE;
   extern __shared__ __attribute__((aligned(16))) char smem[];
-  float* sg = (float*)smem;
-  float* sb = sg + D;
-  float dg_acc[MAXP * 8] = {0.f}, db_acc[MAXP * 8] = {0.f};
+  float* sm = (float*)smem;
+  float acc[NOUT][MAXP * 8] = {{0.f}};
   for (int row = blockIdx.x * WAVES_PER_BLOCK + wid; row < N;
        row += gridDim.x * WAVES_PER_BLOCK) {
     const short* dyr = dy + (long)row * D;
@@ -471,8 +483,8 @@
         float d = bf16_to_f32(vd[p][j]);
         float h = (bf16_to_f32(vx[p][j]) - mean) * rstd;
         float g = d * bf16_to_f32(vg[p][j]);
-        dg_acc[p * 8 + j] += d * h;
-        db_acc[p * 8 + j] += d;
+        acc[0][p * 8 + j] += d * h;
+        acc[1][p * 8 + j] += d;
         s1 += g; s2 += g * h;
       }
     }
@@ -492,6 +504,7 @@
         float d_ = rstd * (g - s1 - h * s2);
         if (der) d_ += bf16_to_f32(ev[j]);
         o[j] = f32_to_bf16(d_);
+        if (DRES) acc[NOUT - 1][p * 8 + j] += bf16_to_f32(o[j]);
       }
       *(short8_t*)(dxr + base) = o;
     }
@@ -499,40 +512,48 @@
   for (int w = 0; w < WAVES_PER_BLOCK; ++w) {
     if (wid == w) {
 #pragma unroll
-      for (int p = 0; p < MAXP; ++p) {
-        int base = (p * WAVE + lane) * 8;
-        if (base >= D) continue;
-#pragma unroll
-        for (int j = 0; j < 8; ++j) {
-          float pg = w ? sg[base + j] : 0.f, pb = w ? sb[base + j] : 0.f;
-          sg[base + j] = pg + dg_acc[p * 8 + j];
-          sb[base + j] = pb + db_acc[p * 8 + j];
+      for (int o = 0; o < NOUT; ++o) {
+#pragma unroll
+        for (int p = 0; p < MAXP; ++p) {
+          int base = (p * WAVE + lane) * 8;
+          if (base >= D) continue;
+          float* so = sm + o * D;
+#pragma unroll
+          for (int j = 0; j < 8; ++j) {
+            float prev = w ? so[base + j] : 0.f;
+            so[base + j] = prev + acc[o][p * 8 + j];
+          }
         }
       }
     }
     __syncthreads();
   }
-  float* og = ws_dgamma + (long)blockIdx.x * D;
-  float* ob = ws_dbeta + (long)blockIdx.x * D;
-  for (int i = threadIdx.x; i < D; i += BLOCK) { og[i] = sg[i]; ob[i] = sb[i]; }
+  float* orow = ws + (long)blockIdx.x * (NOUT * D);
+  for (int i = threadIdx.x; i < NOUT * D; i += BLOCK) orow[i] = sm[i];
 }
 
 #define LN_BWD_G_MAX_D 4096
+template <bool DRES>
 __global__ void __launch_bounds__(BLOCK)
 ln_bwd_wide_kernel(const short* __restrict__ dy, const short* __restrict__ x,
                    const short* __restrict__ gamma,
                    const float* __restrict__ mean_in,
                    const float* __restrict__ rstd_in,
                    const short* __restrict__ ds_extra,
-                   short* __restrict__ dx, float* __restrict__ ws_dgamma,
-                   float* __restrict__ ws_dbeta, int N, int D) {
+                   short* __restrict__ dx, float* __restrict__ ws, int N,
+                   int D) {
+  constexpr int NOUT = DRES ? 3 : 2;
   const int lane = threadIdx.x & (WAVE - 1);
   const int wid = threadIdx.x / WAVE;
-  float* og = ws_dgamma + (long)(blockIdx.x * WAVES_PER_BLOCK + wid) * D;
-  float* ob = ws_dbeta + (long)(blockIdx.x * WAVES_PER_BLOCK + wid) * D;
+  float* og = ws + (long)(blockIdx.x * WAVES_PER_BLOCK + wid) * (NOUT * D);
+  float* ob = og + D;
+  float* od = og + (NOUT - 1) * D;
   for (int i = lane * 8; i < D; i += WAVE * 8) {
 #pragma unroll
-    for (int j = 0; j < 8; ++j) { og[i + j] = 0.f; ob[i + j] = 0.f; }
+    for (int j = 0; j < 8; ++j) {
+      og[i + j] = 0.f; ob[i + j] = 0.f;
+      if (DRES) od[i + j] = 0.f;
+    }
   }
   for (int row = blockIdx.x * WAVES_PER_BLOCK + wid; row < N;
        row += gridDim.x * WAVES_PER_BLOCK) {
@@ -572,6 +593,7 @@
         o[j] = f32_to_bf16(d_);
         og[i + j] += d * h;
         ob[i + j] += d;
+        if (DRES) od[i + j] += bf16_to_f32(o[j]);
       }
       *(short8_t*)(dxr + i) = o;
     }
@@ -594,6 +616,23 @@
     for (int j = 0; j < 4; ++j) s[j] += v[j];
   }
   *(float4_t*)(out + (long)blockIdx.y * D + col) = s;
+}
+
+__global__ void __launch_bounds__(256)
+colsum_stage_bf16_kernel(const float* __restrict__ ws, short* __restrict__ out,
+                         int R, int D) {
+  int col = (blockIdx.x * 256 + threadIdx.x) * 4;
+  if (col >= D) return;
+  float4_t s = {0.f, 0.f, 0.f, 0.f};
+  for (int r = 0; r < R; ++r) {
+    float4_t v = *(const float4_t*)(ws + (long)r * D + col);
+#pragma unroll
+    for (int j = 0; j < 4; ++j) s[j] += v[j];
+  }
+  short4_t o;
+#pragma unroll
+  for (int j = 0; j < 4; ++j) o[j] = f32_to_bf16(s[j]);
+  *(short4_t*)(out + col) = o;
 }
 
 __global__ void __launch_bounds__(256)
@@ -692,74 +731,84 @@
 
 hipError_t ln_bwd_launch(const void* dy, const void* x, const void* gamma,
                          const void* mean, const void* rstd,
-                         const void* ds_extra, void* dx,
-                         void* ws_dgamma, void* ws_dbeta, int N, int D,
-                         int grid, hipStream_t stream) {
-  size_t shm = (size_t)D * 2 * sizeof(float);
+                         const void* ds_extra, void* dx, void* ws, int n_out,
+                         int N, int D, int grid, hipStream_t stream) {
+  if (n_out != 2 && n_out != 3) return hipErrorInvalidValue;
+  const bool dres = n_out == 3;
+  size_t shm = (size_t)D * n_out * sizeof(float);
+#define LNB_ARGS                                                              \
+  (const short*)dy, (const short*)x, (const short*)gamma, (const float*)mean, \
+      (const float*)rstd, (const short*)ds_extra, (short*)dx, (float*)ws, N, D
+#define LNB_K(K, P)                                                           \
+  do {                                                                        \
+    if (ds_extra && dres) {                                                   \
+      K<P, true, true><<<grid, BLOCK, 0, stream>>>(LNB_ARGS);                 \
+    } else if (ds_extra) {                                                    \
+      K<P, true, false><<<grid, BLOCK, 0, stream>>>(LNB_ARGS);                \
+    } else if (dres) {                                                        \
+      K<P, false, true><<<grid, BLOCK, 0, stream>>>(LNB_ARGS);                \
+    } else {                                                                  \
+      K<P, false, false><<<grid, BLOCK, 0, stream>>>(LNB_ARGS);               \
+    }                                                                         \
+  } while (0)
 #define LNB_T(P)                                                              \
   do {                                                                        \
     if (ln_bwd_use_1row()) {                                                  \
-      if (ds_extra)                                                           \
-        ln_bwd_t<P, true><<<grid, BLOCK, 0, stream>>>(                        \
-            (const short*)dy, (const short*)x, (const short*)gamma,           \
-            (const float*)mean, (const float*)rstd, (const short*)ds_extra,   \
-            (short*)dx, (float*)ws_dgamma, (float*)ws_dbeta, N, D);           \
-      else                                                                    \
-        ln_bwd_t<P, false><<<grid, BLOCK, 0, stream>>>(                       \
-            (const short*)dy, (const short*)x, (const short*)gamma,           \
-            (const float*)mean, (const float*)rstd, nullptr, (short*)dx,      \
-            (float*)ws_dgamma, (float*)ws_dbeta, N, D);                       \
-      break;                                                                  \
+      LNB_K(ln_bwd_t, P);                                                     \
+    } else {                                                                  \
+      LNB_K(ln_bwd_t2, P);                                                    \
     }                                                                         \
-    if (ds_extra)                                                             \
-      ln_bwd_t2<P, true><<<grid, BLOCK, 0, stream>>>(                         \
-          (const short*)dy, (const short*)x, (const short*)gamma,             \
-          (const float*)mean, (const float*)rstd, (const short*)ds_extra,     \
-          (short*)dx, (float*)ws_dgamma, (float*)ws_dbeta, N, D);             \
-    else                                                                      \
-      ln_bwd_t2<P, false><<<grid, BLOCK, 0, stream>>>(                        \
-          (const short*)dy, (const short*)x, (const short*)gamma,             \
-          (const float*)mean, (const float*)rstd, nullptr, (short*)dx,        \
-          (float*)ws_dgamma, (float*)ws_dbeta, N, D);                         \
   } while (0)
 #define LNB_G(P)                                                              \
-  ln_bwd_g<P><<<grid, BLOCK, shm, stream>>>(                                  \
-      (const short*)dy, (const short*)x, (const short*)gamma,                 \
-      (const float*)mean, (const float*)rstd, (const short*)ds_extra,         \
-      (short*)dx, (float*)ws_dgamma, (float*)ws_dbeta, N, D)
+  do {                                                                        \
+    if (dres) {                                                               \
+      ln_bwd_g<P, true><<<grid, BLOCK, shm, stream>>>(LNB_ARGS);              \
+    } else {                                                                  \
+      ln_bwd_g<P, false><<<grid, BLOCK, shm, stream>>>(LNB_ARGS);             \
+    }                                                                         \
+  } while (0)
   if (D == 512) LNB_T(1);
   else if (D == 1024) LNB_T(2);
   else if (D <= 512) LNB_G(1);
   else if (D <= 1024) LNB_G(2);
   else if (D <= 2048) LNB_G(4);
   else if (D <= LN_BWD_G_MAX_D) LNB_G(8);
-  else
-    ln_bwd_wide_kernel<<<grid, BLOCK, 0, stream>>>(
-        (const short*)dy, (const short*)x, (const short*)gamma,
-        (const float*)mean, (const float*)rstd, (const short*)ds_extra,
-        (short*)dx, (float*)ws_dgamma, (float*)ws_dbeta, N, D);
+  else if (dres) {
+    ln_bwd_wide_kernel<true><<<grid, BLOCK, 0, stream>>>(LNB_ARGS);
+  } else {
+    ln_bwd_wide_kernel<false><<<grid, BLOCK, 0, stream>>>(LNB_ARGS);
+  }
 #undef LNB_G
 #undef LNB_T
+#undef LNB_K
+#undef LNB_ARGS
   return hipGetLastError();
 }
 
 int ln_bwd_ws_rows(int D, int grid) {
-  const bool per_wave = D == 512 || D == 1024 || D > LN_BWD_G_MAX_D;
-  return per_wave ? grid * WAVES_PER_BLOCK : grid;
+  return D > LN_BWD_G_MAX_D ? grid * WAVES_PER_BLOCK : grid;
 }
 
 #define COLSUM_MAX_SPLITS 256
 #define COLSUM_MID 16
+static hipError_t colsum_final(const float* in, void* out, int R, int D,
+                               int out_bf16, hipStream_t stream) {
+  dim3 grid1((D / 4 + 255) / 256, 1);
+  if (out_bf16) {
+    colsum_stage_bf16_kernel<<<grid1, 256, 0, stream>>>(in, (short*)out, R, D);
+  } else {
+    colsum_stage_kernel<<<grid1, 256, 0, stream>>>(in, (float*)out, R, D, R);
+  }
+  return hipGetLastError();
+}
+
 hipError_t colsum_launch(const void* ws, void* scratch, void* out, int R,
-                         int D, hipStream_t stream) {
+                         int D, int split_w, int out_bf16,
+                         hipStream_t stream) {
   int gx = (D / 4 + 255) / 256;
-  dim3 grid1(gx, 1);
-  if (R <= COLSUM_MID) {
-    colsum_stage_kernel<<<grid1, 256, 0, stream>>>(
-        (const float*)ws, (float*)out, R, D, R);
-    return hipGetLastError();
-  }
-  int splits = 1024 / gx;
+  if (R <= COLSUM_MID)
+    return colsum_final((const float*)ws, out, R, D, out_bf16, stream);
+  int splits = 1024 / ((split_w / 4 + 255) / 256);
   if (splits > COLSUM_MAX_SPLITS) splits = COLSUM_MAX_SPLITS;
   if (splits > R) splits = R;
   int rows_per_split = (R + splits - 1) / splits;
@@ -767,20 +816,16 @@
       (const float*)ws, (float*)scratch, R, D, rows_per_split);
   hipError_t e = hipGetLastError();
   if (e != hipSuccess) return e;
-  if (splits <= COLSUM_MID) {
-    colsum_stage_kernel<<<grid1, 256, 0, stream>>>(
-        (const float*)scratch, (float*)out, splits, D, splits);
-    return hipGetLastError();
-  }
+  if (splits <= COLSUM_MID)
+    return colsum_final((const float*)scratch, out, splits, D, out_bf16,
+                        stream);
   float* mid = (float*)scratch + (long)COLSUM_MAX_SPLITS * D;
   int rps2 = (splits + COLSUM_MID - 1) / COLSUM_MID;
   colsum_stage_kernel<<<dim3(gx, COLSUM_MID), 256, 0, stream>>>(
       (const float*)scratch, mid, splits, D, rps2);
   e = hipGetLastError();
   if (e != hipSuccess) return e;
-  colsum_stage_kernel<<<grid1, 256, 0, stream>>>(
-      mid, (float*)out, COLSUM_MID, D, COLSUM_MID);
-  return hipGetLastError();
-}
-
-}
+  return colsum_final(mid, out, COLSUM_MID, D, out_bf16, stream);
+}
+
+}
diff --git a/csrc/ops.cpp b/csrc/ops.cpp
--- a/csrc/ops.cpp
+++ b/csrc/ops.cpp
@@ -10,10 +10,11 @@
                          void*, void*, void*, void*, int, int, float, int,
                          hipStream_t);
 hipError_t ln_bwd_launch(const void*, const void*, const void*, const void*,
-                         const void*, const void*, void*, void*, void*, int,
+                         const void*, const void*, void*, void*, int, int,
                          int, int, hipStream_t);
 int ln_bwd_ws_rows(int, int);
-hipError_t colsum_launch(const void*, void*, void*, int, int, hipStream_t);
+hipError_t colsum_launch(const void*, void*, void*, int, int, int, int,
+                         hipStream_t);
 hipError_t bias_gelu_fwd_launch(const void*, const void*, void*, long, int,
                                 int, hipStream_t);
 hipError_t bias_gelu_bwd_launch(const void*, const void*, const void*, void*,
@@ -55,11 +56,12 @@
 hipError_t flash_bwd_fused_packed_launch(const void*, const void*,
                                          const void*, const void*,
                                          const void*, const void*, void*,
-                                         int, int, int, float, hipStream_t);
+                                         void*, int, int, int, float,
+                                         hipStream_t);
 hipError_t flash_dq_recompute_packed_launch(const void*, const void*,
                                             const void*, const void*,
                                             const void*, const void*, void*,
-                                            int, int, int, float,
+                                            void*, int, int, int, float,
                                             hipStream_t);
 hipError_t flash_dq_recompute_launch(const void*, const void*, const void*,
                                      const void*, const void*, const void*,
@@ -226,17 +228,24 @@
 std::vector<torch::Tensor> layernorm_bwd(torch::Tensor dy, torch::Tensor x,
                                          torch::Tensor gamma, torch::Tensor mean,
                                          torch::Tensor rstd,
-                                         c10::optional<torch::Tensor> ds_extra) {
+                                         c10::optional<torch::Tensor> ds_extra,
+                                         bool want_dres, bool out_bf16) {
   check_bf16(dy, "dy"); check_bf16(x, "x"); check_bf16(gamma, "gamma");
   const int D = (int)x.size(-1);
   const long N = x.numel() / D;
   TORCH_CHECK(D % 8 == 0, "D must be a multiple of 8, got ", D);
+  TORCH_CHECK(dy.numel() == x.numel(), "dy shape mismatch");
+  TORCH_CHECK(gamma.numel() == D, "gamma must be [D]");
+  check_f32(mean, "mean"); check_f32(rstd, "rstd");
+  TORCH_CHECK(mean.numel() == N && rstd.numel() == N,
+              "mean and rstd must be [N]");
   auto dx = torch::empty_like(x);
   int grid = (int)std::min<long>((N + 3) / 4, D > 4096 ? 256 : 1024);
   long ws_rows = ln_bwd_ws_rows(D, grid);
+  const int n_out = want_dres ? 3 : 2;
+  const int W = n_out * D;
   auto opts = x.options().dtype(torch::kFloat32);
-  auto ws_dg = torch::empty({ws_rows, D}, opts);
-  auto ws_db = torch::empty({ws_rows, D}, opts);
+  auto ws = torch::empty({ws_rows, W}, opts);
   const void* de = nullptr;
   if (ds_extra.has_value()) {
     check_bf16(*ds_extra, "ds_extra");
@@ -245,16 +254,17 @@
   }
   CHECK_HIP(ln_bwd_launch(dy.data_ptr(), x.data_ptr(), gamma.data_ptr(),
                           mean.data_ptr(), rstd.data_ptr(), de, dx.data_ptr(),
-                          ws_dg.data_ptr(), ws_db.data_ptr(), (int)N, D, grid,
+                          ws.data_ptr(), n_out, (int)N, D, grid,
                           cur_stream()));
-  auto dgamma = torch::empty({D}, opts);
-  auto dbeta = torch::empty({D}, opts);
-  auto scratch = torch::empty({256 + 16, D}, opts);
-  CHECK_HIP(colsum_launch(ws_dg.data_ptr(), scratch.data_ptr(),
-                          dgamma.data_ptr(), (int)ws_rows, D, cur_stream()));
-  CHECK_HIP(colsum_launch(ws_db.data_ptr(), scratch.data_ptr(),
-                          dbeta.data_ptr(), (int)ws_rows, D, cur_stream()));
-  return {dx, dgamma, dbeta};
+  auto cols = torch::empty({W}, out_bf16 ? x.options() : opts);
+  auto scratch = torch::empty({256 + 16, W}, opts);
+  CHECK_HIP(colsum_launch(ws.data_ptr(), scratch.data_ptr(), cols.data_ptr(),
+                          (int)ws_rows, W, 2 * D, out_bf16 ? 1 : 0,
+                          cur_stream()));
+  std::vector<torch::Tensor> out = {dx, cols.narrow(0, 0, D),
+                                    cols.narrow(0, D, D)};
+  if (want_dres) out.push_back(cols.narrow(0, 2 * D, D));
+  return out;
 }
 
 torch::Tensor bias_gelu_fwd(torch::Tensor x, torch::Tensor b) {
@@ -272,7 +282,7 @@
 }
 
 std::vector<torch::Tensor> bias_gelu_bwd(torch::Tensor dy, torch::Tensor x,
-                                         torch::Tensor b) {
+                                         torch::Tensor b, bool out_bf16) {
   check_bf16(dy, "dy"); check_bf16(x, "x"); check_bf16(b, "b");
   const int D = (int)x.size(-1);
   const long n = x.numel();
@@ -286,11 +296,12 @@
   CHECK_HIP(bias_gelu_bwd_launch(dy.data_ptr(), x.data_ptr(), b.data_ptr(),
                                  dx.data_ptr(), ws.data_ptr(), n, D, grid,
                                  cur_stream()));
-  auto dbias = torch::empty({D}, x.options().dtype(torch::kFloat32));
+  auto dbias = torch::empty(
+      {D}, out_bf16 ? x.options() : x.options().dtype(torch::kFloat32));
   auto scratch = torch::empty({256 + 16, D},
                              x.options().dtype(torch::kFloat32));
   CHECK_HIP(colsum_launch(ws.data_ptr(), scratch.data_ptr(), dbias.data_ptr(),
-                          grid, D, cur_stream()));
+                          grid, D, D, out_bf16 ? 1 : 0, cur_stream()));
   return {dx, dbias};
 }
 
@@ -587,11 +598,12 @@
   return {o, lse};
 }
 
-torch::Tensor flash_bwd_packed(torch::Tensor qkv, torch::Tensor o,
-                               torch::Tensor dout,
-                               c10::optional<torch::Tensor> mask,
-                               torch::Tensor lse, long H, double scale,
-                               c10::optional<torch::Tensor> seg) {
+namespace {
+
+std::vector<torch::Tensor> flash_bwd_packed_impl(
+    torch::Tensor qkv, torch::Tensor o, torch::Tensor dout,
+    c10::optional<torch::Tensor> mask, torch::Tensor lse, long H,
+    double scale, c10::optional<torch::Tensor> seg, bool want_bias) {
   const auto dims = check_flash_packed(qkv, H, {{"o", o}, {"dout", dout}},
                                        {{"lse", lse}});
   const long B = dims.B, L = dims.L;
@@ -602,15 +614,47 @@
                                  ddot.data_ptr(), (int)B, (int)H, (int)L,
                                  cur_stream()));
   auto dqkv = torch::empty_like(qkv);
+  const auto f32 = qkv.options().dtype(torch::kFloat32);
+  const long W = 3 * H * 64;
+  const long ws_rows = B * ((L + 127) / 128);
+  torch::Tensor ws;
+  void* ws_ptr = nullptr;
+  if (want_bias) {
+    ws = torch::empty({ws_rows, W}, f32);
+    ws_ptr = ws.data_ptr();
+  }
   CHECK_HIP(flash_bwd_fused_packed_launch(
       qkv.data_ptr(), dout.data_ptr(), mptr, sptr, lse.data_ptr(),
-      ddot.data_ptr(), dqkv.data_ptr(), (int)B, (int)H, (int)L, (float)scale,
-      cur_stream()));
+      ddot.data_ptr(), dqkv.data_ptr(), ws_ptr, (int)B, (int)H, (int)L,
+      (float)scale, cur_stream()));
   CHECK_HIP(flash_dq_recompute_packed_launch(
       qkv.data_ptr(), dout.data_ptr(), mptr, sptr, lse.data_ptr(),
-      ddot.data_ptr(), dqkv.data_ptr(), (int)B, (int)H, (int)L, (float)scale,
-      cur_stream()));
-  return dqkv;
+      ddot.data_ptr(), dqkv.data_ptr(), ws_ptr, (int)B, (int)H, (int)L,
+      (float)scale, cur_stream()));
+  if (!want_bias) return {dqkv};
+  auto dbias = torch::empty({W}, qkv.options());
+  auto scratch = torch::empty({256 + 16, W}, f32);
+  CHECK_HIP(colsum_launch(ws.data_ptr(), scratch.data_ptr(), dbias.data_ptr(),
+                          (int)ws_rows, (int)W, (int)W, 1, cur_stream()));
+  return {dqkv, dbias};
+}
+
+}
+
+torch::Tensor flash_bwd_packed(torch::Tensor qkv, torch::Tensor o,
+                               torch::Tensor dout,
+                               c10::optional<torch::Tensor> mask,
+                               torch::Tensor lse, long H, double scale,
+                               c10::optional<torch::Tensor> seg) {
+  return flash_bwd_packed_impl(qkv, o, dout, mask, lse, H, scale, seg,
+                               false)[0];
+}
+
+std::vector<torch::Tensor> flash_bwd_packed_bias(
+    torch::Tensor qkv, torch::Tensor o, torch::Tensor dout,
+    c10::optional<torch::Tensor> mask, torch::Tensor lse, long H,
+    double scale, c10::optional<torch::Tensor> seg) {
+  return flash_bwd_packed_impl(qkv, o, dout, mask, lse, H, scale, seg, true);
 }
 
 torch::Tensor flash_dq_recompute(torch::Tensor q, torch::Tensor k,
@@ -761,6 +805,11 @@
         py::arg("qkv"), py::arg("o"), py::arg("dout"), py::arg("mask"),
         py::arg("lse"), py::arg("H"), py::arg("scale"),
         py::arg("seg") = py::none());
+  m.def("flash_bwd_packed_bias", &flash_bwd_packed_bias,
+        "flash_bwd_packed plus the column sum of dqkv (qkv bias grad, bf16)",
+        py::arg("qkv"), py::arg("o"), py::arg("dout"), py::arg("mask"),
+        py::arg("lse"), py::arg("H"), py::arg("scale"),
+        py::arg("seg") = py::none());
   m.def("fa_dot", &fa_dot, "rowsum(dO*O) per attention row");
   m.def("flash_dq", &flash_dq, "dQ = dS @ K (MFMA, tr_b16 K^T fragments)");
   m.def("bias_grad", &bias_grad, "bf16 column-sum for linear bias grads");
@@ -770,7 +819,10 @@
   m.def("out_repack", &out_repack, "attention output merge");
   m.def("out_repack_bwd", &out_repack_bwd, "attention output merge bwd");
   m.def("layernorm_fwd", &layernorm_fwd, "fused LayerNorm fwd (bf16, gfx950)");
-  m.def("layernorm_bwd", &layernorm_bwd, "fused LayerNorm bwd");
+  m.def("layernorm_bwd", &layernorm_bwd, "fused LayerNorm bwd",
+        py::arg("dy"), py::arg("x"), py::arg("gamma"), py::arg("mean"),
+        py::arg("rstd"), py::arg("ds_extra"), py::arg("want_dres") = false,
+        py::arg("out_bf16") = false);
   m.def("bias_gelu_fwd", &bias_gelu_fwd, "fused bias+GeLU fwd");
   m.def("lt_linear_gelu_bias", &lt_linear_gelu_bias,
         "hipBLASLt GEMM with fused GELU_BIAS epilogue (inference)");
@@ -778,7 +830,9 @@
         "time the heuristic's top algos for a bf16 GEMM config");
   m.def("lt_probe_epilogue", &lt_probe_epilogue,
         "does this hipBLASLt have kernels for (m, n, k, epilogue)?");
-  m.def("bias_gelu_bwd", &bias_gelu_bwd, "fused bias+GeLU bwd");
+  m.def("bias_gelu_bwd", &bias_gelu_bwd, "fused bias+GeLU bwd",
+        py::arg("dy"), py::arg("x"), py::arg("b"),
+        py::arg("out_bf16") = false);
   m.def("softmax_fwd", &softmax_fwd, "fused scaled masked softmax fwd");
   m.def("softmax_bwd", &softmax_bwd, "fused softmax bwd");
   m.def("adamw_step", &adamw_step, "fused AdamW over flat params");
diff --git a/tosem2021_amd/models/classifier.py b/tosem2021_amd/models/classifier.py
--- a/tosem2021_amd/models/classifier.py
+++ b/tosem2021_amd/models/classifier.py
@@ -67,7 +67,13 @@
 _USE_WGRAD = os.environ.get("TOSEM_WGRAD", "0") == "1"
 
 
-def _linear(mod: nn.Linear, x: torch.Tensor) -> torch.Tensor:
+_FOLD_BIAS_GRAD = os.environ.get("TOSEM_FOLD_BIAS_GRAD", "0") == "1"
+
+
+def _linear(mod: nn.Linear, x: torch.Tensor,
+            fold_bias: bool = False) -> torch.Tensor:
+    if fold_bias:
+        return F.linear(x, mod.weight, mod.bias.detach())
     if x.is_cuda and torch.is_grad_enabled():
         if _USE_WGRAD and ops.wgrad_linear_supported(
                 mod.out_features, mod.in_features,
@@ -89,12 +95,13 @@
         self.proj = nn.Linear(cfg.d_model, cfg.d_model, bias=True)
 
     def forward(self, x, mask_bias: Optional[torch.Tensor],
-                seg: Optional[torch.Tensor] = None):
+                seg: Optional[torch.Tensor] = None, fold_bias: bool = False):
         B, L, D = x.shape
         if ops.flash_supported(self.head_dim, L):
-            out = ops.flash_attention_packed(_linear(self.qkv, x), self.n_heads,
-                                             mask_bias, self.scale, seg)
-            return _linear(self.proj, out)
+            out = ops.flash_attention_packed(
+                _linear(self.qkv, x, fold_bias), self.n_heads, mask_bias,
+                self.scale, seg, self.qkv.bias if fold_bias else None)
+            return _linear(self.proj, out, fold_bias)
         if seg is not None:
             if x.is_cuda:
                 raise RuntimeError(
@@ -105,12 +112,12 @@
             s = torch.matmul(q, k.transpose(-1, -2)).float() * self.scale
             p = torch.softmax(s + ops.reference.segment_bias(seg), dim=-1)
             out = torch.matmul(p.to(v.dtype), v)
-            return self.proj(ops.out_repack(out))
+            return _linear(self.proj, ops.out_repack(out), fold_bias)
         q, k, v = ops.qkv_repack(self.qkv(x), self.n_heads)
         scores = torch.matmul(q, k.transpose(-1, -2))
         p = ops.fused_softmax(scores, mask_bias, self.scale)
         out = torch.matmul(p, v)
-        return self.proj(ops.out_repack(out))
+        return _linear(self.proj, ops.out_repack(out), fold_bias)
 
 
 class FFN(nn.Module):
@@ -121,7 +128,7 @@
         self.up_bias = nn.Parameter(torch.zeros(cfg.d_ff))
         self.down = nn.Linear(cfg.d_ff, cfg.d_model, bias=True)
 
-    def forward(self, x):
+    def forward(self, x, fold_bias: bool = False):
         if x.is_cuda and not torch.is_grad_enabled():
             B, L, D = x.shape
             a = ops.lt_linear_gelu_bias(x.reshape(-1, D).contiguous(),
@@ -129,7 +136,7 @@
             return self.down(a.view(B, L, -1))
         h = _linear(self.up, x)
         h = ops.fused_bias_gelu(h, self.up_bias)
-        return _linear(self.down, h)
+        return _linear(self.down, h, fold_bias)
 
 
 class EncoderBlock(nn.Module):
@@ -145,25 +152,34 @@
     def _drop(self, h):
         return F.dropout(h, self.dropout, self.training) if self.dropout else h
 
-    def forward(self, x, delta, mask_bias, seg=None):
+    def fold_ok(self) -> bool:
+        return not (self.dropout and self.training)
+
+    def forward(self, x, delta, mask_bias, seg=None, delta_bias=None,
+                fold_bias: bool = False):
         if delta is None:
             y1 = ops.fused_layernorm(x, self.ln1.weight, self.ln1.bias,
                                      self.ln1.eps)
             s1 = x
         else:
             y1, s1 = ops.fused_add_layernorm(x, delta, self.ln1.weight,
-                                             self.ln1.bias, self.ln1.eps)
-        h = self._drop(self.attn(y1, mask_bias, seg))
-        y2, s2 = ops.fused_add_layernorm(s1, h, self.ln2.weight,
-                                         self.ln2.bias, self.ln2.eps)
-        h2 = self._drop(self.ffn(y2))
+                                             self.ln1.bias, self.ln1.eps,
+                                             delta_bias)
+        fold_bias = fold_bias and self.fold_ok()
+        h = self._drop(self.attn(y1, mask_bias, seg, fold_bias))
+        y2, s2 = ops.fused_add_layernorm(
+            s1, h, self.ln2.weight, self.ln2.bias, self.ln2.eps,
+            self.attn.proj.bias if fold_bias else None)
+        h2 = self._drop(self.ffn(y2, fold_bias))
         return s2, h2
 
 
 class MLTC(nn.Module):
-    def __init__(self, cfg: MLTCConfig):
+    def __init__(self, cfg: MLTCConfig,
+                 fold_bias_grad: Optional[bool] = None):
         super().__init__()
         self.cfg = cfg
+        self.fold_bias_grad = fold_bias_grad
         self.tok_emb = nn.Embedding(cfg.vocab_size, cfg.d_model)
         self.pos_emb = nn.Embedding(cfg.max_seq, cfg.d_model)
         self.blocks = nn.ModuleList(EncoderBlock(cfg) for _ in range(cfg.n_layers))
@@ -179,6 +195,28 @@
             nn.init.normal_(m.weight, std=0.02)
             if isinstance(m, nn.Linear) and m.bias is not None:
                 nn.init.zeros_(m.bias)
+
+    def _fold_active(self, x: torch.Tensor) -> bool:
+        if self.fold_bias_grad is None:
+            on = _FOLD_BIAS_GRAD and x.is_cuda
+        else:
+            on = self.fold_bias_grad
+        return (on and torch.is_grad_enabled()
+                and not (self.cfg.dropout and self.training)
+                and not _USE_FUSED_LINEAR and not _USE_WGRAD)
+
+    def _run_blocks(self, x, mask_bias, seg):
+        fold = self._fold_active(x)
+        delta = delta_bias = None
+        for blk in self.blocks:
+            x, delta = blk(x, delta, mask_bias, seg, delta_bias, fold)
+            delta_bias = blk.ffn.down.bias if fold and blk.fold_ok() else None
+        if delta is None:
+            return self.ln_f(x)
+        x, _ = ops.fused_add_layernorm(x, delta, self.ln_f.weight,
+                                       self.ln_f.bias, self.ln_f.eps,
+                                       delta_bias)
+        return x
 
     def forward(self, tokens: Optional[torch.Tensor],
                 attn_mask: Optional[torch.Tensor] = None,
@@ -193,14 +231,7 @@
             mask_bias = torch.where(
                 attn_mask, 0.0, -1e9
             ).to(torch.float32).contiguous()
-        delta = None
-        for blk in self.blocks:
-            x, delta = blk(x, delta, mask_bias)
-        if delta is None:
-            x = self.ln_f(x)
-        else:
-            x, _ = ops.fused_add_layernorm(x, delta, self.ln_f.weight,
-                                           self.ln_f.bias, self.ln_f.eps)
+        x = self._run_blocks(x, mask_bias, None)
         pooled = ops.masked_mean_pool(x, attn_mask)
         return {name: head(pooled) for name, head in self.heads.items()}
 
@@ -212,14 +243,7 @@
             tokens = packing.tokens
         R, L = tokens.shape
         x = self.tok_emb(tokens) + self.pos_emb(packing.pos)
-        delta = None
-        for blk in self.blocks:
-            x, delta = blk(x, delta, None, packing.seg)
-        if delta is None:
-            x = self.ln_f(x)
-        else:
-            x, _ = ops.fused_add_layernorm(x, delta, self.ln_f.weight,
-                                           self.ln_f.bias, self.ln_f.eps)
+        x = self._run_blocks(x, None, packing.seg)
         pooled = ops.segment_mean_pool(x.reshape(R * L, -1), packing.seg_start,
                                        packing.seg_len, packing.pos2seg)
         return {name: head(pooled) for name, head in self.heads.items()}
@@ -265,7 +289,8 @@
         return total
 
 
-def build_model(name_or_cfg, dtype=torch.bfloat16) -> MLTC:
+def build_model(name_or_cfg, dtype=torch.bfloat16,
+                fold_bias_grad: Optional[bool] = None) -> MLTC:
     cfg = CONFIGS[name_or_cfg] if isinstance(name_or_cfg, str) else name_or_cfg
-    model = MLTC(cfg)
+    model = MLTC(cfg, fold_bias_grad)
     return model.to(dtype)
diff --git a/tosem2021_amd/ops/__init__.py b/tosem2021_amd/ops/__init__.py
--- a/tosem2021_amd/ops/__init__.py
+++ b/tosem2021_amd/ops/__init__.py
@@ -51,10 +51,10 @@
         x, gamma, mean, rstd = ctx.saved_tensors
         dy = dy.contiguous()
         if x.is_cuda:
-            dx, dgamma, dbeta = hip_ops().layernorm_bwd(dy, x, gamma, mean,
-                                                        rstd, None)
-        else:
-            dx, dgamma, dbeta = reference.layernorm_bwd(dy, x, gamma, mean, rstd)
+            dx, dgamma, dbeta = hip_ops().layernorm_bwd(
+                dy, x, gamma, mean, rstd, None, False, True)
+            return dx, dgamma, dbeta, None
+        dx, dgamma, dbeta = reference.layernorm_bwd(dy, x, gamma, mean, rstd)
         return dx, dgamma.to(gamma.dtype), dbeta.to(gamma.dtype), None
 
 
@@ -65,7 +65,8 @@
 class _AddLayerNormFn(torch.autograd.Function):
 
     @staticmethod
-    def forward(ctx, x, residual, gamma, beta, eps):
+    def forward(ctx, x, residual, gamma, beta, eps, residual_bias=None):
+        ctx.rb_dtype = None if residual_bias is None else residual_bias.dtype
         if x.is_cuda:
             y, s, mean, rstd = hip_ops().layernorm_fwd(x, residual, gamma,
                                                        beta, eps)
@@ -79,20 +80,29 @@
     def backward(ctx, dy, ds):
         s, gamma, mean, rstd = ctx.saved_tensors
         dy = dy.contiguous()
+        want_dres = ctx.rb_dtype is not None and ctx.needs_input_grad[5]
+        dres = None
         if s.is_cuda:
             de = ds.contiguous() if ds is not None else None
-            dx, dgamma, dbeta = hip_ops().layernorm_bwd(dy, s, gamma, mean,
-                                                        rstd, de)
-        else:
-            dx, dgamma, dbeta = reference.layernorm_bwd(dy, s, gamma, mean, rstd)
-            if ds is not None:
-                dx = dx + ds
-        return dx, dx, dgamma.to(gamma.dtype), dbeta.to(gamma.dtype), None
-
-
-def fused_add_layernorm(x, residual, gamma, beta, eps: float = 1e-5):
+            out = hip_ops().layernorm_bwd(dy, s, gamma, mean, rstd, de,
+                                          want_dres, True)
+            dx, dgamma, dbeta = out[:3]
+            if want_dres:
+                dres = out[3].to(ctx.rb_dtype)
+            return dx, dx, dgamma, dbeta, None, dres
+        dx, dgamma, dbeta = reference.layernorm_bwd(dy, s, gamma, mean, rstd)
+        if ds is not None:
+            dx = dx + ds
+        if want_dres:
+            dres = reference.folded_bias_grad(dx).to(ctx.rb_dtype)
+        return (dx, dx, dgamma.to(gamma.dtype), dbeta.to(gamma.dtype), None,
+                dres)
+
+
+def fused_add_layernorm(x, residual, gamma, beta, eps: float = 1e-5,
+                        residual_bias=None):
     return _AddLayerNormFn.apply(x.contiguous(), residual.contiguous(),
-                                 gamma, beta, eps)
+                                 gamma, beta, eps, residual_bias)
 
 
 class _BiasGeluFn(torch.autograd.Function):
@@ -108,9 +118,8 @@
         x, b = ctx.saved_tensors
         dy = dy.contiguous()
         if x.is_cuda:
-            dx, dbias = hip_ops().bias_gelu_bwd(dy, x, b)
-        else:
-            dx, dbias = reference.bias_gelu_bwd(dy, x, b)
+            return tuple(hip_ops().bias_gelu_bwd(dy, x, b, True))
+        dx, dbias = reference.bias_gelu_bwd(dy, x, b)
         return dx, dbias.to(b.dtype)
 
 
@@ -319,7 +328,8 @@
 class _FlashAttentionPackedFn(torch.autograd.Function):
 
     @staticmethod
-    def forward(ctx, qkv, n_heads, mask, scale, seg=None):
+    def forward(ctx, qkv, n_heads, mask, scale, seg=None, qkv_bias=None):
+        ctx.qb_dtype = None if qkv_bias is None else qkv_bias.dtype
         if qkv.is_cuda:
             o, lse = hip_ops().flash_fwd_packed(qkv, n_heads, mask, scale,
                                                 seg)
@@ -345,10 +355,15 @@
         n_heads, mask, scale = ctx.n_heads, ctx.mask, ctx.scale
         seg = ctx.seg
         do = do.contiguous()
+        want_bias = ctx.qb_dtype is not None and ctx.needs_input_grad[5]
         if qkv.is_cuda:
+            if want_bias:
+                dqkv, dbias = hip_ops().flash_bwd_packed_bias(
+                    qkv, o, do, mask, lse, n_heads, scale, seg)
+                return dqkv, None, None, None, None, dbias.to(ctx.qb_dtype)
             dqkv = hip_ops().flash_bwd_packed(qkv, o, do, mask, lse,
                                               n_heads, scale, seg)
-            return dqkv, None, None, None, None
+            return dqkv, None, None, None, None, None
         bias = reference.segment_bias(seg) if seg is not None else None
         B, L, D3 = qkv.shape
         d = D3 // 3
@@ -365,14 +380,17 @@
         dqkv = torch.cat(
             [t.transpose(1, 2).reshape(B, L, d) for t in (dq, dk, dv)],
             dim=-1)
-        return dqkv, None, None, None, None
+        dbias = None
+        if want_bias:
+            dbias = reference.folded_bias_grad(dqkv).to(ctx.qb_dtype)
+        return dqkv, None, None, None, None, dbias
 
 
 def flash_attention_packed(qkv, n_heads: int, mask=None, scale: float = 1.0,
-                           seg=None):
+                           seg=None, qkv_bias=None):
     _check_mask_seg(mask, seg)
     return _FlashAttentionPackedFn.apply(qkv.contiguous(), n_heads, mask,
-                                         scale, seg)
+                                         scale, seg, qkv_bias)
 
 
 def flash_supported(head_dim: int, L: int) -> bool:
diff --git a/tosem2021_amd/ops/reference.py b/tosem2021_amd/ops/reference.py
--- a/tosem2021_amd/ops/reference.py
+++ b/tosem2021_amd/ops/reference.py
@@ -44,6 +44,10 @@
     dgamma = (dyf * xhat).sum(dim=0)
     dbeta = dyf.sum(dim=0)
     return dx.reshape(x.shape).to(x.dtype), dgamma, dbeta
+
+
+def folded_bias_grad(g: torch.Tensor) -> torch.Tensor:
+    return g.float().reshape(-1, g.shape[-1]).sum(dim=0)
 
 
 def bias_gelu_fwd(x: torch.Tensor, b: torch.Tensor) -> torch.Tensor:
```

Result: faster. 804,800 tokens/s, median of 6 (+1.1%).
